# youmi-zym/GO-SLAM

Hardware: AMD Instinct MI355X
Metric: BA keyframes/s (6 x FactorGraph.update: reproject + corr lookup + GRU + 2 GN BA iters) on synthetic 640x480 RGB-D (higher is better)
Workload: dtype f32 (BA/geometry; fp64 solve), f16 (corr volume, GRU convs); 1 GPU; configs[1]-shaped frontend window: 60x80 maps (480x640 RGB-D), P=25 keyframes, E=75 edges, 6 updates/keyframe, iters=2, RGB-D depth prior, upsample on; parallelism=replicas x1 (tracking does not shard)

## Files before the change

go_slam_amd/_lib.py:

```python
import ctypes
import os
import subprocess

_HERE = os.path.dirname(os.path.abspath(__file__))
CSRC = os.path.join(_HERE, "csrc")
LIB_PATH = os.environ.get("GOSLAM_HIP_LIB") or os.path.join(CSRC, "libgoslam_hip.so")

_lib = None

c_int, c_float, c_void_p, c_size_t = ctypes.c_int, ctypes.c_float, ctypes.c_void_p, ctypes.c_size_t

_P = c_void_p
SIGNATURES = {
    "gs_version": (ctypes.c_char_p, []),
    "gs_last_error": (ctypes.c_char_p, []),
    "gs_enc_conv_wpack_elems": (c_size_t, [c_int, c_int, c_int]),
    "gs_enc_conv_stat_chunks": (c_int, [c_int, c_int, c_int]),
    "gs_enc_conv": (c_int, [_P, c_int, c_int, _P, _P, _P, c_int, c_int, c_int, c_int, c_int, c_int, c_int, _P, _P, _P]),
    "gs_norm_act_workspace_bytes_chunks": (c_size_t, [c_int, c_int, c_int]),
    "gs_timing_begin": (c_int, [_P]),
    "gs_timing_end": (c_int, []),
    "gs_timing_read": (c_int, [ctypes.c_char_p, ctypes.POINTER(ctypes.c_double), ctypes.POINTER(c_int)]),
    "gs_timing_names": (c_int, [ctypes.c_char_p, c_int]),
    "gs_corr_index_forward": (c_int, [_P, _P, _P] + [c_int] * 7 + [_P]),
    "gs_corr_index_backward": (c_int, [_P, _P, _P] + [c_int] * 7 + [_P]),
    "gs_corr_lookup_pyramid": (c_int, [_P] * 6 + [c_int] * 9 + [_P]),
    "gs_corr_lookup_enc": (c_int, [_P] * 8 + [c_int] * 7 + [_P]),
    "gs_corr_lookup_enc_slots": (c_int, [_P] * 9 + [c_int] * 7 + [_P]),
    "gs_corr_lookup_pyramid_slots": (c_int, [_P] * 7 + [c_int] * 9 + [_P]),
    "gs_corr_volume_pyramid_slots": (c_int, [_P] * 7 + [c_int] * 5 + [_P, c_size_t, _P]),
    "gs_corr_volume_workspace_bytes": (c_size_t, [c_int] * 4),
    "gs_corr_volume_pyramid": (c_int, [_P] * 6 + [c_int] * 5 + [_P, c_size_t, _P]),
    "gs_corr_level_elems": (c_size_t, [c_int] * 4),
    "gs_altcorr_backward": (c_int, [_P] * 6 + [c_int] * 8 + [_P]),
    "gs_altcorr_forward": (c_int, [_P] * 4 + [c_int] * 9 + [_P]),
    "gs_altcorr_pyramid": (c_int, [_P] * 8 + [c_int] * 5 + [_P]),
    "gs_reproject": (c_int, [_P] * 7 + [c_int] * 3 + [_P]),
    "gs_projmap": (c_int, [_P] * 7 + [c_int] * 3 + [_P]),
    "gs_frame_distance": (c_int, [_P] * 6 + [c_int] * 3 + [c_float, _P]),
    "gs_iproj": (c_int, [_P] * 4 + [c_int] * 3 + [_P]),
    "gs_depth_filter": (c_int, [_P] * 6 + [c_int] * 4 + [_P]),
    "gs_pointcloud_workspace_bytes": (c_size_t, [c_int] * 3),
    "gs_pointcloud_count": (c_int, [_P] * 5 + [c_float, c_float] + [c_int] * 4 + [_P, c_size_t, _P]),
    "gs_pointcloud_mask": (c_int, [_P, _P] + [c_int] * 4 + [_P, c_size_t, _P]),
    "gs_pointcloud_scan": (c_int, [c_int] * 3 + [_P, c_size_t, _P, _P]),
    "gs_pointcloud_emit": (c_int, [_P] * 5 + [c_int] * 4 + [_P, c_size_t, ctypes.c_longlong, _P, _P, _P]),
    "gs_tsdf_batch": (c_int, []),
    "gs_tsdf_integrate": (c_int, [_P] * 3 + [c_int] * 3 + [_P] * 4 + [c_int] * 3 + [c_float] * 10 + [_P]),
    "gs_tsdf_vertex_attr": (c_int, [_P, c_int, _P, _P, c_int, c_int, c_int, c_float, _P, _P, _P]),
    "gs_tsdf_brick_flags_bytes": (c_size_t, [c_int] * 3),
    "gs_tsdf_brick_flags": (c_int, [_P, c_int, c_int, c_int, _P, _P]),
    "gs_tsdf_raycast": (c_int, [_P] * 3 + [c_int] * 3 + [_P, _P] + [c_int] * 3 + [c_float] * 12 + [_P] * 4),
    "gs_frame_prep_color": (c_int, [_P, c_int, c_int, c_int, c_int, c_int, _P]),
    "gs_frame_prep_depth": (c_int, [_P, c_int, c_float, c_int, c_int, c_int, c_int, _P]),
    "gs_cvx_upsample":(c_int, [_P] * 4 + [c_int] * 4 + [_P]),
    "gs_upmask_upsample": (c_int, [_P, c_int, _P, _P, _P, _P, _P, c_int, c_int, c_int, _P]),
    "gs_bias_act": (c_int, [_P, _P, _P, c_int, c_int, c_int, c_int, c_int, _P]),
    "gs_motion_features": (c_int, [_P, _P, _P, c_int, c_int, c_int, _P]),
    "gs_ba_inputs": (c_int, [_P] * 6 + [c_int, c_int, c_int, _P]),
    "gs_lowmem_gather": (c_int, [_P] * 7 + [c_int, c_int, c_int, _P]),
    "gs_lowmem_scatter": (c_int, [_P] * 8 + [c_int, c_int, c_int, _P]),
    "gs_damping_rows": (c_int, [_P] * 5 + [c_int, c_int, c_float, c_float, _P]),
    "gs_conv1x1": (c_int, [_P, c_int, c_int, _P, _P, c_int, _P, c_int, c_int, ctypes.c_longlong, _P]),
    "gs_conv7x7_c4": (c_int, [_P, _P, _P, _P, c_int, c_int, c_int, c_int, c_int, c_int, _P]),
    "gs_conv3x3_wpack_elems": (c_size_t, [c_int, c_int]),
    "gs_conv3x3_pp": (c_int, [_P, c_int, c_int, _P, c_int, _P, c_int, c_int, c_int, c_int, c_int, c_int, _P]),
    "gs_conv3x3_bias_relu": (c_int, [_P, c_int, c_int, _P, _P, _P, c_int, c_int, c_int, c_int, c_int, _P]),
    "gs_conv3x3_gru_zr": (c_int, [_P, c_int, c_int, _P, _P, _P, _P, _P, _P, c_int, c_int, c_int, _P]),
    "gs_conv3x3_gru_zr2": (c_int, [_P, _P, c_int, c_int, _P, _P, _P, _P, _P, _P, c_int, c_int, c_int, _P]),
    "gs_conv3x3_gru_q": (c_int, [_P, _P, c_int, c_int, _P, _P, _P, _P, _P, _P, _P, c_int, c_int, c_int, _P]),
    "gs_conv3x3_head": (c_int, [_P, c_int, _P, c_int, _P, _P, c_int, c_int, c_float, _P, c_int, c_int, c_int, _P]),
    "gs_conv3x3_heads": (c_int, [_P, c_int, c_int, _P, c_int, _P, _P, c_int, _P, _P, c_int, c_int, c_int, c_int, c_int, _P]),
    "gs_conv3x3_heads_finish": (c_int, [_P, _P, _P, c_int, c_int, c_float, c_float, _P, _P, c_int, c_int, c_int, _P]),
    "gs_segment_mean": (c_int, [_P, c_int, _P, c_int, _P, _P, _P, c_int, c_int, c_int, _P]),
    "gs_norm_act_workspace_bytes": (c_size_t, [c_int, c_int, c_int]),
    "gs_norm_act": (c_int, [_P, _P, _P, _P] + [c_int] * 6 + [c_float, _P, c_size_t, c_int, _P]),
    "gs_gru_glo_workspace_bytes": (c_size_t, [c_int]),
    "gs_gru_glo": (c_int, [_P] * 11 + [c_int, c_int, _P, c_size_t, _P]),
    "gs_gru_glo_fused_workspace_bytes": (c_size_t, [c_int, c_int]),
    "gs_gru_glo_fused": (c_int, [_P, c_int] + [_P] * 10 + [c_int, c_int, _P, c_size_t, _P]),
    "gs_gru_gate_zr": (c_int, [_P] * 6 + [c_int] * 3 + [_P]),
    "gs_gru_gate_q": (c_int, [_P] * 7 + [c_int] * 2 + [_P]),
    "gs_edge_prep": (c_int, [_P] * 4 + [c_int, _P, _P] + [c_int] * 6 + [c_float, c_int, c_int, _P]),
    "gs_edge_greedy": (c_int, [_P] * 5 + [c_int] * 5 + [c_float, c_int, c_int, _P]),
    "gs_ba_workspace_bytes": (c_size_t, [c_int] * 5),
    "gs_ba": (c_int, [_P] * 9 + [c_int] * 3 + [c_float, c_float] + [c_int] * 6 + [_P, _P, _P, _P, c_size_t, _P]),
    "gs_ba_ex": (c_int, [_P] * 9 + [c_int] * 3 + [c_float, c_float] + [c_int] * 6 + [_P, _P, _P, _P, c_size_t, c_int, _P]),
    "gs_chol_solve": (c_int, [_P, _P, c_int, c_float, c_float, c_int, _P, _P, _P]),
    "gs_traj_eval_workspace_bytes": (c_size_t, [c_int]),
    "gs_traj_world": (c_int, [_P, _P, c_int, _P, _P, _P]),
    "gs_ape_moments": (c_int, [_P, _P, _P, c_int, _P, _P, c_size_t, _P]),
    "gs_ape_stats": (c_int, [_P, _P, _P, _P, c_int, _P, _P, _P, c_size_t, _P]),
    "gs_grid_meta_default": (c_int, [_P]),
    "gs_neus_level_major_min_points": (c_int, [c_int]),
    "gs_render_sample": (c_int, [_P] * 7 + [c_float, _P, _P, _P] + [c_int] * 3 + [_P]),
    "gs_grid_encode": (c_int, [_P] * 4 + [c_int, _P]),
    "gs_grid_backward": (c_int, [_P, _P, _P, c_int, c_float, _P, _P, c_int, c_float, _P, _P, c_int, _P]),
    "gs_mlp_workspace_bytes": (c_size_t, [c_int, c_int]),
    "gs_mlp_forward": (c_int, [_P] * 3 + [c_int] * 3 + [_P, c_size_t, _P]),
    "gs_neus_forward_workspace_bytes": (c_size_t, [c_int, c_int]),
    "gs_neus_forward": (c_int, [_P] * 9 + [c_float] + [_P] * 18 + [c_float, _P, c_float, c_int, c_int, _P, c_size_t, _P]),
    "gs_neus_forward_pieces": (c_int, [c_int] * 3),
    "gs_neus_forward_segmented": (c_int, [_P] * 9 + [c_float] + [_P] * 18 + [c_float, c_int, _P, _P, c_float]
                                  + [c_int] * 4 + [_P, c_size_t, _P]),
    "gs_render_img_sample": (c_int, [_P, c_int, c_int] + [c_float] * 4 + [_P] * 5 + [c_int] + [_P] * 5
                             + [c_int, c_int, _P]),
    "gs_render_img_metrics_workspace_bytes": (c_size_t, []),
    "gs_render_img_metrics": (c_int, [_P] * 7 + [c_int, c_int] + [_P] * 5 + [c_size_t, _P]),
    "gs_image_quality_tile": (c_int, [ctypes.POINTER(c_int), ctypes.POINTER(c_int)]),
    "gs_image_quality_workspace_bytes": (c_size_t, [c_int, c_int]),
    "gs_image_quality": (c_int, [_P] * 4 + [c_int, c_int, _P, _P, c_size_t, _P]),
    "gs_neus_backward_rays": (c_int, [_P] * 13 + [c_int, c_int, _P]),
    "gs_mapping_loss": (c_int, [_P] * 8 + [c_float] * 4 + [c_int] + [_P] * 4 + [c_int, c_int, _P]),
    "gs_map_grad_sqnorm": (c_int, [_P, c_size_t, c_float, _P, c_size_t, _P, _P]),
    "gs_map_adamw": (c_int, [_P, _P, _P, _P, _P, c_size_t, c_float, _P, c_size_t] + [c_float] * 6 + [c_int, _P, c_float, _P]),
    "gs_map_gram_blocks": (c_int, [c_int]),
    "gs_map_gram": (c_int, [_P, c_int, _P, _P]),
    "gs_map_step_prep": (c_int, [_P, c_int, _P, c_float, c_float, c_int] + [_P] * 13),
    "gs_map_step_post": (c_int, [_P, c_int, c_float, _P, c_int, _P, _P, _P, c_float, _P, _P, c_int, c_float, c_int, _P, _P, _P]),
    "gs_map_adamw_seg": (c_int, [_P, _P, _P, _P, _P, c_size_t, c_float, _P, _P, _P, _P, _P, c_size_t] + [c_float] * 6
                         + [c_int, _P, _P, c_float, _P]),
    "gs_mlp_backward_blocks": (c_int, [c_int]),
    "gs_mlp_backward": (c_int, [_P, _P, _P, _P, c_float, _P, _P, c_int, _P]),
    "gs_neus_backward_points": (c_int, [_P] * 7 + [c_float] + [_P] * 9 + [c_int, c_float, _P, _P, c_int, c_float] + [_P] * 5 + [c_int, c_float, c_int, _P, c_int, c_int, _P, _P]),
    "gs_neus_backward_points_binned": (c_int, [_P] * 7 + [c_float] + [_P] * 9 + [c_int, c_float, _P, _P, c_float] + [_P] * 5
                                       + [c_int, c_float, c_int, _P, c_int, c_int, _P, c_size_t, _P, _P, _P]),
    "gs_neus_bin_workspace_bytes": (c_size_t, [c_int]),
    "gs_neus_backward_raygrad": (c_int, [_P] * 7 + [c_float] + [_P] * 9 + [c_int, c_float] + [_P] * 3
                                 + [c_int, c_int, _P]),
    "gs_pose_grad_reduce": (c_int, [_P, _P, _P, c_int, _P, _P]),
    "gs_ray_draw": (c_int, [_P] * 7 + [c_int] * 4 + [c_float] * 4 + [_P] * 5),
    "gs_sdf_lattice": (c_int, [_P] * 3 + [c_int] * 3 + [_P] * 6 + [_P]),
    "gs_mcubes_workspace_bytes": (c_size_t, [c_int] * 3),
    "gs_mcubes_count": (c_int, [_P, c_int, c_int, c_int, c_float, _P, c_size_t, _P]),
    "gs_mcubes_scan": (c_int, [c_int, c_int, c_int, _P, c_size_t, _P, _P]),
    "gs_mcubes_emit": (c_int, [_P, c_int, c_int, c_int, c_float, _P, c_size_t, ctypes.c_longlong, ctypes.c_longlong,
                               _P, _P, _P]),
    "gs_mesh_depth_workspace_bytes": (c_size_t, []),
    "gs_mesh_depth": (c_int, [_P, c_int, _P, c_int, _P, c_int] + [c_float] * 4 + [c_int, c_int, c_float, c_float, _P, _P,
                                                                                   c_size_t, _P]),
    "gs_mesh_visibility": (c_int, [_P, c_int, _P, _P, c_int] + [c_float] * 4 + [c_int, c_int, c_float, _P, _P, _P]),
    "gs_face_components_workspace_bytes": (c_size_t, [c_int]),
    "gs_face_components": (c_int, [_P, c_int, _P, _P, c_size_t, _P]),
    "gs_face_component_areas": (c_int, [_P, _P, c_int, _P, _P, _P, _P, _P, c_size_t, _P]),
    "gs_hull_extremes_workspace_bytes": (c_size_t, [c_int]),
    "gs_hull_extremes": (c_int, [_P, c_int, _P, _P, c_size_t, _P]),
    "gs_hull_prefilter": (c_int, [_P, c_int, _P, c_int, ctypes.c_double, _P, _P]),
    "gs_mesh_visbuf_workspace_bytes": (c_size_t, []),
    "gs_mesh_visbuf": (c_int, [_P, c_int, _P, c_int, _P, c_int] + [c_float] * 4 + [c_int, c_int, c_float, c_float, _P, _P,
                                                                                    c_size_t, _P]),
    "gs_line_visbuf": (c_int, [_P, c_int, ctypes.c_uint, _P, c_int] + [c_float] * 4 + [c_int, c_int, c_float, c_float, _P,
                                                                                        _P]),
    "gs_vertex_normals": (c_int, [_P, c_int, _P, c_int, ctypes.c_double, _P, _P, _P]),
    "gs_visbuf_resolve": (c_int, [_P, c_int, c_int, c_int, _P, c_int, _P, c_int, _P] + [c_float] * 4
                          + [_P, _P, c_int, _P, c_int, c_float, c_float, ctypes.c_uint, _P, _P]),
    "gs_nn_cell_keys":(c_int, [_P, c_int, _P, _P, _P, _P]),
    "gs_nn_grid_build": (c_int, [_P, c_int, _P, _P, _P, _P, _P, _P, _P]),
    "gs_nn_query_workspace_bytes": (c_size_t, [c_int]),
    "gs_nn_query": (c_int, [_P, _P, _P, _P, c_int, _P, _P, _P, c_int, _P, ctypes.c_double, _P, _P, _P, c_size_t, _P]),
    "gs_icp_moments_workspace_bytes": (c_size_t, [c_int]),
    "gs_icp_moments": (c_int, [_P, c_int, _P, _P, _P, _P, _P, _P, c_size_t, _P]),
}


class ColorView(ctypes.Structure):
    _fields_ = [("src", c_void_p), ("map_x", c_void_p), ("map_y", c_void_p), ("tmp", c_void_p), ("dst", c_void_p),
                ("h", c_int), ("w", c_int), ("c", c_int), ("mh", c_int), ("mw", c_int)]


class DepthView(ctypes.Structure):
    _fields_ = [("src", c_void_p), ("dst", c_void_p), ("h", c_int), ("w", c_int)]


FRAME_PREP_MAX_VIEWS = 32


class GridMeta(ctypes.Structure):
    _fields_ = [("scale", c_float * 16), ("resolution", ctypes.c_uint32 * 16), ("size", ctypes.c_uint32 * 16),
                ("offset", ctypes.c_uint32 * 16), ("hashed", ctypes.c_uint32 * 16), ("total", ctypes.c_uint32)]


def grid_meta():
    m = GridMeta()
    check(lib().gs_grid_meta_default(ctypes.byref(m)), "gs_grid_meta_default")
    return m


def build(verbose=False):
    cmd = ["make", "-C", CSRC, "-j8"]
    res = subprocess.run(cmd, stdout=subprocess.PIPE, stderr=subprocess.STDOUT, text=True)
    if verbose or res.returncode != 0:
        print(res.stdout)
    if res.returncode != 0:
        raise RuntimeError("building libgoslam_hip.so failed:\n" + res.stdout[-4000:])
    return LIB_PATH


def lib():
    global _lib
    if _lib is None:
        if not os.path.exists(LIB_PATH):
            raise RuntimeError(
                f"{LIB_PATH} not found: build it with `python -c 'import __graft_entry__ as g; g.build()'` "
                "(go_slam_amd has no CPU fallback)")
        handle = ctypes.CDLL(LIB_PATH)
        for name, (res, args) in SIGNATURES.items():
            fn = getattr(handle, name)
            fn.restype = res
            fn.argtypes = args
        _lib = handle
    return _lib


def check(rc, what):
    if rc != 0:
# ... 49 lines not shown
```

go_slam_amd/csrc/ba.hip:

```cpp
#include "common.h"

int gs_chol_solve_launch(double* H, double* b, int n, float lm, float ep, float* dx_out, int32_t* fail_flag,
                         int32_t* fail_count, hipStream_t st);

namespace {

constexpr float kMinDepth = 0.25f;
constexpr float kAlpha = 0.05f;
constexpr int kPrepThreads = 1024;
constexpr int kAccSplit = 4;
constexpr int kMaxBuf = 4096;

struct BaWs {
  int32_t* hdr;
  int32_t* kinv;
  int32_t* kx;
  int32_t* edge_m;
  int32_t* row_ptr;
  int32_t* csr_edge;
  int32_t* ent_ptr;
  int32_t* ent_src;
  int32_t* ent_pose;
  int32_t* pair_ptr;
  float* Q;
  float* W;
  float* Ei;
  float* Eij;
  float* part;
  double* H;
  double* b;
  size_t total;
};

BaWs carve(void* base, int E, int P, int M, int nbuf, int hw) {
  BaWs w;
  size_t off = 0;
  auto take = [&](size_t bytes) { size_t o = off; off += gs_align(bytes); return (char*)base + o; };
  w.hdr = (int32_t*)take(16 * 4);
  w.kinv = (int32_t*)take((size_t)nbuf * 4);
  w.kx = (int32_t*)take((size_t)(M + 1) * 4);
  w.edge_m = (int32_t*)take((size_t)(E + 1) * 4);
  w.row_ptr = (int32_t*)take((size_t)(M + 2) * 4);
  w.csr_edge = (int32_t*)take((size_t)(E + 1) * 4);
  w.ent_ptr = (int32_t*)take((size_t)(M + 2) * 4);
  w.ent_src = (int32_t*)take((size_t)(M + E + 1) * 4);
  w.ent_pose = (int32_t*)take((size_t)(M + E + 1) * 4);
  w.pair_ptr = (int32_t*)take((size_t)(M + 2) * 4);
  w.Q = (float*)take((size_t)M * hw * 4);
  w.W = (float*)take((size_t)M * hw * 4);
  w.Ei = (float*)take((size_t)M * 6 * hw * 4);
  w.Eij = (float*)take((size_t)E * 6 * hw * 4);
  w.part = (float*)take((size_t)kAccSplit * M * 8 * hw * 4);
  const size_t n = (size_t)6 * P;
  w.H = (double*)take((n * n + n) * 8);
  w.b = w.H + n * n;
  w.total = off;
  return w;
}

__device__ void block_exclusive_scan(int* data, int n, int* scratch , int* total) {
  const int tid = threadIdx.x;
  const int per = (n + kPrepThreads - 1) / kPrepThreads;
  const int beg = min(tid * per, n), end = min(beg + per, n);
  int s = 0;
  for (int i = beg; i < end; ++i) s += data[i];
  scratch[tid] = s;
  __syncthreads();
  for (int off = 1; off < kPrepThreads; off <<= 1) {
    int v = (tid >= off) ? scratch[tid - off] : 0;
    __syncthreads();
    scratch[tid] += v;
    __syncthreads();
  }
  int run = scratch[tid] - s;
  for (int i = beg; i < end; ++i) {
    int v = data[i];
    data[i] = run;
    run += v;
  }
  if (tid == kPrepThreads - 1) *total = scratch[tid];
  __syncthreads();
}

__global__ __launch_bounds__(kPrepThreads) void ba_prep_kernel(
    const int64_t* __restrict__ ii, const int64_t* __restrict__ jj, int E, int nbuf, int t0, int t1,
    int M_host, BaWs w) {
  __shared__ int flag[kMaxBuf];
  __shared__ int cnt_a[kMaxBuf];
  __shared__ int cnt_b[kMaxBuf];
  __shared__ int scratch[kPrepThreads];
  __shared__ int total;
  const int tid = threadIdx.x;

  for (int k = tid; k < nbuf; k += kPrepThreads) flag[k] = (k >= t0 && k < t1) ? 1 : 0;
  __syncthreads();
  for (int e = tid; e < E; e += kPrepThreads) {
    const int i = (int)ii[e];
    if (i >= 0 && i < nbuf) flag[i] = 1;
  }
  __syncthreads();
  for (int k = tid; k < nbuf; k += kPrepThreads) cnt_a[k] = flag[k];
  __syncthreads();
  block_exclusive_scan(flag, nbuf, scratch, &total);
  const int M_dev = total;
  const int M = min(M_dev, M_host);
  for (int k = tid; k < nbuf; k += kPrepThreads) {
    const bool mem = cnt_a[k] != 0;
    const int r = flag[k];
    const int row = (mem && r < M) ? r : -1;
    w.kinv[k] = row;
    if (row >= 0) w.kx[row] = k;
  }
  if (tid == 0) {
    w.hdr[0] = M_dev;
    w.hdr[1] = (M_dev != M_host) ? 1 : 0;
    w.hdr[2] = 0;
    w.hdr[3] = 0;
  }
  __syncthreads();
  for (int m = tid; m < kMaxBuf; m += kPrepThreads) { cnt_a[m] = 0; cnt_b[m] = 0; }
  __syncthreads();
  for (int k = tid; k < nbuf; k += kPrepThreads) {
    const int row = w.kinv[k];
    if (row >= 0 && k >= t0 && k < t1) cnt_b[row] = 1;
  }
  __syncthreads();
  for (int e = tid; e < E; e += kPrepThreads) {
    const int i = (int)ii[e], j = (int)jj[e];
    const int row = (i >= 0 && i < nbuf) ? w.kinv[i] : -1;
    w.edge_m[e] = row;
    if (row >= 0) {
      atomicAdd(&cnt_a[row], 1);
      if (j >= t0 && j < t1) atomicAdd(&cnt_b[row], 1);
    }
  }
  __syncthreads();
  for (int m = tid; m < M_host; m += kPrepThreads) flag[m] = cnt_b[m] * cnt_b[m];
  __syncthreads();
  block_exclusive_scan(cnt_a, M_host, scratch, &total);
  if (tid == 0) w.row_ptr[M_host] = total;
  block_exclusive_scan(cnt_b, M_host, scratch, &total);
  if (tid == 0) w.ent_ptr[M_host] = total;
  block_exclusive_scan(flag, M_host, scratch, &total);
  if (tid == 0) { w.pair_ptr[M_host] = total; w.hdr[4] = total; }
  __syncthreads();
  for (int m = tid; m < M_host; m += kPrepThreads) {
    w.row_ptr[m] = cnt_a[m];
    w.ent_ptr[m] = cnt_b[m];
    w.pair_ptr[m] = flag[m];
  }
  __syncthreads();
  for (int m = tid; m < M; m += kPrepThreads) {
    int rp = cnt_a[m], ep = cnt_b[m];
    const int k = w.kx[m];
    if (k >= t0 && k < t1) { w.ent_src[ep] = m; w.ent_pose[ep] = k - t0; ++ep; }
    for (int e = 0; e < E; ++e) {
      if (w.edge_m[e] == m) {
        w.csr_edge[rp++] = e;
        const int j = (int)jj[e];
        if (j >= t0 && j < t1) { w.ent_src[ep] = M_host + e; w.ent_pose[ep] = j - t0; ++ep; }
      }
    }
  }
}

__global__ __launch_bounds__(256) void ba_accum_kernel(
    const float* __restrict__ poses, const float* __restrict__ disps, const float* __restrict__ intr,
    const float* __restrict__ disps_sens, const float* __restrict__ targets, const float* __restrict__ weights,
    const float* __restrict__ eta, const int64_t* __restrict__ jj, int t0, int t1, int hw, int wd,
    int motion_only, int reset_fail, BaWs w) {
  __shared__ float red[4][92];
  if (reset_fail && blockIdx.x == 0 && blockIdx.y == 0 && blockIdx.z == 0 && threadIdx.x == 0) { w.hdr[2] = 0; w.hdr[3] = 0; }
  typedef const __attribute__((address_space(4))) int* cip;
  typedef const __attribute__((address_space(4))) int64_t* clp;
  typedef const __attribute__((address_space(4))) float* cfp;
  const int m = blockIdx.y;
  if (m >= ((cip)w.hdr)[0]) return;
  const int split = blockIdx.z, nsp = gridDim.z;
  const int nsplit = min(nsp, max(((cip)w.row_ptr)[m + 1] - ((cip)w.row_ptr)[m], 1));
  if (split >= nsplit) return;
  const int tid = threadIdx.x;
  const int p = blockIdx.x * 256 + tid;
  const bool active = p < hw;
  const int pc = active ? p : hw - 1;
  const int k = ((cip)w.kx)[m];
  const int P = t1 - t0;
  const int n6 = 6 * P;
  const float fx = ((cfp)intr)[0], fy = ((cfp)intr)[1], cx = ((cfp)intr)[2], cy = ((cfp)intr)[3];
  const float u = (float)(pc % wd), v = (float)(pc / wd);
  const float disp = disps[(size_t)k * hw + pc];
  float Xi[4] = {(u - cx) / fx, (v - cy) / fy, 1.0f, disp};
  float ti[3], qi[4];
  {
    cfp pp = (cfp)(poses + (size_t)k * 7);
    ti[0] = pp[0]; ti[1] = pp[1]; ti[2] = pp[2];
    qi[0] = pp[3]; qi[1] = pp[4]; qi[2] = pp[5]; qi[3] = pp[6];
  }
  const int pi = k - t0;
  const bool i_in = (pi >= 0) && (pi < P);

  float Csum = 0.f, wsum = 0.f;
  float Ei[6] = {0.f, 0.f, 0.f, 0.f, 0.f, 0.f};

  const int e_beg = ((cip)w.row_ptr)[m], e_end = ((cip)w.row_ptr)[m + 1];
  for (int idx = e_beg + split; idx < e_end; idx += nsp) {
    const int e = ((cip)w.csr_edge)[idx];
    const int jx = (int)((clp)jj)[e];
    const size_t tb = ((size_t)e * 2) * hw + pc;
    const float w_u = weights[tb], w_v = weights[tb + hw], t_u = targets[tb], t_v = targets[tb + hw];
    float tij[3], qij[4];
    if (jx == k) {
      tij[0] = -0.1f; tij[1] = 0.f; tij[2] = 0.f;
      qij[0] = 0.f; qij[1] = 0.f; qij[2] = 0.f; qij[3] = 1.f;
    } else {
      cfp pj = (cfp)(poses + (size_t)jx * 7);
      float tj[3] = {pj[0], pj[1], pj[2]};
      float qj[4] = {pj[3], pj[4], pj[5], pj[6]};
      gs_rel_se3(ti, qi, tj, qj, tij, qij);
    }
    float Xj[4];
    gs_act_se3(tij, qij, Xi, Xj);
    const float x = Xj[0], y = Xj[1], h = Xj[3];
    const bool close = Xj[2] < kMinDepth;
    const float d = close ? 0.0f : 1.0f / Xj[2];
    const float d2 = d * d;
    float wu = (close || !active) ? 0.0f : 0.001f * w_u;
    float wv = (close || !active) ? 0.0f : 0.001f * w_v;
    const float ru = t_u - (fx * d * x + cx);
    const float rv = t_v - (fy * d * y + cy);

    float hij[78];
#pragma unroll
    for (int l = 0; l < 78; ++l) hij[l] = 0.f;
    float vi[6], vj[6], Eii_e[6], Eij_e[6];
    float Jx[12];
    float* Ji = &Jx[0];
    float* Jj = &Jx[6];

    Jj[0] = fx * (h * d);
    Jj[1] = fx * 0.0f;
    Jj[2] = fx * (-x * h * d2);
    Jj[3] = fx * (-x * y * d2);
    Jj[4] = fx * (1.0f + x * x * d2);
    Jj[5] = fx * (-y * d);
    float Jz = fx * (tij[0] * d - tij[2] * (x * d2));
    float Ce = wu * Jz * Jz;
    float be = wu * ru * Jz;
    if (jx == k) wu = 0.0f;
    gs_adj_se3(tij, qij, Jj, Ji);
#pragma unroll
    for (int n = 0; n < 6; ++n) Ji[n] = -Ji[n];
    {
      int l = 0;
#pragma unroll
      for (int n = 0; n < 12; ++n)
#pragma unroll
        for (int mm = 0; mm <= n; ++mm) { hij[l] = fmaf(wu * Jx[n], Jx[mm], hij[l]); ++l; }
    }
#pragma unroll
    for (int n = 0; n < 6; ++n) {
      vi[n] = wu * ru * Ji[n];
      vj[n] = wu * ru * Jj[n];
      Eii_e[n] = wu * Jz * Ji[n];
      Eij_e[n] = wu * Jz * Jj[n];
    }
    Jj[0] = fy * 0.0f;
    Jj[1] = fy * (h * d);
    Jj[2] = fy * (-y * h * d2);
    Jj[3] = fy * (-1.0f - y * y * d2);
    Jj[4] = fy * (x * y * d2);
    Jj[5] = fy * (x * d);
    Jz = fy * (tij[1] * d - tij[2] * (y * d2));
    Ce = Ce + wv * Jz * Jz;
    be = be + wv * rv * Jz;
    if (jx == k) wv = 0.0f;
    gs_adj_se3(tij, qij, Jj, Ji);
#pragma unroll
    for (int n = 0; n < 6; ++n) Ji[n] = -Ji[n];
    {
      int l = 0;
#pragma unroll
      for (int n = 0; n < 12; ++n)
#pragma unroll
        for (int mm = 0; mm <= n; ++mm) { hij[l] = fmaf(wv * Jx[n], Jx[mm], hij[l]); ++l; }
    }
#pragma unroll
    for (int n = 0; n < 6; ++n) {
      vi[n] = vi[n] + wv * rv * Ji[n];
      vj[n] = vj[n] + wv * rv * Jj[n];
      Eii_e[n] = Eii_e[n] + wv * Jz * Ji[n];
      Eij_e[n] = Eij_e[n] + wv * Jz * Jj[n];
    }

    if (!motion_only) {
      Csum += Ce;
      wsum += be;
#pragma unroll
      for (int n = 0; n < 6; ++n) Ei[n] += Eii_e[n];
      if (active) {
        float* eo = w.Eij + ((size_t)e * 6) * hw + p;
#pragma unroll
        for (int n = 0; n < 6; ++n) eo[(size_t)n * hw] = Eij_e[n];
      }
    }

    const int pj_ = jx - t0;
    const bool j_in = (pj_ >= 0) && (pj_ < P);
    if (i_in || j_in) {
      const int wave = tid >> 6, lane = tid & 63;
      float rs[90];
#pragma unroll
      for (int l = 0; l < 78; ++l) rs[l] = hij[l];
#pragma unroll
      for (int n = 0; n < 6; ++n) { rs[78 + n] = vi[n]; rs[84 + n] = vj[n]; }
      gs_wave_reduce_scatter<90>(rs, lane);
      const int ix = gs_bitrev6(lane);
      red[wave][ix] = rs[0];
      if (64 + ix < 90) red[wave][64 + ix] = rs[1];
      __syncthreads();
      if (tid < 90) {
        const double s = (double)((red[0][tid] + red[1][tid]) + (red[2][tid] + red[3][tid]));
        if (tid < 78) {
          int n = 0;
          while ((n + 1) * (n + 2) / 2 <= tid) ++n;
          const int mm = tid - n * (n + 1) / 2;
// ... 13 lines not shown
      }
      __syncthreads();
    }
  }

  if (!motion_only && active) {
    if (nsplit > 1) {
      float* po = w.part + (((size_t)split * gridDim.y + m) * 8) * hw + p;
      po[0] = Csum;
      po[(size_t)hw] = wsum;
#pragma unroll
      for (int n = 0; n < 6; ++n) po[(size_t)(2 + n) * hw] = Ei[n];
      return;
    }
    const size_t o = (size_t)m * hw + p;
    const float sens = disps_sens[(size_t)k * hw + p];
    const float mk = (sens > 0.0f) ? 1.0f : 0.0f;
    const float C = Csum + mk * kAlpha + (1.0f - mk) * eta[o];
    const float ww = wsum - mk * kAlpha * (disp - sens);
    w.Q[o] = 1.0f / C;
    w.W[o] = ww;
    if (i_in) {
      float* eo = w.Ei + ((size_t)m * 6) * hw + p;
#pragma unroll
      for (int n = 0; n < 6; ++n) eo[(size_t)n * hw] = Ei[n];
    }
  }
}

__global__ __launch_bounds__(256) void ba_accum_finish_kernel(const float* __restrict__ disps,
                                                              const float* __restrict__ disps_sens,
                                                              const float* __restrict__ eta, int t0, int t1, int hw, int nsp,
                                                              BaWs w) {
  const int m = blockIdx.y;
  if (m >= w.hdr[0]) return;
  const int nsplit = min(nsp, max(w.row_ptr[m + 1] - w.row_ptr[m], 1));
  if (nsplit <= 1) return;
  const int p = blockIdx.x * 256 + threadIdx.x;
  if (p >= hw) return;
  float acc[8];
#pragma unroll
  for (int n = 0; n < 8; ++n) acc[n] = 0.0f;
  for (int s2 = 0; s2 < nsplit; ++s2) {
    const float* pi_ = w.part + (((size_t)s2 * gridDim.y + m) * 8) * hw + p;
#pragma unroll
    for (int n = 0; n < 8; ++n) acc[n] += pi_[(size_t)n * hw];
  }
  const int k = w.kx[m];
  const size_t o = (size_t)m * hw + p;
  const float disp = disps[(size_t)k * hw + p];
  const float sens = disps_sens[(size_t)k * hw + p];
  const float mk = (sens > 0.0f) ? 1.0f : 0.0f;
  const float C = acc[0] + mk * kAlpha + (1.0f - mk) * eta[o];
  const float ww = acc[1] - mk * kAlpha * (disp - sens);
  w.Q[o] = 1.0f / C;
  w.W[o] = ww;
  const int pi = k - t0;
  if (pi >= 0 && pi < t1 - t0) {
    float* eo = w.Ei + ((size_t)m * 6) * hw + p;
#pragma unroll
    for (int n = 0; n < 6; ++n) eo[(size_t)n * hw] = acc[2 + n];
  }
}

__global__ __launch_bounds__(256) void ba_schur_kernel(int M, int hw, int P, BaWs w) {
  __shared__ float red[4][44];
  const int tid = threadIdx.x;
  const int wave = tid >> 6, lane = tid & 63;
  typedef const __attribute__((address_space(4))) int* cip;
  cip pair_ptr = (cip)w.pair_ptr, ent_ptr = (cip)w.ent_ptr, ent_pose = (cip)w.ent_pose, ent_src = (cip)w.ent_src;
  const int n_pairs = pair_ptr[M];
  const int n6 = 6 * P;
  for (int pidx = blockIdx.x; pidx < n_pairs; pidx += gridDim.x) {
    int lo = 0, hi = M;
    while (hi - lo > 1) {
      const int mid = (lo + hi) >> 1;
      if (pair_ptr[mid] <= pidx) lo = mid; else hi = mid;
    }
    const int m = lo;
    const int eb = ent_ptr[m];
    const int nm = ent_ptr[m + 1] - eb;
    const int r = pidx - pair_ptr[m];
    const int a = r / nm, b = r - a * nm;
    const int pa = ent_pose[eb + a], pb = ent_pose[eb + b];
    if (pa < pb) continue;
    const int sa = ent_src[eb + a], sb = ent_src[eb + b];
    const float* Ea = (sa < M) ? w.Ei + (size_t)sa * 6 * hw : w.Eij + (size_t)(sa - M) * 6 * hw;
    const float* Eb = (sb < M) ? w.Ei + (size_t)sb * 6 * hw : w.Eij + (size_t)(sb - M) * 6 * hw;
    const float* Qm = w.Q + (size_t)m * hw;
    const float* Wm = w.W + (size_t)m * hw;
    const bool diag = (a == b);
    float S[36];
#pragma unroll
    for (int i = 0; i < 36; ++i) S[i] = 0.f;
    float vv[6] = {0.f, 0.f, 0.f, 0.f, 0.f, 0.f};
    constexpr int UP = 4;
    for (int p0 = tid; p0 < hw; p0 += UP * 256) {
      float q[UP], ea[UP][6], eb_[UP][6], ww[UP];
#pragma unroll
      for (int u = 0; u < UP; ++u) {
        const int p = p0 + 256 * u;
        const bool ok = p < hw;
        const int pc = ok ? p : tid;
        q[u] = Qm[pc];
#pragma unroll
        for (int n = 0; n < 6; ++n) {
          ea[u][n] = Ea[(size_t)n * hw + pc];
          eb_[u][n] = Eb[(size_t)n * hw + pc];
        }
        ww[u] = diag ? Wm[pc] : 0.0f;
      }
#pragma unroll
      for (int u = 0; u < UP; ++u) {
        if (p0 + 256 * u < hw) {
#pragma unroll
          for (int n = 0; n < 6; ++n) ea[u][n] = ea[u][n] * q[u];
#pragma unroll
          for (int n = 0; n < 6; ++n)
#pragma unroll
            for (int c = 0; c < 6; ++c) S[n * 6 + c] = fmaf(ea[u][n], eb_[u][c], S[n * 6 + c]);
          if (diag) {
#pragma unroll
            for (int n = 0; n < 6; ++n) vv[n] = fmaf(ea[u][n], ww[u], vv[n]);
          }
        }
      }
    }
    {
      float rs[42];
#pragma unroll
      for (int i = 0; i < 36; ++i) rs[i] = S[i];
#pragma unroll
      for (int n = 0; n < 6; ++n) rs[36 + n] = vv[n];
      gs_wave_reduce_scatter<42>(rs, lane);
      const int ix = gs_bitrev6(lane);
      if (ix < 42) red[wave][ix] = rs[0];
    }
    __syncthreads();
    if (tid < 36) {
      const int rr = tid / 6, cc = tid - rr * 6;
      const double s = (double)((red[0][tid] + red[1][tid]) + (red[2][tid] + red[3][tid]));
      if (pa > pb || rr >= cc)
        gs_atomic_add_f64(&w.H[(size_t)(6 * pa + rr) * n6 + (6 * pb + cc)], -s);
    } else if (diag && tid < 42) {
      const double s = (double)((red[0][tid] + red[1][tid]) + (red[2][tid] + red[3][tid]));
      gs_atomic_add_f64(&w.b[6 * pa + (tid - 36)], -s);
    }
    __syncthreads();
  }
}

__global__ __launch_bounds__(256) void ba_update_kernel(
    float* __restrict__ poses, float* __restrict__ disps, const float* __restrict__ dx,
    float* __restrict__ dz, int M, int t0, int t1, int hw, BaWs w) {
  const int tid = threadIdx.x;
  const int P = t1 - t0;
  if ((int)blockIdx.y == M) {
    if (blockIdx.x != 0) return;
    for (int kk = t0 + tid; kk < t1; kk += 256) {
      float* pp = poses + (size_t)kk * 7;
      float t[3] = {pp[0], pp[1], pp[2]};
      float q[4] = {pp[3], pp[4], pp[5], pp[6]};
      float xi[6], tn[3], qn[4];
#pragma unroll
      for (int n = 0; n < 6; ++n) xi[n] = dx[(size_t)(kk - t0) * 6 + n];
      gs_retr_se3(xi, t, q, tn, qn);
      pp[0] = tn[0]; pp[1] = tn[1]; pp[2] = tn[2];
      pp[3] = qn[0]; pp[4] = qn[1]; pp[5] = qn[2]; pp[6] = qn[3];
    }
    return;
  }
  const int m = blockIdx.y;
  const int p = blockIdx.x * 256 + tid;
  if (p >= hw) return;
  if (m >= w.hdr[0]) {
    dz[(size_t)m * hw + p] = 0.0f;
    return;
  }
  const int eb = w.ent_ptr[m], ee = w.ent_ptr[m + 1];
  float dw = 0.f;
  for (int idx = eb; idx < ee; ++idx) {
    const int pn = w.ent_pose[idx];
    if (pn <= 0 || pn >= P) continue;
    const int s = w.ent_src[idx];
    const float* En = (s < M) ? w.Ei + (size_t)s * 6 * hw : w.Eij + (size_t)(s - M) * 6 * hw;
    float acc = 0.f;
#pragma unroll
    for (int n = 0; n < 6; ++n) acc += En[(size_t)n * hw + p] * dx[(size_t)pn * 6 + n];
    dw += acc;
  }
  const size_t o = (size_t)m * hw + p;
  const float z = w.Q[o] * (w.W[o] - dw);
  dz[o] = z;
  const size_t dk = (size_t)w.kx[m] * hw + p;
  disps[dk] = disps[dk] + z;
}

__global__ void ba_status_kernel(int32_t* status_out, BaWs w) {
  if (threadIdx.x < 4) status_out[threadIdx.x] = (threadIdx.x == 2) ? w.hdr[3] : (threadIdx.x == 3 ? w.hdr[4] : w.hdr[threadIdx.x]);
}

}

extern "C" size_t gs_ba_workspace_bytes(int n_edges, int n_poses, int n_depth, int nbuf, int hw) {
  if (n_edges < 0 || n_poses < 0 || n_depth < 0 || nbuf < 0 || hw < 0) return 0;
  return carve(nullptr, n_edges, n_poses, n_depth, nbuf, hw).total + 256;
}

extern "C" int gs_ba_ex(float* poses, float* disps, const float* intrinsics, const float* disps_sens,
                        const float* targets, const float* weights, const float* eta, const int64_t* ii,
                        const int64_t* jj, int t0, int t1, int iterations, float lm, float ep, int motion_only,
                        int n_edges, int n_depth, int nbuf, int h, int w, float* dx, float* dz,
                        int32_t* status_out, void* workspace, size_t workspace_bytes, int flags, gs_stream_t stream) {
  GS_REQUIRE(poses && disps && intrinsics && disps_sens && targets && weights && ii && jj && dx && workspace,
             "ba: null pointer");
  GS_REQUIRE(motion_only || (eta && dz), "ba: eta/dz required unless motion_only");
  GS_REQUIRE(h > 0 && w > 0 && n_edges >= 0 && iterations >= 0, "ba: bad shape");
  GS_REQUIRE(t0 >= 0 && t1 > t0 && t1 <= nbuf, "ba: window [%d,%d) outside buffer of %d frames", t0, t1, nbuf);
  GS_REQUIRE(nbuf <= kMaxBuf, "ba: buffer of %d frames exceeds the supported %d", nbuf, kMaxBuf);
  GS_REQUIRE(n_depth > 0 && n_depth <= nbuf && n_depth <= 65534, "ba: n_depth=%d out of range", n_depth);
  const int hw = h * w, P = t1 - t0, M = n_depth;
  const size_t need = gs_ba_workspace_bytes(n_edges, P, M, nbuf, hw);
  if (workspace_bytes < need) {
    gs_set_error("ba: workspace too small (%zu < %zu bytes)", workspace_bytes, need);
    return GS_ERR_WORKSPACE;
  }
  void* base = (void*)gs_align((size_t)workspace);
  BaWs ws = carve(base, n_edges, P, M, nbuf, hw);
  hipStream_t st = (hipStream_t)stream;
  const int n6 = 6 * P;

  const bool reuse = (flags & 1) != 0;
  if (!reuse) {
    ba_prep_kernel<<<1, kPrepThreads, 0, st>>>(ii, jj, n_edges, nbuf, t0, t1, M, ws);
    GS_CHECK_LAUNCH("ba_prep");
  }
  const int chunks = gs_cdiv(hw, 256);
  for (int it = 0; it < iterations; ++it) {
    if (hipMemsetAsync(ws.H, 0, ((size_t)n6 * n6 + n6) * sizeof(double), st) != hipSuccess) {
      gs_set_error("ba: memset failed");
      return GS_ERR_LAUNCH;
    }
    const int nsp = (!motion_only && n_edges >= 6 * M) ? kAccSplit : 1;
    ba_accum_kernel<<<dim3(chunks, M, nsp), 256, 0, st>>>(poses, disps, intrinsics, disps_sens, targets, weights,
                                                          eta, jj, t0, t1, hw, w, motion_only,
                                                          (reuse && it == 0) ? 1 : 0, ws);
    GS_CHECK_LAUNCH("ba_accum");
    if (!motion_only) {
      if (nsp > 1) {
        ba_accum_finish_kernel<<<dim3(chunks, M), 256, 0, st>>>(disps, disps_sens, eta, t0, t1, hw, nsp, ws);
        GS_CHECK_LAUNCH("ba_accum_finish");
      }
      ba_schur_kernel<<<2048, 256, 0, st>>>(M, hw, P, ws);
      GS_CHECK_LAUNCH("ba_schur");
    }
    int rc = gs_chol_solve_launch(ws.H, ws.b, n6, lm, ep, dx, &ws.hdr[2], &ws.hdr[3], st);
    if (rc != GS_OK) return rc;
    if (motion_only)
      ba_update_kernel<<<dim3(1, 1), 256, 0, st>>>(poses, disps, dx, dz, 0, t0, t1, hw, ws);
    else
      ba_update_kernel<<<dim3(chunks, M + 1), 256, 0, st>>>(poses, disps, dx, dz, M, t0, t1, hw, ws);
    GS_CHECK_LAUNCH("ba_update");
  }
  if (status_out) {
    ba_status_kernel<<<1, 64, 0, st>>>(status_out, ws);
    GS_CHECK_LAUNCH("ba_status");
  }
  return GS_OK;
}

extern "C" int gs_ba(float* poses, float* disps, const float* intrinsics, const float* disps_sens,
                     const float* targets, const float* weights, const float* eta, const int64_t* ii,
                     const int64_t* jj, int t0, int t1, int iterations, float lm, float ep, int motion_only,
                     int n_edges, int n_depth, int nbuf, int h, int w, float* dx, float* dz,
                     int32_t* status_out, void* workspace, size_t workspace_bytes, gs_stream_t stream) {
  return gs_ba_ex(poses, disps, intrinsics, disps_sens, targets, weights, eta, ii, jj, t0, t1, iterations, lm, ep,
                  motion_only, n_edges, n_depth, nbuf, h, w, dx, dz, status_out, workspace, workspace_bytes, 0, stream);
}
```

go_slam_amd/csrc/chol.hip:

```cpp
#include "common.h"

namespace {

constexpr int NB = 32;
constexpr int PR = 64;
constexpr int TT = 64;
constexpr int SB = 64;

__device__ __forceinline__ double readlane_f64(double v, int lane) {
  const unsigned long long u = __builtin_bit_cast(unsigned long long, v);
  const unsigned int lo = __builtin_amdgcn_readlane((int)(u & 0xffffffffu), lane);
  const unsigned int hi = __builtin_amdgcn_readlane((int)(u >> 32), lane);
  return __builtin_bit_cast(double, ((unsigned long long)hi << 32) | lo);
}

__device__ __forceinline__ void sqrt_rsqrt(double x, double& s, double& rs) {
  const double r = __builtin_amdgcn_rsq(x);
  double g = x * r, h = 0.5 * r;
  double e = fma(-g, h, 0.5);
  g = fma(g, e, g); h = fma(h, e, h);
  e = fma(-g, h, 0.5);
  g = fma(g, e, g); h = fma(h, e, h);
  s = g; rs = h + h;
}
// ... 461 lines not shown
  for (int p0 = 0; p0 < n; p0 += PW) {
    const int pend = min(p0 + PW, n);
    for (int k0 = p0; k0 < pend; k0 += CB) {
      const int s0 = k0 + CB;
      const int rows = n + 1 - s0;
      const int kw = k0 - p0;
      if (kw > 0) {
        const int rr = tid / 3, cg = tid - 3 * rr;
        if (rr < rows + CB) {
          const int r = k0 + rr;
          const double* Xr = Lp + tri(r, p0);
          const int c0 = 2 * cg, c1 = c0 + 1;
          const bool ok0 = k0 + c0 <= r && k0 + c0 < n, ok1 = k0 + c1 <= r && k0 + c1 < n;
          const double* L0 = Lp + tri(min(k0 + c0, n - 1), p0);
          const double* L1 = Lp + tri(min(k0 + c1, n - 1), p0);
          double a0 = 0.0, a1 = 0.0;
#pragma unroll 6
          for (int k = 0; k < kw; ++k) {
            const double x = Xr[k];
            a0 = fma(x, L0[k], a0);
            a1 = fma(x, L1[k], a1);
          }
          if (ok0) Lp[tri(r, k0 + c0)] -= a0;
          if (ok1) Lp[tri(r, k0 + c1)] -= a1;
        }
        __syncthreads();
      }
      CHOL_ACC(2);
      const bool need = tid < ((max(rows, CB) + 63) & ~63);
      double l[CB][CB], inv[CB];
      if (need) {
#pragma unroll
        for (int i = 0; i < CB; ++i)
#pragma unroll
          for (int j = 0; j <= i; ++j) l[i][j] = Lp[tri(k0 + i, k0 + j)];
#pragma unroll
        for (int j = 0; j < CB; ++j) {
          double piv = l[j][j];
#pragma unroll
          for (int t = 0; t < j; ++t) piv = fma(-l[j][t], l[j][t], piv);
          if (!(piv > 0.0) && piv == piv) bad = true;
          sqrt_rsqrt(piv, l[j][j], inv[j]);
#pragma unroll
          for (int i = j + 1; i < CB; ++i) {
            double sacc = l[i][j];
#pragma unroll
            for (int t = 0; t < j; ++t) sacc = fma(-l[i][t], l[j][t], sacc);
            l[i][j] = sacc * inv[j];
          }
        }
      }
      CHOL_ACC(0);
      if (tid < rows) {
        double* Ar = Lp + tri(s0 + tid, k0);
        double x[CB];
#pragma unroll
        for (int j = 0; j < CB; ++j) {
          double s = Ar[j];
#pragma unroll
          for (int u = 0; u < j; ++u) s = fma(-x[u], l[j][u], s);
          x[j] = s * inv[j];
        }
#pragma unroll
        for (int j = 0; j < CB; ++j) Ar[j] = x[j];
      }
      CHOL_ACC(1);
      __syncthreads();
      if (tid < CB) {
#pragma unroll
        for (int i = 0; i < CB; ++i)
          if (i == tid) {
#pragma unroll
            for (int j = 0; j <= i; ++j) Lp[tri(k0 + i, k0 + j)] = l[i][j];
            invd[k0 + i] = inv[i];
          }
      }
      CHOL_ACC(3);
    }
    const int s1 = pend;
    const int rows1 = n + 1 - s1;
    const int pw = pend - p0;
    if (rows1 > 1) {
      typedef double double4v __attribute__((ext_vector_type(4)));
      const int T = (rows1 + 15) >> 4, ntile = (T * (T + 1)) >> 1;
      const int wv = __builtin_amdgcn_readfirstlane(tid >> 6), ln = tid & 63;
      for (int t = wv; t < ntile; t += SMALL_NT / 64) {
        int ti = (int)((sqrtf(8.0f * (float)t + 1.0f) - 1.0f) * 0.5f);
        while (((ti + 1) * (ti + 2)) >> 1 <= t) ++ti;
        while ((ti * (ti + 1)) >> 1 > t) --ti;
        const int tj = t - ((ti * (ti + 1)) >> 1);
        const int r0 = s1 + 16 * ti, c0 = s1 + 16 * tj;
        const double* pa = Lp + tri(min(r0 + (ln & 15), n), p0);
        const double* pb = Lp + tri(min(c0 + (ln & 15), n), p0);
        double4v acc = {0.0, 0.0, 0.0, 0.0};
#pragma unroll
        for (int kb = 0; kb < (PW + 3) / 4; ++kb) {
          const int k = 4 * kb + (ln >> 4);
          const double a = k < pw ? pa[k] : 0.0, b = k < pw ? pb[k] : 0.0;
          acc = __builtin_amdgcn_mfma_f64_16x16x4f64(a, b, acc, 0, 0, 0);
        }
        const int c = c0 + (ln & 15);
#pragma unroll
        for (int q = 0; q < 4; ++q) {
          const int rr = r0 + (ln >> 4) + 4 * q;
          if (rr <= n && c < n && c <= rr) Lp[tri(rr, c)] -= acc[q];
        }
      }
    }
    __syncthreads();
    CHOL_ACC(4);
  }
  CHOL_ACC_DUMP;
}

__device__ __forceinline__ void lds_backward(double* Lp, const double* invd, const int n, float* __restrict__ dx) {
  const int npk = (n * (n + 1)) >> 1;
  double* y = Lp + npk;
  if (threadIdx.x < 64) {
    const int lane = threadIdx.x;
    for (int k0 = n - CB; k0 >= 0; k0 -= CB) {
      double l[CB][CB], x[CB];
#pragma unroll
      for (int i = 0; i < CB; ++i)
#pragma unroll
        for (int j = 0; j <= i; ++j) l[i][j] = Lp[tri(k0 + i, k0 + j)];
#pragma unroll
      for (int i = CB - 1; i >= 0; --i) {
        double sacc = y[k0 + i];
#pragma unroll
        for (int t = i + 1; t < CB; ++t) sacc = fma(-l[t][i], x[t], sacc);
        x[i] = sacc * invd[k0 + i];
      }
      for (int c = k0 - 1 - lane; c >= 0; c -= 64) {
        double s = y[c];
#pragma unroll
        for (int i = 0; i < CB; ++i) s = fma(-Lp[tri(k0 + i, c)], x[i], s);
        y[c] = s;
      }
      if (lane < CB) {
        double xl = x[0];
#pragma unroll
        for (int i = 1; i < CB; ++i) xl = (i == lane) ? x[i] : xl;
        dx[k0 + lane] = (float)xl;
        y[k0 + lane] = xl;
      }
      __builtin_amdgcn_fence(__ATOMIC_RELEASE, "wavefront");
      __builtin_amdgcn_wave_barrier();
      __builtin_amdgcn_fence(__ATOMIC_ACQUIRE, "wavefront");
    }
  }
  __syncthreads();
}

__device__ __forceinline__ void lds_load_packed(double* Lp, const double* __restrict__ H, const double* __restrict__ bg,
                                                const int n, const int c0, const double lm, const double ep) {
  const int tid = threadIdx.x;
  const int m = n - c0;
  const int npk = (m * (m + 1)) >> 1;
  for (int base = 0; base < npk; base += SMALL_NT * 4) {
    double v[4];
    int dg[4];
#pragma unroll
    for (int u = 0; u < 4; ++u) {
      const int idx = base + u * SMALL_NT + tid;
      int r = (int)((sqrtf(8.0f * (float)idx + 1.0f) - 1.0f) * 0.5f);
      while (((r + 1) * (r + 2)) >> 1 <= idx) ++r;
      while ((r * (r + 1)) >> 1 > idx) --r;
      const int c = idx - ((r * (r + 1)) >> 1);
      dg[u] = (c == r) ? 1 : 0;
      v[u] = idx < npk ? H[(size_t)(c0 + r) * n + (c0 + c)] : 0.0;
    }
#pragma unroll
    for (int u = 0; u < 4; ++u) {
      const int idx = base + u * SMALL_NT + tid;
      if (idx < npk) Lp[idx] = dg[u] ? v[u] + (ep + lm * v[u]) : v[u];
    }
  }
  for (int i = tid; i <= m; i += SMALL_NT) Lp[npk + i] = (i < m) ? bg[c0 + i] : 0.0;
}

__global__ __launch_bounds__(SMALL_NT) void chol_small_kernel(const double* __restrict__ H, const double* __restrict__ bg,
                                                         int n, double lm, double ep, float* __restrict__ dx,
                                                         int32_t* fail_flag, int32_t* fail_count) {
  extern __shared__ double sm[];
  double* Lp = sm;
  double* invd = sm + (((n + 1) * (n + 2)) >> 1);
  const int tid = threadIdx.x;
  CHOL_STAMP(0);
  lds_load_packed(Lp, H, bg, n, 0, lm, ep);
  __syncthreads();
  CHOL_STAMP(1);

  __shared__ int s_bad;
  bool bad = false;
  lds_factor(Lp, invd, n, bad);
  CHOL_STAMP(2);

  if (tid == 0) s_bad = bad ? 1 : 0;
  __syncthreads();
  if (s_bad) {
    for (int i = tid; i < n; i += SMALL_NT) dx[i] = 0.0f;
    if (tid == 0) { *fail_flag = 1; *fail_count += 1; }
    return;
  }
  if (tid == 0) *fail_flag = 0;
  lds_backward(Lp, invd, n, dx);
  CHOL_STAMP(3);
}

#ifndef CHOL_TB
#define CHOL_TB 2
#endif
constexpr int MID_N = 300;
constexpr int MID_SW60_N = 300;

template <int KS>
__device__ __forceinline__ __attribute__((ext_vector_type(4))) double mid_tile_product(const double* pa, const double* pb,
                                                                                      int ln, int SW) {
  typedef double double4v __attribute__((ext_vector_type(4)));
  double4v acc = {0.0, 0.0, 0.0, 0.0};
  constexpr int G = 5;
#pragma unroll
  for (int g0 = 0; g0 < KS; g0 += G) {
    double a[G], b[G];
#pragma unroll
    for (int u = 0; u < G; ++u) {
      const int k = 4 * (g0 + u) + (ln >> 4);
      a[u] = (g0 + u < KS && k < SW) ? pa[k] : 0.0;
      b[u] = (g0 + u < KS && k < SW) ? pb[k] : 0.0;
    }
#pragma unroll
    for (int u = 0; u < G; ++u)
      if (g0 + u < KS) acc = __builtin_amdgcn_mfma_f64_16x16x4f64(a[u], b[u], acc, 0, 0, 0);
  }
  return acc;
}

__global__ __launch_bounds__(SMALL_NT) void chol_mid_kernel(double* __restrict__ H, double* __restrict__ bg, int n,
                                                       double lm, double ep, int SW, float* __restrict__ dx,
                                                       int32_t* fail_flag, int32_t* fail_count) {
  extern __shared__ double sm[];
  typedef double double4v __attribute__((ext_vector_type(4)));
  const int tid = threadIdx.x;
  const int wv = __builtin_amdgcn_readfirstlane(tid >> 6), ln = tid & 63;
  double* invd = sm;
  double* yv = sm + n;
  double* T = sm + 2 * n;
  const int SWP = SW + 1;
  __shared__ int s_bad;
  bool bad = false;
  for (int i = tid; i < n; i += SMALL_NT) {
    const double d = H[(size_t)i * n + i];
    H[(size_t)i * n + i] = d + (ep + lm * d);
  }
  __syncthreads();
  int c0 = 0;
  CHOL_STAMP(20);
  for (; n - c0 > SMALL_N; c0 += SW) {
    const int R = n + 1 - c0;
    const int stg_ = (c0 / SW) < 4 ? 21 + 4 * (c0 / SW) : 56;
    (void)stg_;
    for (int base = 0; base < R * SW; base += 4 * SMALL_NT) {
      double v[4];
      int at[4];
#pragma unroll
      for (int u = 0; u < 4; ++u) {
        const int idx = base + u * SMALL_NT + tid;
        const int r = idx / SW, k = idx - r * SW;
        v[u] = 0.0;
        at[u] = idx < R * SW ? r * SWP + k : -1;
        if (idx < R * SW) {
          if (r == R - 1) v[u] = bg[c0 + k];
          else if (k <= r) v[u] = H[(size_t)(c0 + r) * n + (c0 + k)];
        }
      }
#pragma unroll
      for (int u = 0; u < 4; ++u)
        if (at[u] >= 0) T[at[u]] = v[u];
    }
    __syncthreads();
    CHOL_STAMP(stg_ + 0);
    for (int p0 = 0; p0 < SW; p0 += PW) {
      const int pend = p0 + PW;
      for (int k0 = p0; k0 < pend; k0 += CB) {
        const int s0 = k0 + CB;
        const int rows = R - s0;
        const int kw = k0 - p0;
        if (kw > 0) {
          const int cg = tid % 3;
          for (int rr = tid < 3 * (SMALL_NT / 3) ? tid / 3 : R; rr < rows + CB; rr += SMALL_NT / 3) {
            const int r = k0 + rr;
            const double* Xr = T + r * SWP + p0;
            const int c0 = 2 * cg, c1 = c0 + 1;
            const bool ok0 = k0 + c0 <= r, ok1 = k0 + c1 <= r;
            const double* L0 = T + (k0 + c0) * SWP + p0;
            const double* L1 = T + (k0 + c1) * SWP + p0;
            double a0 = 0.0, a1 = 0.0;
#pragma unroll 6
            for (int k = 0; k < kw; ++k) {
              const double x = Xr[k];
              a0 = fma(x, L0[k], a0);
              a1 = fma(x, L1[k], a1);
            }
            if (ok0) T[r * SWP + k0 + c0] -= a0;
            if (ok1) T[r * SWP + k0 + c1] -= a1;
          }
          __syncthreads();
        }
        const bool need = tid < ((max(rows, CB) + 63) & ~63);
        double l[CB][CB], inv[CB];
        if (need) {
#pragma unroll
          for (int i = 0; i < CB; ++i)
#pragma unroll
            for (int j = 0; j <= i; ++j) l[i][j] = T[(k0 + i) * SWP + (k0 + j)];
#pragma unroll
          for (int j = 0; j < CB; ++j) {
            double piv = l[j][j];
#pragma unroll
            for (int t = 0; t < j; ++t) piv = fma(-l[j][t], l[j][t], piv);
            if (!(piv > 0.0) && piv == piv) bad = true;
            sqrt_rsqrt(piv, l[j][j], inv[j]);
#pragma unroll
            for (int i = j + 1; i < CB; ++i) {
              double sacc = l[i][j];
#pragma unroll
              for (int t = 0; t < j; ++t) sacc = fma(-l[i][t], l[j][t], sacc);
              l[i][j] = sacc * inv[j];
            }
          }
        }
        if (tid < rows) {
          double* Ar = T + (s0 + tid) * SWP + k0;
          double x[CB];
#pragma unroll
          for (int j = 0; j < CB; ++j) {
            double s = Ar[j];
#pragma unroll
            for (int u = 0; u < j; ++u) s = fma(-x[u], l[j][u], s);
            x[j] = s * inv[j];
          }
#pragma unroll
// ... 63 lines not shown
            if (ok[u][q]) cur[u][q] = (rl == R - 1) ? bg[c0 + cl] : H[(size_t)(c0 + rl) * n + (c0 + cl)];
          }
        }
#pragma unroll
        for (int u = 0; u < TB; ++u) {
          if (tb + u >= ntile) break;
          const double* pa = T + min(r0s[u] + (ln & 15), R - 1) * SWP;
          const double* pb = T + min(q0s[u] + (ln & 15), R - 1) * SWP;
          const double4v acc = SW == 60 ? mid_tile_product<15>(pa, pb, ln, SW) : mid_tile_product<8>(pa, pb, ln, SW);
          const int cl = q0s[u] + (ln & 15);
#pragma unroll
          for (int q = 0; q < 4; ++q) {
            const int rl = r0s[u] + (ln >> 4) + 4 * q;
            if (ok[u][q]) {
              const double v = cur[u][q] - acc[q];
              if (rl == R - 1) bg[c0 + cl] = v;
              else H[(size_t)(c0 + rl) * n + (c0 + cl)] = v;
            }
          }
        }
      }
    }
    CHOL_STAMP(stg_ + 2);
    for (int idx = tid; idx < (R - 1) * SW; idx += SMALL_NT) {
      const int r = idx / SW, k = idx - r * SW;
      if (k <= r) H[(size_t)(c0 + r) * n + (c0 + k)] = T[r * SWP + k];
    }
    for (int k = tid; k < SW; k += SMALL_NT) yv[c0 + k] = T[(R - 1) * SWP + k];
    __threadfence_block();
    __syncthreads();
    CHOL_STAMP(stg_ + 3);
  }
  const int m = n - c0;
  double* Lp = T;
  lds_load_packed(Lp, H, bg, n, c0, 0.0, 0.0);
  __syncthreads();
  CHOL_STAMP(40);
  lds_factor(Lp, invd + c0, m, bad);
  CHOL_STAMP(41);
  if (tid == 0) s_bad = 0;
  __syncthreads();
  if (bad) s_bad = 1;
  __syncthreads();
  if (s_bad) {
    for (int i = tid; i < n; i += SMALL_NT) dx[i] = 0.0f;
    if (tid == 0) { *fail_flag = 1; *fail_count += 1; }
    return;
  }
  if (tid == 0) *fail_flag = 0;
  lds_backward(Lp, invd + c0, m, dx + c0);
  CHOL_STAMP(42);
  {
    const double* xt = Lp + ((m * (m + 1)) >> 1);
    for (int i = tid; i < m; i += SMALL_NT) yv[c0 + i] = xt[i];
  }
  __syncthreads();
  {
    double* part = T;
    const int ng = 8;
    for (int idx = tid; idx < ng * c0; idx += SMALL_NT) {
      const int g = idx / c0, c = idx - g * c0;
      double s = 0.0;
      for (int r = c0 + g; r < n; r += ng) s = fma(H[(size_t)r * n + c], yv[r], s);
      part[g * c0 + c] = s;
    }
    __syncthreads();
    for (int c = tid; c < c0; c += SMALL_NT) {
      double s = yv[c];
#pragma unroll
      for (int g = 0; g < 8; ++g) s -= part[g * c0 + c];
      yv[c] = s;
    }
    __syncthreads();
  }
  CHOL_STAMP(43);
  for (int a = c0 - SW; a >= 0; a -= SW) {
    for (int idx = tid; idx < SW * SW; idx += SMALL_NT) {
      const int r = idx / SW, k = idx - r * SW;
      T[r * SWP + k] = (k <= r) ? H[(size_t)(a + r) * n + (a + k)] : 0.0;
    }
    __syncthreads();
    for (int k0 = SW - CB; k0 >= 0; k0 -= CB) {
      double x[CB];
      if (tid < ((max(k0, CB) + 63) & ~63)) {
        double l[CB][CB];
#pragma unroll
        for (int i = 0; i < CB; ++i)
#pragma unroll
          for (int j = 0; j <= i; ++j) l[i][j] = T[(k0 + i) * SWP + (k0 + j)];
#pragma unroll
        for (int i = CB - 1; i >= 0; --i) {
          double sacc = yv[a + k0 + i];
#pragma unroll
          for (int t = i + 1; t < CB; ++t) sacc = fma(-l[t][i], x[t], sacc);
          x[i] = sacc * invd[a + k0 + i];
        }
      }
      __syncthreads();
      if (tid < CB) {
#pragma unroll
        for (int i = 0; i < CB; ++i)
          if (i == tid) { dx[a + k0 + i] = (float)x[i]; yv[a + k0 + i] = x[i]; }
      }
      for (int c = tid; c < k0; c += SMALL_NT) {
        double s = yv[a + c];
#pragma unroll
        for (int i = 0; i < CB; ++i) s = fma(-T[(k0 + i) * SWP + c], x[i], s);
        yv[a + c] = s;
      }
      __syncthreads();
    }
    if (a > 0) {
      double* part = T;
      const int ng = min(16, SMALL_NT / a);
      for (int idx = tid; idx < ng * a; idx += SMALL_NT) {
        const int g = idx / a, c = idx - g * a;
        double s = 0.0;
        for (int r = g; r < SW; r += ng) s = fma(H[(size_t)(a + r) * n + c], yv[a + r], s);
        part[g * a + c] = s;
      }
      __syncthreads();
      for (int c = tid; c < a; c += SMALL_NT) {
        double s = yv[c];
        for (int g = 0; g < ng; ++g) s -= part[g * a + c];
        yv[c] = s;
      }
      __syncthreads();
    }
  }
  CHOL_STAMP(44);
}

enum { CHOL_PATH_DISPATCH = 0, CHOL_PATH_SMALL = 1, CHOL_PATH_MID = 2, CHOL_PATH_BLOCKED = 3 };

size_t chol_mid_lds(int n) {
  const int SW = n <= MID_SW60_N ? 60 : 30;
  const size_t tall = (size_t)(n + 1) * (SW + 1);
  const size_t tail = (size_t)(SMALL_N + 1) * (SMALL_N + 2) / 2 + SMALL_N;
  return ((size_t)2 * n + (tall > tail ? tall : tail)) * sizeof(double);
}

bool chol_small_fits(int n) { return n >= 1 && n <= SMALL_N && n % CB == 0; }
bool chol_mid_fits(int n) {
  return n >= 1 && n <= MID_N && n % CB == 0 && chol_mid_lds(n) <= 160 * 1024 - 256;
}

int chol_dispatch(int n) {
  if (chol_small_fits(n)) return CHOL_PATH_SMALL;
  if (chol_mid_fits(n)) return CHOL_PATH_MID;
  return CHOL_PATH_BLOCKED;
}

int chol_solve_path(double* H, double* b, int n, float lm, float ep, int path, float* dx_out, int32_t* fail_flag,
                    int32_t* fail_count, hipStream_t st) {
  if (path == CHOL_PATH_SMALL) {
    const size_t lds = ((size_t)(n + 1) * (n + 2) / 2 + (size_t)n) * sizeof(double);
    static GsLdsLimit limit;
    const size_t cap = ((size_t)(SMALL_N + 1) * (SMALL_N + 2) / 2 + SMALL_N) * sizeof(double);
    if (int rc = limit.raise((const void*)chol_small_kernel, cap, "chol")) return rc;
    chol_small_kernel<<<1, SMALL_NT, lds, st>>>(H, b, n, (double)lm, (double)ep, dx_out, fail_flag, fail_count);
    GS_CHECK_LAUNCH("chol_small");
    return GS_OK;
  }
  if (path == CHOL_PATH_MID) {
    const int SW = n <= MID_SW60_N ? 60 : 30;
    const size_t lds = chol_mid_lds(n);
    static GsLdsLimit limit;
    if (int rc = limit.raise((const void*)chol_mid_kernel, lds, "chol_mid")) return rc;
    chol_mid_kernel<<<1, SMALL_NT, lds, st>>>(H, b, n, (double)lm, (double)ep, SW, dx_out, fail_flag, fail_count);
    GS_CHECK_LAUNCH("chol_mid");
    return GS_OK;
  }
  const int nb0 = n < NB ? n : NB;
  chol_panel_kernel<<<gs_cdiv(n - nb0 + 1, PR), 64, 0, st>>>(H, b, n, 0, fail_flag, 1, (double)lm, (double)ep);
  GS_CHECK_LAUNCH("chol_panel");
  constexpr size_t step_lds = ((size_t)NB * DS + (size_t)(2 * NB + 2 * PR) * (NB + 1) + NB) * sizeof(double);
  static_assert(step_lds >= (size_t)2 * TT * (NB + 1) * sizeof(double), "chol_step: the trailing role's operands fit");
  for (int kp = 0; kp + NB < n; kp += NB) {
    const int c1 = kp + NB, nb1 = (n - c1 < NB) ? (n - c1) : NB, rem1 = n - c1 - nb1;
    const int n_panel = gs_cdiv(rem1 + 1, PR);
    const int T = rem1 > 0 ? gs_cdiv(rem1 + 1, TT) : 0;
    chol_step_kernel<<<n_panel + T * (T + 1) / 2, 256, step_lds, st>>>(H, b, n, kp, n_panel, fail_flag);
    GS_CHECK_LAUNCH("chol_step");
  }
  int k0 = ((n - 1) / SB) * SB;
  for (; k0 >= SB; k0 -= 2 * SB) {
    const int k_lo = k0 - SB;
    chol_back_pair_kernel<<<gs_cdiv(k_lo, 192) + 1, 256, 0, st>>>(H, b, n, k_lo, dx_out, fail_flag, fail_count);
    GS_CHECK_LAUNCH("chol_back_pair");
  }
  if (k0 == 0) {
    chol_back_block_kernel<<<1, 256, 0, st>>>(H, b, n, 0, dx_out, fail_flag, fail_count);
    GS_CHECK_LAUNCH("chol_back_block");
  }
  return GS_OK;
}

}

int gs_chol_solve_launch(double* H, double* b, int n, float lm, float ep, float* dx_out, int32_t* fail_flag,
                         int32_t* fail_count, hipStream_t st) {
  return chol_solve_path(H, b, n, lm, ep, chol_dispatch(n), dx_out, fail_flag, fail_count, st);
}

extern "C" int gs_chol_solve(double* H, double* b, int n, float lm, float ep, int path, float* dx, int32_t* status,
                             gs_stream_t stream) {
  GS_REQUIRE(n >= 1, "chol_solve: n = %d < 1", n);
  GS_REQUIRE(path >= CHOL_PATH_DISPATCH && path <= CHOL_PATH_BLOCKED, "chol_solve: unknown path %d (0 .. 3)", path);
  if (path == CHOL_PATH_SMALL && !chol_small_fits(n)) {
    gs_set_error("chol_solve: the small path needs n <= %d and n %% %d == 0 (n = %d)", SMALL_N, CB, n);
    return GS_ERR_UNSUPPORTED;
  }
  if (path == CHOL_PATH_MID && !chol_mid_fits(n)) {
    gs_set_error("chol_solve: the mid path needs n <= %d, n %% %d == 0 and %zu B of LDS to fit (n = %d)", MID_N, CB,
                 chol_mid_lds(n), n);
    return GS_ERR_UNSUPPORTED;
  }
  GS_REQUIRE(H && b && dx && status, "chol_solve: null pointer");
  if (path == CHOL_PATH_DISPATCH) path = chol_dispatch(n);
  return chol_solve_path(H, b, n, lm, ep, path, dx, status, status + 1, (hipStream_t)stream);
}
```

go_slam_amd/csrc/common.h:

```cpp
#pragma once
#include <hip/hip_runtime.h>
#include <hip/hip_fp16.h>
#include <stdint.h>
#include <stdio.h>
#include <stdarg.h>

#include "../../include/goslam_hip.h"

#define GS_WAVE 64

void gs_set_error(const char* fmt, ...);

#define GS_REQUIRE(cond, ...)                      \
  do {                                             \
    if (!(cond)) {                                 \
      gs_set_error(__VA_ARGS__);                   \
      return GS_ERR_INVALID_ARG;                   \
    }                                              \
  } while (0)

extern thread_local int gs_timing_on;
void gs_timing_mark(const char* name);

#define GS_TIMING_PRE()                      \
  do {                                       \
    if (gs_timing_on) gs_timing_mark("");    \
  } while (0)

#define GS_CHECK_LAUNCH(name)                                                   \
  do {                                                                          \
     \
    hipError_t e_ = hipGetLastError();                                          \
    if (gs_timing_on) gs_timing_mark(name);                                     \
    if (e_ != hipSuccess) {                                                     \
      gs_set_error("%s: launch failed: %s", name, hipGetErrorString(e_));       \
      return GS_ERR_LAUNCH;                                                     \
    }                                                                           \
  } while (0)

#include <atomic>
struct GsLdsLimit {
  std::atomic<unsigned int> raised[64];
  GsLdsLimit() { for (auto& r : raised) r.store(0u, std::memory_order_relaxed); }
  int raise(const void* fn, size_t bytes, const char* what) {
    int dev = 0;
    if (hipGetDevice(&dev) != hipSuccess) dev = 0;
    std::atomic<unsigned int>& slot = raised[dev & 63];
    if (dev < 64 && slot.load(std::memory_order_acquire) >= bytes) return GS_OK;
    if (hipFuncSetAttribute(fn, hipFuncAttributeMaxDynamicSharedMemorySize, (int)bytes) != hipSuccess) {
      gs_set_error("%s: cannot raise the dynamic LDS limit to %zu bytes", what, bytes);
      return GS_ERR_LAUNCH;
    }
    unsigned int cur = slot.load(std::memory_order_relaxed);
    while (cur < bytes && !slot.compare_exchange_weak(cur, (unsigned int)bytes, std::memory_order_release)) {}
    return GS_OK;
  }
};

static inline int gs_cdiv(int a, int b) { return (a + b - 1) / b; }
static inline size_t gs_align(size_t x, size_t a = 256) { return (x + a - 1) / a * a; }


__device__ __forceinline__ void gs_act_so3(const float* q, const float* X, float* Y) {
  float uv0 = 2.0f * (q[1] * X[2] - q[2] * X[1]);
  float uv1 = 2.0f * (q[2] * X[0] - q[0] * X[2]);
  float uv2 = 2.0f * (q[0] * X[1] - q[1] * X[0]);
  Y[0] = X[0] + q[3] * uv0 + (q[1] * uv2 - q[2] * uv1);
  Y[1] = X[1] + q[3] * uv1 + (q[2] * uv0 - q[0] * uv2);
  Y[2] = X[2] + q[3] * uv2 + (q[0] * uv1 - q[1] * uv0);
}

__device__ __forceinline__ void gs_act_se3(const float* t, const float* q, const float* X, float* Y) {
  float R[3];
  gs_act_so3(q, X, R);
  Y[0] = R[0] + X[3] * t[0];
  Y[1] = R[1] + X[3] * t[1];
  Y[2] = R[2] + X[3] * t[2];
  Y[3] = X[3];
}

__device__ __forceinline__ void gs_adj_se3(const float* t, const float* q, const float* X, float* Y) {
  float qinv[4] = {-q[0], -q[1], -q[2], q[3]};
  gs_act_so3(qinv, &X[0], &Y[0]);
  gs_act_so3(qinv, &X[3], &Y[3]);
  float u[3], v[3];
  u[0] = t[2] * X[1] - t[1] * X[2];
  u[1] = t[0] * X[2] - t[2] * X[0];
  u[2] = t[1] * X[0] - t[0] * X[1];
  gs_act_so3(qinv, u, v);
  Y[3] = Y[3] + v[0];
  Y[4] = Y[4] + v[1];
  Y[5] = Y[5] + v[2];
}

__device__ __forceinline__ void gs_rel_se3(const float* ti, const float* qi, const float* tj,
                                           const float* qj, float* tij, float* qij) {
  qij[0] = -qj[3] * qi[0] + qj[0] * qi[3] - qj[1] * qi[2] + qj[2] * qi[1];
  qij[1] = -qj[3] * qi[1] + qj[1] * qi[3] - qj[2] * qi[0] + qj[0] * qi[2];
  qij[2] = -qj[3] * qi[2] + qj[2] * qi[3] - qj[0] * qi[1] + qj[1] * qi[0];
  qij[3] = qj[3] * qi[3] + qj[0] * qi[0] + qj[1] * qi[1] + qj[2] * qi[2];
  float r[3];
  gs_act_so3(qij, ti, r);
  tij[0] = tj[0] - r[0];
  tij[1] = tj[1] - r[1];
  tij[2] = tj[2] - r[2];
}

__device__ __forceinline__ void gs_quat_mul(const float* a, const float* b, float* o) {
  o[0] = a[3] * b[0] + a[0] * b[3] + a[1] * b[2] - a[2] * b[1];
  o[1] = a[3] * b[1] + a[1] * b[3] + a[2] * b[0] - a[0] * b[2];
  o[2] = a[3] * b[2] + a[2] * b[3] + a[0] * b[1] - a[1] * b[0];
  o[3] = a[3] * b[3] - a[0] * b[0] - a[1] * b[1] - a[2] * b[2];
}

__device__ __forceinline__ void gs_exp_so3(const float* phi, float* q) {
  float theta_sq = phi[0] * phi[0] + phi[1] * phi[1] + phi[2] * phi[2];
  float theta_p4 = theta_sq * theta_sq;
  float theta = sqrtf(theta_sq);
  float imag, real;
  if (theta_sq < 1e-8f) {
    imag = 0.5f - (1.0f / 48.0f) * theta_sq + (1.0f / 3840.0f) * theta_p4;
    real = 1.0f - (1.0f / 8.0f) * theta_sq + (1.0f / 384.0f) * theta_p4;
  } else {
    imag = sinf(0.5f * theta) / theta;
    real = cosf(0.5f * theta);
  }
  q[0] = imag * phi[0];
  q[1] = imag * phi[1];
  q[2] = imag * phi[2];
  q[3] = real;
}

__device__ __forceinline__ void gs_cross_inplace(const float* a, float* b) {
  float x0 = a[1] * b[2] - a[2] * b[1];
  float x1 = a[2] * b[0] - a[0] * b[2];
  float x2 = a[0] * b[1] - a[1] * b[0];
  b[0] = x0; b[1] = x1; b[2] = x2;
}

__device__ __forceinline__ void gs_exp_se3(const float* xi, float* t, float* q) {
  gs_exp_so3(xi + 3, q);
  float tau[3] = {xi[0], xi[1], xi[2]};
  float phi[3] = {xi[3], xi[4], xi[5]};
  float theta_sq = phi[0] * phi[0] + phi[1] * phi[1] + phi[2] * phi[2];
  float theta = sqrtf(theta_sq);
  t[0] = tau[0]; t[1] = tau[1]; t[2] = tau[2];
  if (theta > 1e-4f) {
    float a = (1.0f - cosf(theta)) / theta_sq;
    gs_cross_inplace(phi, tau);
    t[0] = t[0] + a * tau[0];
    t[1] = t[1] + a * tau[1];
    t[2] = t[2] + a * tau[2];
    float b = (theta - sinf(theta)) / (theta * theta_sq);
    gs_cross_inplace(phi, tau);
    t[0] = t[0] + b * tau[0];
    t[1] = t[1] + b * tau[1];
    t[2] = t[2] + b * tau[2];
  }
}

__device__ __forceinline__ void gs_retr_se3(const float* xi, const float* t, const float* q,
                                            float* t1, float* q1) {
  float dt[3], dq[4];
  gs_exp_se3(xi, dt, dq);
  gs_quat_mul(dq, q, q1);
  float r[3];
  gs_act_so3(dq, t, r);
  t1[0] = r[0] + dt[0];
  t1[1] = r[1] + dt[1];
  t1[2] = r[2] + dt[2];
}

template <int CTRL>
__device__ __forceinline__ float gs_dpp(float v) {
  return __builtin_bit_cast(float, __builtin_amdgcn_update_dpp(0, __builtin_bit_cast(int, v), CTRL, 0xf, 0xf, true));
}

__device__ __forceinline__ float gs_wave_sum(float v) {
  v = v + gs_dpp<0xB1>(v);
  v = v + gs_dpp<0x4E>(v);
  v = v + gs_dpp<0x141>(v);
  v = v + gs_dpp<0x140>(v);
  float r0 = __builtin_bit_cast(float, __builtin_amdgcn_readlane(__builtin_bit_cast(int, v), 0));
  float r1 = __builtin_bit_cast(float, __builtin_amdgcn_readlane(__builtin_bit_cast(int, v), 16));
  float r2 = __builtin_bit_cast(float, __builtin_amdgcn_readlane(__builtin_bit_cast(int, v), 32));
  float r3 = __builtin_bit_cast(float, __builtin_amdgcn_readlane(__builtin_bit_cast(int, v), 48));
  return (r0 + r1) + (r2 + r3);
}

__device__ __forceinline__ float gs_sigmoid(float x) { return __builtin_amdgcn_rcpf(1.0f + __expf(-x)); }
__device__ __forceinline__ float gs_tanh(float x) {
// ... 54 lines not shown
```

go_slam_amd/csrc/geom.hip:

```cpp
#include "geom_common.h"

namespace {

constexpr float kMinDepthKernel = 0.25f;
constexpr float kMinDepthPy = 0.2f;

__global__ __launch_bounds__(256) void reproject_kernel(
    const float* __restrict__ poses, const float* __restrict__ disps, const float* __restrict__ intr,
    const int64_t* __restrict__ ii, const int64_t* __restrict__ jj, float* __restrict__ coords,
    float* __restrict__ valid, int hw, int wd) {
  const int p = blockIdx.x * 256 + threadIdx.x;
  const int e = blockIdx.y;
  if (p >= hw) return;
  const int ix = (int)ii[e], jx = (int)jj[e];
  float tij[3], qij[4];
  if (ix == jx) {
    tij[0] = -0.1f; tij[1] = 0.f; tij[2] = 0.f;
    qij[0] = 0.f; qij[1] = 0.f; qij[2] = 0.f; qij[3] = 1.f;
  } else {
    float ti[3], qi[4], tj[3], qj[4];
    gs_load_pose(poses, ix, ti, qi);
    gs_load_pose(poses, jx, tj, qj);
    float qinv[4] = {-qi[0], -qi[1], -qi[2], qi[3]};
    float r[3], tinv[3];
    gs_act_so3(qinv, ti, r);
    tinv[0] = -r[0]; tinv[1] = -r[1]; tinv[2] = -r[2];
    gs_act_so3(qj, tinv, r);
    tij[0] = tj[0] + r[0]; tij[1] = tj[1] + r[1]; tij[2] = tj[2] + r[2];
    gs_quat_mul(qj, qinv, qij);
  }
  const float fxi = intr[ix * 4 + 0], fyi = intr[ix * 4 + 1], cxi = intr[ix * 4 + 2], cyi = intr[ix * 4 + 3];
  const float fxj = intr[jx * 4 + 0], fyj = intr[jx * 4 + 1], cxj = intr[jx * 4 + 2], cyj = intr[jx * 4 + 3];
  const float u = (float)(p % wd), v = (float)(p / wd);
  float X0[4] = {(u - cxi) / fxi, (v - cyi) / fyi, 1.0f, disps[(size_t)ix * hw + p]};
  float X1[4];
  gs_act_se3(tij, qij, X0, X1);
  const float Z = (X1[2] < 0.5f * kMinDepthPy) ? 1.0f : X1[2];
  const size_t o = (size_t)e * hw + p;
  reinterpret_cast<float2*>(coords)[o] = make_float2(fxj * (X1[0] / Z) + cxj, fyj * (X1[1] / Z) + cyj);
  valid[o] = ((X1[2] > kMinDepthPy) && (X0[2] > kMinDepthPy)) ? 1.0f : 0.0f;
}

__global__ __launch_bounds__(256) void projmap_kernel(
    const float* __restrict__ poses, const float* __restrict__ disps, const float* __restrict__ intr,
    const int64_t* __restrict__ ii, const int64_t* __restrict__ jj, float* __restrict__ coords,
    float* __restrict__ valid, int hw, int wd) {
  const int p = blockIdx.x * 256 + threadIdx.x;
  const int e = blockIdx.y;
  if (p >= hw) return;
  const int ix = (int)ii[e], jx = (int)jj[e];
  float ti[3], qi[4], tj[3], qj[4], tij[3], qij[4];
  gs_load_pose(poses, ix, ti, qi);
  gs_load_pose(poses, jx, tj, qj);
  gs_rel_se3(ti, qi, tj, qj, tij, qij);
  const float fx = intr[0], fy = intr[1], cx = intr[2], cy = intr[3];
  const float u = (float)(p % wd), v = (float)(p / wd);
  float Xi[4] = {(u - cx) / fx, (v - cy) / fy, 1.0f, disps[(size_t)ix * hw + p]};
  float Xj[4];
  gs_act_se3(tij, qij, Xi, Xj);
  float cu = u, cv = v;
  if (Xj[2] > 0.01f) {
    cu = fx * (Xj[0] / Xj[2]) + cx;
    cv = fy * (Xj[1] / Xj[2]) + cy;
  }
  const size_t o = (size_t)e * hw + p;
  coords[o * 3 + 0] = cu;
  coords[o * 3 + 1] = cv;
  coords[o * 3 + 2] = 0.0f;
  valid[o] = (Xj[2] > kMinDepthKernel) ? 1.0f : 0.0f;
}

__global__ __launch_bounds__(256) void frame_distance_kernel(
    const float* __restrict__ poses, const float* __restrict__ disps, const float* __restrict__ intr,
    const int64_t* __restrict__ ii, const int64_t* __restrict__ jj, float* __restrict__ dist,
    int hw, int wd, float beta) {
  const int e = blockIdx.x;
  const int ix = (int)ii[e], jx = (int)jj[e];
  float ti[3], qi[4], tj[3], qj[4], tij[3], qij[4];
  gs_load_pose(poses, ix, ti, qi);
  gs_load_pose(poses, jx, tj, qj);
  gs_rel_se3(ti, qi, tj, qj, tij, qij);
  const float fx = intr[0], fy = intr[1], cx = intr[2], cy = intr[3];
  float accum = 0.f, valid = 0.f;
  const float* dsp = disps + (size_t)ix * hw;
  for (int p = threadIdx.x; p < hw; p += 256) {
    const float u = (float)(p % wd), v = (float)(p / wd);
    float Xi[4] = {(u - cx) / fx, (v - cy) / fy, 1.0f, dsp[p]};
    float Xj[4];
    gs_act_se3(tij, qij, Xi, Xj);
    float du = fx * (Xj[0] / Xj[2]) + cx - u;
    float dv = fy * (Xj[1] / Xj[2]) + cy - v;
    float d = sqrtf(du * du + dv * dv);
    if (Xj[2] > kMinDepthKernel) { accum += beta * d; valid += beta; }
    float Yx = Xi[0] + Xi[3] * tij[0];
    float Yy = Xi[1] + Xi[3] * tij[1];
    float Yz = Xi[2] + Xi[3] * tij[2];
    du = fx * (Yx / Yz) + cx - u;
    dv = fy * (Yy / Yz) + cy - v;
    d = sqrtf(du * du + dv * dv);
    if (Yz > kMinDepthKernel) { accum += (1.0f - beta) * d; valid += (1.0f - beta); }
  }
  __shared__ float red[2][4];
  accum = gs_wave_sum(accum);
  valid = gs_wave_sum(valid);
  const int wave = threadIdx.x >> 6;
  if ((threadIdx.x & 63) == 0) { red[0][wave] = accum; red[1][wave] = valid; }
  __syncthreads();
  if (threadIdx.x == 0) {
    const float a = (red[0][0] + red[0][1]) + (red[0][2] + red[0][3]);
    const float vl = (red[1][0] + red[1][1]) + (red[1][2] + red[1][3]);
    const float total = (float)hw * (beta + (1.0f - beta));
    dist[e] = (vl / (total + 1e-8f) < 0.75f) ? 1000.0f : a / vl;
  }
}

__global__ __launch_bounds__(256) void iproj_kernel(
    const float* __restrict__ poses, const float* __restrict__ disps, const float* __restrict__ intr,
    float* __restrict__ points, int hw, int wd) {
  const int p = blockIdx.x * 256 + threadIdx.x;
  const int n = blockIdx.y;
  if (p >= hw) return;
  float t[3], q[4];
  gs_load_pose(poses, n, t, q);
  const float u = (float)(p % wd), v = (float)(p / wd);
  gs_iproj_point(t, q, intr[0], intr[1], intr[2], intr[3], u, v, disps[(size_t)n * hw + p],
                 points + ((size_t)n * hw + p) * 3);
}

__global__ __launch_bounds__(256) void depth_filter_kernel(
    const float* __restrict__ poses, const float* __restrict__ disps, const float* __restrict__ intr,
    const int64_t* __restrict__ inds, const float* __restrict__ thresh, float* __restrict__ counter,
    int num, int hw, int ht, int wd) {
  const int p = blockIdx.x * 256 + threadIdx.x;
  const int b = blockIdx.y;
  if (p >= hw) return;
  counter[(size_t)b * hw + p] = gs_depth_filter_count(poses, disps, (int)inds[b], p, intr[0], intr[1], intr[2],
                                                      intr[3], thresh[b], num, hw, ht, wd);
}

}

#define GS_GEOM_COMMON(name)                                                              \
  GS_REQUIRE(n >= 0 && h > 0 && w > 0, name ": bad shape");                               \
  if (n == 0) return GS_OK;                                                               \
  hipStream_t st = (hipStream_t)stream;                                                   \
  const int hw = h * w;

extern "C" int gs_reproject(const float* poses, const float* disps, const float* intrinsics,
                            const int64_t* ii, const int64_t* jj, float* coords, float* valid, int n, int h,
                            int w, gs_stream_t stream) {
  GS_REQUIRE(poses && disps && intrinsics && ii && jj && coords && valid, "reproject: null pointer");
  GS_GEOM_COMMON("reproject");
  GS_REQUIRE(n <= 65535, "reproject: n=%d exceeds grid.y limit", n);
  reproject_kernel<<<dim3(gs_cdiv(hw, 256), n), 256, 0, st>>>(poses, disps, intrinsics, ii, jj, coords, valid, hw, w);
  GS_CHECK_LAUNCH("reproject");
  return GS_OK;
}

extern "C" int gs_projmap(const float* poses, const float* disps, const float* intrinsics, const int64_t* ii,
                          const int64_t* jj, float* coords, float* valid, int n, int h, int w,
                          gs_stream_t stream) {
  GS_REQUIRE(poses && disps && intrinsics && ii && jj && coords && valid, "projmap: null pointer");
  GS_GEOM_COMMON("projmap");
  GS_REQUIRE(n <= 65535, "projmap: n=%d exceeds grid.y limit", n);
  projmap_kernel<<<dim3(gs_cdiv(hw, 256), n), 256, 0, st>>>(poses, disps, intrinsics, ii, jj, coords, valid, hw, w);
  GS_CHECK_LAUNCH("projmap");
  return GS_OK;
}

extern "C" int gs_frame_distance(const float* poses, const float* disps, const float* intrinsics,
                                 const int64_t* ii, const int64_t* jj, float* dist, int n, int h, int w,
                                 float beta, gs_stream_t stream) {
  GS_REQUIRE(poses && disps && intrinsics && ii && jj && dist, "frame_distance: null pointer");
  GS_GEOM_COMMON("frame_distance");
  frame_distance_kernel<<<n, 256, 0, st>>>(poses, disps, intrinsics, ii, jj, dist, hw, w, beta);
  GS_CHECK_LAUNCH("frame_distance");
  return GS_OK;
}

extern "C" int gs_iproj(const float* poses, const float* disps, const float* intrinsics, float* points, int n,
                        int h, int w, gs_stream_t stream) {
  GS_REQUIRE(poses && disps && intrinsics && points, "iproj: null pointer");
  GS_GEOM_COMMON("iproj");
  GS_REQUIRE(n <= 65535, "iproj: n=%d exceeds grid.y limit", n);
  iproj_kernel<<<dim3(gs_cdiv(hw, 256), n), 256, 0, st>>>(poses, disps, intrinsics, points, hw, w);
  GS_CHECK_LAUNCH("iproj");
  return GS_OK;
}

extern "C" int gs_depth_filter(const float* poses, const float* disps, const float* intrinsics,
                               const int64_t* ix, const float* thresh, float* counter, int n, int num, int h,
                               int w, gs_stream_t stream) {
  GS_REQUIRE(poses && disps && intrinsics && ix && thresh && counter, "depth_filter: null pointer");
  GS_GEOM_COMMON("depth_filter");
  GS_REQUIRE(n <= 65535 && num > 0, "depth_filter: bad n/num");
  depth_filter_kernel<<<dim3(gs_cdiv(hw, 256), n), 256, 0, st>>>(poses, disps, intrinsics, ix, thresh, counter, num, hw, h, w);
  GS_CHECK_LAUNCH("depth_filter");
  return GS_OK;
}
```

go_slam_amd/csrc/gru_gates.hip:

```cpp
#include "common.h"

namespace {

typedef _Float16 half8 __attribute__((ext_vector_type(8)));

__device__ __forceinline__ float sigm(float x) { return gs_sigmoid(x); }

__global__ __launch_bounds__(256) void gru_gate_zr_kernel(const _Float16* __restrict__ zr_pre,
                                                          const float* __restrict__ bias,
                                                          const float* __restrict__ glo,
                                                          const _Float16* __restrict__ inp_pre,
                                                          _Float16* __restrict__ hx,
                                                          _Float16* __restrict__ z_out, int hw, int ldx,
                                                          size_t total ) {
  const size_t t = (size_t)blockIdx.x * 256 + threadIdx.x;
  if (t >= total) return;
  const int c8 = (int)(t & 15);
  const size_t pix = t >> 4;
  const int n = (int)(pix / hw);
  const half8 zp = *reinterpret_cast<const half8*>(zr_pre + pix * 256 + c8 * 8);
  const half8 rp = *reinterpret_cast<const half8*>(zr_pre + pix * 256 + 128 + c8 * 8);
  half8* hp = reinterpret_cast<half8*>(hx + pix * ldx + c8 * 8);
  const half8 net = *hp;
  half8 zi = {0, 0, 0, 0, 0, 0, 0, 0}, ri = zi;
// ... 245 lines not shown
        acc[k] += __shfl_xor(acc[k], 8);
        acc[k] += __shfl_xor(acc[k], 16);
        acc[k] += __shfl_xor(acc[k], 32);
      }
      if (lane < 8) {
        float* dst = partial + blk * 128 + pr * 64 + lane * 8;
        *reinterpret_cast<float4*>(dst) = make_float4(acc[0], acc[1], acc[2], acc[3]);
        *reinterpret_cast<float4*>(dst + 4) = make_float4(acc[4], acc[5], acc[6], acc[7]);
      }
      __builtin_amdgcn_fence(__ATOMIC_RELEASE, "wavefront");
      __builtin_amdgcn_wave_barrier();
    }
  }
}

__global__ __launch_bounds__(384) void glo_heads_kernel(const float* __restrict__ partial, int nchunk, float inv_hw,
                                                        const _Float16* __restrict__ wz, const _Float16* __restrict__ wr,
                                                        const _Float16* __restrict__ wq, const float* __restrict__ bz,
                                                        const float* __restrict__ br, const float* __restrict__ bq,
                                                        float* __restrict__ gzr, float* __restrict__ gq) {
  const int n = blockIdx.x, t = threadIdx.x;
  __shared__ float g[128];
  __shared__ float part3[3][128];
  {
    const int third = t >> 7, ch = t & 127;
    float s = 0.0f;
    for (int c0 = third; c0 < nchunk; c0 += 30) {
      float v[10];
#pragma unroll
      for (int u = 0; u < 10; ++u) {
        const int c = c0 + 3 * u;
        v[u] = c < nchunk ? partial[((size_t)n * nchunk + c) * 128 + ch] : 0.0f;
      }
#pragma unroll
      for (int u = 0; u < 10; ++u)
        if (c0 + 3 * u < nchunk) s += v[u];
    }
    part3[third][ch] = s;
  }
  __syncthreads();
  if (t < 128) g[t] = (float)(_Float16)(((part3[0][t] + part3[1][t]) + part3[2][t]) * inv_hw);
  __syncthreads();
  const int head = t >> 7, o = t & 127;
  const _Float16* w = (head == 0 ? wz : head == 1 ? wr : wq) + (size_t)o * 128;
  float s = (head == 0 ? bz : head == 1 ? br : bq)[o];
#pragma unroll 4
  for (int k8 = 0; k8 < 16; ++k8) {
    const half8 v = *reinterpret_cast<const half8*>(w + k8 * 8);
#pragma unroll
    for (int k = 0; k < 8; ++k) s = fmaf((float)v[k], g[k8 * 8 + k], s);
  }
  s = (float)(_Float16)s;
  if (head < 2) gzr[(size_t)n * 256 + head * 128 + o] = s;
  else gq[(size_t)n * 128 + o] = s;
}
}

extern "C" int gs_bias_act(const void* x, const float* bias, void* y, int rows, int channels, int x_stride,
                           int y_stride, int act, gs_stream_t stream) {
  GS_REQUIRE(x && y, "bias_act: null pointer");
  GS_REQUIRE(rows >= 0 && channels > 0 && channels % 8 == 0, "bias_act: channels must be a multiple of 8");
  GS_REQUIRE(x_stride >= channels && x_stride % 8 == 0, "bias_act: x_stride must be >= channels and a multiple of 8");
  GS_REQUIRE(y_stride >= channels && y_stride % 8 == 0, "bias_act: y_stride must be >= channels and a multiple of 8");
  GS_REQUIRE(act >= 0 && act <= 2, "bias_act: act in {0 none, 1 relu, 2 sigmoid}");
  if (rows == 0) return GS_OK;
  const size_t total = (size_t)rows * (channels / 8);
  const unsigned grid = (unsigned)((total + 255) / 256);
  hipStream_t st = (hipStream_t)stream;
  const _Float16* xi = (const _Float16*)x;
  _Float16* yo = (_Float16*)y;
  const int c8n = channels / 8;
#define GS_BA(A, B) bias_act_kernel<A, B><<<grid, 256, 0, st>>>(xi, bias, yo, c8n, x_stride, y_stride, total)
  if (bias) { if (act == 0) GS_BA(0, true); else if (act == 1) GS_BA(1, true); else GS_BA(2, true); }
  else      { if (act == 0) GS_BA(0, false); else if (act == 1) GS_BA(1, false); else GS_BA(2, false); }
#undef GS_BA
  GS_CHECK_LAUNCH("bias_act");
  return GS_OK;
}

extern "C" int gs_segment_mean(const void* x, int x_stride, const float* in_bias, int in_relu, const int* seg_offsets,
                               const int* seg_edges, void* out, int n_seg, int hw, int channels, gs_stream_t stream) {
  GS_REQUIRE(x && seg_offsets && seg_edges && out, "segment_mean: null pointer");
  GS_REQUIRE(n_seg >= 0 && hw > 0 && channels > 0 && channels % 8 == 0, "segment_mean: channels must be a multiple of 8");
  GS_REQUIRE(x_stride >= channels && x_stride % 8 == 0, "segment_mean: x_stride must be >= channels, multiple of 8");
  if (n_seg == 0) return GS_OK;
  const size_t total = (size_t)n_seg * hw * (channels / 8);
  segment_mean_kernel<<<(unsigned)((total + 255) / 256), 256, 0, (hipStream_t)stream>>>(
      (const _Float16*)x, x_stride, in_bias, in_relu, seg_offsets, seg_edges, (_Float16*)out, hw, channels / 8, total);
  GS_CHECK_LAUNCH("segment_mean");
  return GS_OK;
}

constexpr int GLO_CHUNKS = 32;
extern "C" size_t gs_gru_glo_workspace_bytes(int n) { return (size_t)(n > 0 ? n : 0) * GLO_CHUNKS * 128 * sizeof(float); }

extern "C" int gs_gru_glo(const void* w_pre, const float* w_bias, const void* net, const void* wz, const void* wr,
                          const void* wq, const float* bz, const float* br, const float* bq, float* gzr, float* gq,
                          int n, int hw, void* workspace, size_t workspace_bytes, gs_stream_t stream) {
  GS_REQUIRE(w_pre && w_bias && net && wz && wr && wq && bz && br && bq && gzr && gq, "gru_glo: null pointer");
  GS_REQUIRE(n >= 0 && hw > 0, "gru_glo: bad shape");
  if (n == 0) return GS_OK;
  GS_REQUIRE(workspace && workspace_bytes >= gs_gru_glo_workspace_bytes(n), "gru_glo: workspace too small");
  hipStream_t st = (hipStream_t)stream;
  const int nchunk = GLO_CHUNKS;
  glo_pool_kernel<<<dim3(nchunk, n), 256, 0, st>>>((const _Float16*)w_pre, w_bias, (const _Float16*)net,
                                                   (float*)workspace, hw, nchunk);
  GS_CHECK_LAUNCH("gru_glo pool");
  glo_heads_kernel<<<n, 384, 0, st>>>((const float*)workspace, nchunk, 1.0f / (float)hw, (const _Float16*)wz,
                                      (const _Float16*)wr, (const _Float16*)wq, bz, br, bq, gzr, gq);
  GS_CHECK_LAUNCH("gru_glo heads");
  return GS_OK;
}

extern "C" size_t gs_gru_glo_fused_workspace_bytes(int n, int hw) {
  if (n <= 0 || hw <= 0) return 0;
  return (size_t)n * ((hw + 31) / 32) * 128 * sizeof(float);
}

extern "C" int gs_gru_glo_fused(const void* net, int net_stride, const void* w_pack, const float* w_bias, const void* wz,
                                const void* wr, const void* wq, const float* bz, const float* br, const float* bq,
                                float* gzr, float* gq, int n, int hw, void* workspace, size_t workspace_bytes,
                                gs_stream_t stream) {
  GS_REQUIRE(net && w_pack && w_bias && wz && wr && wq && bz && br && bq && gzr && gq, "gru_glo_fused: null pointer");
  GS_REQUIRE(n >= 0 && hw > 0 && net_stride >= 128 && net_stride % 8 == 0, "gru_glo_fused: bad shape");
  GS_REQUIRE((((size_t)net | (size_t)w_pack) & 15) == 0, "gru_glo_fused: net / w_pack must be 16-byte aligned");
  if (n == 0) return GS_OK;
  GS_REQUIRE(workspace && workspace_bytes >= gs_gru_glo_fused_workspace_bytes(n, hw), "gru_glo_fused: workspace too small");
  hipStream_t st = (hipStream_t)stream;
  const int bpi = (hw + 31) / 32;
  const size_t nblk = (size_t)n * bpi;
  const size_t lds = (size_t)(4 * 8 * 512 + 4 * 32 * 72) * sizeof(_Float16) + 128 * sizeof(float);
  static GsLdsLimit limit;
  if (int rc = limit.raise((const void*)glo_conv_pool_kernel, lds, "gru_glo_fused")) return rc;
  size_t grid = 256 * 3;
  if (grid > (nblk + 3) / 4) grid = (nblk + 3) / 4;
  glo_conv_pool_kernel<<<(unsigned)grid, 256, lds, st>>>((const _Float16*)net, net_stride, (const _Float16*)w_pack, w_bias,
                                                         (float*)workspace, hw, bpi, nblk);
  GS_CHECK_LAUNCH("gru_glo_fused pool");
  glo_heads_kernel<<<n, 384, 0, st>>>((const float*)workspace, bpi, 1.0f / (float)hw, (const _Float16*)wz,
                                      (const _Float16*)wr, (const _Float16*)wq, bz, br, bq, gzr, gq);
  GS_CHECK_LAUNCH("gru_glo_fused heads");
  return GS_OK;
}

namespace {
__global__ __launch_bounds__(256) void motion_features_kernel(const float2* __restrict__ coords1,
                                                              const float2* __restrict__ target,
                                                              _Float16* __restrict__ out, int hw, int w, size_t total) {
  const size_t t = (size_t)blockIdx.x * 256 + threadIdx.x;
  if (t >= total) return;
  const int p = (int)(t % hw);
  const float gx = (float)(p % w), gy = (float)(p / w);
  const float2 c = coords1[t], tg = target[t];
  typedef _Float16 half4m __attribute__((ext_vector_type(4)));
  half4m o;
  o[0] = (_Float16)fminf(fmaxf(c.x - gx, -64.0f), 64.0f);
  o[1] = (_Float16)fminf(fmaxf(c.y - gy, -64.0f), 64.0f);
  o[2] = (_Float16)fminf(fmaxf(tg.x - c.x, -64.0f), 64.0f);
  o[3] = (_Float16)fminf(fmaxf(tg.y - c.y, -64.0f), 64.0f);
  reinterpret_cast<half4m*>(out)[t] = o;
}

__global__ __launch_bounds__(256) void damping_rows_kernel(const float* __restrict__ eta, const int* __restrict__ inv,
                                                           const int64_t* __restrict__ index,
                                                           float* __restrict__ damping_buf, float* __restrict__ out,
                                                           int hw, float scale, float eps, size_t total) {
  const size_t t = (size_t)blockIdx.x * 256 + threadIdx.x;
  if (t >= total) return;
  const int k = (int)(t / hw), p = (int)(t - (size_t)k * hw);
  const int m = inv[k];
  float* slot = damping_buf + (size_t)index[k] * hw + p;
  float v;
  if (m >= 0) { v = eta[(size_t)m * hw + p]; *slot = v; }
  else v = *slot;
  out[t] = scale * v + eps;
}

__global__ __launch_bounds__(256) void ba_inputs_kernel(const float2* __restrict__ coords1, const float2* __restrict__ delta,
                                                        const float2* __restrict__ weight, float2* __restrict__ target,
                                                        float* __restrict__ ba_target, float* __restrict__ ba_weight,
                                                        int hw, size_t total) {
  const size_t t = (size_t)blockIdx.x * 256 + threadIdx.x;
  if (t >= total) return;
  const size_t e = t / hw;
  const int p = (int)(t - e * hw);
  const float2 c = coords1[t], d = delta[t], wt = weight[t];
  const float2 tg = make_float2(c.x + d.x, c.y + d.y);
  target[t] = tg;
  float* bt = ba_target + e * 2 * hw + p;
  bt[0] = tg.x; bt[hw] = tg.y;
  float* bw = ba_weight + e * 2 * hw + p;
  bw[0] = wt.x; bw[hw] = wt.y;
}
}

extern "C" int gs_motion_features(const float* coords1, const float* target, void* out, int n, int h, int w,
                                  gs_stream_t stream) {
  GS_REQUIRE(coords1 && target && out, "motion_features: null pointer");
  GS_REQUIRE(n >= 0 && h > 0 && w > 0, "motion_features: bad shape");
  if (n == 0) return GS_OK;
  const size_t total = (size_t)n * h * w;
  motion_features_kernel<<<(unsigned)((total + 255) / 256), 256, 0, (hipStream_t)stream>>>(
      (const float2*)coords1, (const float2*)target, (_Float16*)out, h * w, w, total);
  GS_CHECK_LAUNCH("motion_features");
  return GS_OK;
}

extern "C" int gs_ba_inputs(const float* coords1, const float* delta, const float* weight, float* target,
                            float* ba_target, float* ba_weight, int n, int h, int w, gs_stream_t stream) {
  GS_REQUIRE(coords1 && delta && weight && target && ba_target && ba_weight, "ba_inputs: null pointer");
  GS_REQUIRE(n >= 0 && h > 0 && w > 0, "ba_inputs: bad shape");
  if (n == 0) return GS_OK;
  const size_t total = (size_t)n * h * w;
  ba_inputs_kernel<<<(unsigned)((total + 255) / 256), 256, 0, (hipStream_t)stream>>>(
      (const float2*)coords1, (const float2*)delta, (const float2*)weight, (float2*)target, ba_target, ba_weight,
      h * w, total);
  GS_CHECK_LAUNCH("ba_inputs");
  return GS_OK;
}

extern "C" int gs_damping_rows(const float* eta, const int* inv, const int64_t* index, float* damping_buf, float* out,
                               int n_rows, int hw, float scale, float eps, gs_stream_t stream) {
  GS_REQUIRE(inv && index && damping_buf && out, "damping_rows: null pointer");
  GS_REQUIRE(n_rows >= 0 && hw > 0, "damping_rows: bad shape");
  if (n_rows == 0) return GS_OK;
  const size_t total = (size_t)n_rows * hw;
  damping_rows_kernel<<<(unsigned)((total + 255) / 256), 256, 0, (hipStream_t)stream>>>(eta, inv, index, damping_buf, out,
                                                                                       hw, scale, eps, total);
  GS_CHECK_LAUNCH("damping_rows");
  return GS_OK;
}
```

go_slam_amd/depth_video.py:

```python
import torch
import torch.multiprocessing as _mp

from . import droid_backends
from .droid_net import cvx_upsample


class DepthVideo:
    def __init__(self, cfg_or_ht, args_or_wd, buffer=512, device="cuda:0", stereo=False, full_res=False):
        if isinstance(cfg_or_ht, int):
            self.cfg, self.args = None, None
            mh, mw = int(cfg_or_ht), int(args_or_wd)
            shared = False
        else:
            cfg, args = cfg_or_ht, args_or_wd
            self.cfg, self.args = cfg, args
            mh, mw = cfg["cam"]["H_out"] // 8, cfg["cam"]["W_out"] // 8
            buffer, device = cfg["tracking"]["buffer"], args.device
            stereo = (cfg["mode"] == "stereo")
            full_res, shared = True, True
        self.device = torch.device(device)
        self.scale_factor = 8
        self.map_ht, self.map_wd = mh, mw
        self.ht, self.wd = (cfg["cam"]["H_out"], cfg["cam"]["W_out"]) if self.cfg is not None else (8 * mh, 8 * mw)
        self.stereo = stereo
# ... 56 lines not shown
    def _count(self):
        return int(self._counter.value)

    def _set_count(self, n):
        self._counter.value = int(n)

    def __setitem__(self, index, item):
        n = self._count()
        if isinstance(index, int) and index >= n:
            self._set_count(index + 1)
        elif torch.is_tensor(index) and int(index.max()) > n:
            self._set_count(int(index.max()) + 1)
        self.timestamp[index] = item[0]
        if hasattr(self, "images"):
            self.images[index] = item[1]
        pose, disp, depth = item[2], item[3], item[4]
        if pose is not None:
            self.poses[index] = pose
        if disp is not None:
            self.disps[index] = disp
        if depth is not None:
            if hasattr(self, "depths_gt"):
                self.depths_gt[index] = depth
            sub = depth[..., 3::8, 3::8].to(self.device)
            self.disps_sens[index] = torch.where(sub > 0, 1.0 / sub, sub)
            self.disps[index] = self.disps_sens[index].clone()
        for slot, name in ((5, "intrinsics"), (6, "fmaps"), (7, "nets"), (8, "inps")):
            if len(item) > slot and (slot > 5 or item[slot] is not None):
                getattr(self, name)[index] = item[slot]
        if len(item) > 6:
            self._run_write_hooks(index)
        if len(item) > 9 and item[9] is not None and hasattr(self, "poses_gt"):
            self.poses_gt[index] = item[9].to(self.poses_gt.device)

    def add_write_hook(self, fn):
        import weakref
        hooks = self.__dict__.setdefault("_write_hooks", [])
        hooks.append(weakref.WeakMethod(fn) if hasattr(fn, "__self__") else (lambda f=fn: f))

    def __getstate__(self):
        state = dict(self.__dict__)
        state.pop("_write_hooks", None)
        return state

    def _run_write_hooks(self, index):
        hooks = self.__dict__.get("_write_hooks")
        if hooks:
            live = []
            for h in hooks:
                fn = h()
                if fn is not None:
                    fn(index)
                    live.append(h)
            self._write_hooks = live

    def __getitem__(self, index):
        if isinstance(index, int) and index > 0:
            index = self._count() + index
        return (self.poses[index], self.disps[index], self.intrinsics[index], self.fmaps[index], self.nets[index],
                self.inps[index])

    def append(self, *item):
        self[self._count()] = item

    def get_bound(self):
        with self.mapping.get_lock():
            return self.bound[0]

    def get_mapping_item(self, index, device="cuda:0", decay=0.1):
        from .lietorch_shim import SE3
        with self.mapping.get_lock():
            image = self.images[index].permute(1, 2, 0).contiguous().to(device)
            mask = self.mask_filtered[index].clone().to(device)
            depth = 1.0 / (self.disps_filtered[index].to(device) + 1e-7)
            w2c = SE3(self.poses_filtered[index].clone()).to(device)
            c2w = (SE3(self.pose_compensate[0].clone()).to(device) * w2c.inv()).matrix()
            gt_c2w = self.poses_gt[index].clone().to(device)
            self.update_priority[index] *= decay
            self._finish_locked_section()
        return image, depth, c2w, gt_c2w, mask

    def get_mapping_items(self, indices, device="cuda:0", decay=0.1):
        from .lietorch_shim import SE3
        order = list(indices)
        uniq = list(dict.fromkeys(order))
        if not uniq:
            return {}
        t = torch.as_tensor(uniq, dtype=torch.long, device=self.images.device)
        count = {}
        for i in order:
            count[i] = count.get(i, 0) + 1
        with self.mapping.get_lock():
            images = self.images[t].permute(0, 2, 3, 1).contiguous().to(device)
            masks = self.mask_filtered[t].clone().to(device)
            depths = 1.0 / (self.disps_filtered[t].to(device) + 1e-7)
            w2c = SE3(self.poses_filtered[t].clone()).to(device)
            c2w = (SE3(self.pose_compensate[0:1].clone()).to(device) * w2c.inv()).matrix()
            gt = self.poses_gt[t].clone().to(device)
            for k in range(max(count.values())):
                sel = [i for i in uniq if count[i] > k]
                self.update_priority[torch.as_tensor(sel, dtype=torch.long, device=self.update_priority.device)] *= decay
            self._finish_locked_section()
        return {i: (images[j], depths[j], c2w[j], gt[j], masks[j]) for j, i in enumerate(uniq)}

    def normalize(self):
        with self.get_lock():
            n = self._count()
            s = self.disps[:n].mean()
            self.disps[:n] /= s
            self.poses[:n, :3] *= s
            self.dirty[:n] = True
            self._finish_locked_section()

    def _finish_locked_section(self):
        if self._shared and self.device.type == "cuda":
            torch.cuda.current_stream(self.device).synchronize()

    @staticmethod
    def format_indices(ii, jj, device="cuda"):
        if not isinstance(ii, torch.Tensor):
            ii = torch.as_tensor(ii)
        if not isinstance(jj, torch.Tensor):
            jj = torch.as_tensor(jj)
        return (ii.to(device=device, dtype=torch.long).reshape(-1).contiguous(),
                jj.to(device=device, dtype=torch.long).reshape(-1).contiguous())

    def upsample(self, ix, mask):
        if hasattr(mask, "upsample_into"):
            ix = ix.to(device=self.device, dtype=torch.long).contiguous()
            if self.disps.is_cuda and self.disps.is_contiguous() and self.disps_up.is_contiguous():
                mask.upsample_into(self.disps, ix, self.disps_up)
                return
            mask = mask.materialize()
        m = mask.reshape(-1, 576, self.map_ht, self.map_wd)
        if m.dtype == torch.float16 and m.is_cuda:
            cl = m.is_contiguous(memory_format=torch.channels_last)
            if not cl:
                m = m.contiguous()
            ix = ix.to(device=self.device, dtype=torch.long).contiguous()
            from . import _lib
            with torch.cuda.device(self.device):
                rc = _lib.lib().gs_cvx_upsample(_lib.ptr(self.disps), _lib.ptr(m), _lib.ptr(ix),
                                                _lib.ptr(self.disps_up), ix.numel(), self.map_ht, self.map_wd, int(cl),
                                                _lib.stream_ptr(self.device))
            _lib.check(rc, "DepthVideo.upsample")
            return
        up = cvx_upsample(self.disps[ix].unsqueeze(-1), mask)
        self.disps_up[ix] = up.squeeze(-1).float()

    def reproject(self, ii, jj):
        ii, jj = DepthVideo.format_indices(ii, jj, self.device)
        return droid_backends.reproject(self.poses, self.disps, self.intrinsics, ii, jj)

    def distance(self, ii=None, jj=None, beta=0.3, bidirectional=True):
        return_matrix = False
        N = self._count()
        if ii is None:
            return_matrix = True
            ii, jj = torch.meshgrid(torch.arange(N), torch.arange(N), indexing="ij")
        ii, jj = DepthVideo.format_indices(ii, jj, self.device)
        intr = self.intrinsics[0].contiguous()
        if bidirectional:
            poses = self.poses[:N].clone()
            d1 = droid_backends.frame_distance(poses, self.disps, intr, ii, jj, beta)
            d2 = droid_backends.frame_distance(poses, self.disps, intr, jj, ii, beta)
            d = 0.5 * (d1 + d2)
        else:
            d = droid_backends.frame_distance(self.poses, self.disps, intr, ii, jj, beta)
        return d.reshape(N, N) if return_matrix else d

    ba_accepts_tables = True

    def ba(self, target, weight, eta, ii, jj, t0=1, t1=None, iters=2, lm=1e-4, ep=0.1,
           motion_only=False, ba_type=None, tables=None):
        lock = self.get_lock() if ba_type is None else self.get_ba_lock(ba_type)
        with lock:
            if t1 is None:
                t1 = max(int(ii.max()), int(jj.max())) + 1
            out = droid_backends.ba(self.poses, self.disps, self.intrinsics[0].contiguous(), self.disps_sens,
                                    target, weight, eta, ii, jj, t0, t1, iters, lm, ep, motion_only, tables=tables)
            self.disps.clamp_(min=0.001)
            self._finish_locked_section()
        return out
```

go_slam_amd/droid_backends.py:

```python
import os

import torch

from . import _lib

_DT = {torch.float16: 0, torch.float32: 1, torch.float64: 2}

_ws_cache = {}
_ba_status = {}
BA_CHECK = os.environ.get("GOSLAM_BA_CHECK", "0") == "1"


def _chk(name, t, dtype=None):
    if not isinstance(t, torch.Tensor):
        raise RuntimeError(f"{name} must be a tensor")
    if not t.is_cuda:
        raise RuntimeError(f"{name} must be a GPU tensor (go_slam_amd has no CPU path)")
    if not t.is_contiguous():
        raise RuntimeError(f"{name} must be contiguous")
    if dtype is not None and t.dtype != dtype:
        raise RuntimeError(f"{name} must have dtype {dtype}, got {t.dtype}")
    return t


# ... 49 lines not shown
        rc = L.gs_ba_ex(_lib.ptr(poses), _lib.ptr(disps), _lib.ptr(intrinsics), _lib.ptr(disps_sens),
                        _lib.ptr(targets), _lib.ptr(weights), _lib.ptr(eta), _lib.ptr(ii), _lib.ptr(jj),
                        int(t0), int(t1), int(iterations), float(lm), float(ep), int(bool(motion_only)),
                        E, M, nbuf, ht, wd, _lib.ptr(dx), _lib.ptr(dz), _lib.ptr(status),
                        _lib.ptr(ws), ws.numel(), flags, _lib.stream_ptr(dev))
    _lib.check(rc, "droid_backends.ba")
    if new_key is not None:
        tables["key"] = new_key
        tables["ii"], tables["jj"] = ii, jj
    if BA_CHECK:
        st = ba_status(dev)
        if st["depth_rows_mismatch"]:
            raise RuntimeError(f"droid_backends.ba: eta has {M} rows but the graph has {st['depth_keyframes']} depth "
                               "keyframes (unique(arange(t0, t1) U ii))")
    return [dx, dz]


def ba_status(device=None):
    dev = torch.device("cuda", torch.cuda.current_device()) if device is None else torch.device(device)
    status = _ba_status.get(dev.index if dev.index is not None else torch.cuda.current_device())
    if status is None:
        return None
    s = status.tolist()
    return {"depth_keyframes": s[0], "depth_rows_mismatch": bool(s[1]), "cholesky_failures": s[2]}


def frame_distance(poses, disps, intrinsics, ii, jj, beta):
    _chk("poses", poses, torch.float32)
    _chk("disps", disps, torch.float32)
    _chk("intrinsics", intrinsics, torch.float32)
    _chk("ii", ii, torch.int64)
    _chk("jj", jj, torch.int64)
    n = ii.shape[0]
    _, ht, wd = disps.shape
    dist = torch.empty(n, dtype=torch.float32, device=poses.device)
    with torch.cuda.device(poses.device):
        rc = _lib.lib().gs_frame_distance(_lib.ptr(poses), _lib.ptr(disps), _lib.ptr(intrinsics), _lib.ptr(ii),
                                          _lib.ptr(jj), _lib.ptr(dist), n, ht, wd, float(beta),
                                          _lib.stream_ptr(poses.device))
    _lib.check(rc, "droid_backends.frame_distance")
    return dist


def projmap(poses, disps, intrinsics, ii, jj):
    _chk("poses", poses, torch.float32)
    _chk("disps", disps, torch.float32)
    _chk("intrinsics", intrinsics, torch.float32)
    _chk("ii", ii, torch.int64)
    _chk("jj", jj, torch.int64)
    n = ii.shape[0]
    _, ht, wd = disps.shape
    coords = torch.empty(n, ht, wd, 3, dtype=torch.float32, device=poses.device)
    valid = torch.empty(n, ht, wd, 1, dtype=torch.float32, device=poses.device)
    with torch.cuda.device(poses.device):
        rc = _lib.lib().gs_projmap(_lib.ptr(poses), _lib.ptr(disps), _lib.ptr(intrinsics), _lib.ptr(ii),
                                   _lib.ptr(jj), _lib.ptr(coords), _lib.ptr(valid), n, ht, wd,
                                   _lib.stream_ptr(poses.device))
    _lib.check(rc, "droid_backends.projmap")
    return [coords, valid]


def depth_filter(poses, disps, intrinsics, ix, thresh):
    _chk("poses", poses, torch.float32)
    _chk("disps", disps, torch.float32)
    _chk("intrinsics", intrinsics, torch.float32)
    _chk("ix", ix, torch.int64)
    _chk("thresh", thresh, torch.float32)
    num, ht, wd = disps.shape
    n = ix.shape[0]
    counter = torch.empty(n, ht, wd, dtype=torch.float32, device=disps.device)
    with torch.cuda.device(disps.device):
        rc = _lib.lib().gs_depth_filter(_lib.ptr(poses), _lib.ptr(disps), _lib.ptr(intrinsics), _lib.ptr(ix),
                                        _lib.ptr(thresh), _lib.ptr(counter), n, num, ht, wd,
                                        _lib.stream_ptr(disps.device))
    _lib.check(rc, "droid_backends.depth_filter")
    return counter


def iproj(poses, disps, intrinsics):
    _chk("poses", poses, torch.float32)
    _chk("disps", disps, torch.float32)
    _chk("intrinsics", intrinsics, torch.float32)
    n, ht, wd = disps.shape
    points = torch.empty(n, ht, wd, 3, dtype=torch.float32, device=disps.device)
    with torch.cuda.device(disps.device):
        rc = _lib.lib().gs_iproj(_lib.ptr(poses), _lib.ptr(disps), _lib.ptr(intrinsics), _lib.ptr(points),
                                 n, ht, wd, _lib.stream_ptr(disps.device))
    _lib.check(rc, "droid_backends.iproj")
    return points


def corr_index_forward(volume, coords, radius):
    _chk("volume", volume)
    _chk("coords", coords, torch.float32)
    if volume.dtype not in _DT:
        raise RuntimeError(f"corr_index_forward: unsupported dtype {volume.dtype}")
    n, h1, w1, h2, w2 = volume.shape
    rd = 2 * radius + 1
    corr = torch.empty(n, rd, rd, h1, w1, dtype=volume.dtype, device=volume.device)
    with torch.cuda.device(volume.device):
        rc = _lib.lib().gs_corr_index_forward(_lib.ptr(volume), _lib.ptr(coords), _lib.ptr(corr), n, h1, w1, h2,
                                              w2, int(radius), _DT[volume.dtype],
                                              _lib.stream_ptr(volume.device))
    _lib.check(rc, "droid_backends.corr_index_forward")
    return [corr]


def corr_index_backward(volume, coords, corr_grad, radius):
    _chk("volume", volume)
    _chk("coords", coords, torch.float32)
    _chk("corr_grad", corr_grad, volume.dtype)
    n, h1, w1, h2, w2 = volume.shape
    grad = torch.zeros_like(volume)
    with torch.cuda.device(volume.device):
        rc = _lib.lib().gs_corr_index_backward(_lib.ptr(coords), _lib.ptr(corr_grad), _lib.ptr(grad), n, h1, w1,
                                               h2, w2, int(radius), _DT[volume.dtype],
                                               _lib.stream_ptr(volume.device))
    _lib.check(rc, "droid_backends.corr_index_backward")
    return [grad]


CORR_ROWMAJOR, CORR_TILE8 = 0, 1


def corr_lookup_pyramid(pyramid, coords, radius=3, channels_last=False, layout=CORR_ROWMAJOR, map_size=None):
    assert len(pyramid) == 4
    for i, v in enumerate(pyramid):
        _chk(f"pyramid[{i}]", v, pyramid[0].dtype)
    _chk("coords", coords, torch.float32)
    if layout == CORR_TILE8:
        n, h1, w1 = pyramid[0].shape[:3]
        h2, w2 = map_size
        for l in range(4):
            want = (n, h1, w1, _lib.lib().gs_corr_level_elems(h2, w2, l, layout)) if l < 2 else (n, h1, w1, h2 >> l, w2 >> l)
            if tuple(pyramid[l].shape) != want:
                raise RuntimeError(f"tile8 pyramid level {l} has shape {tuple(pyramid[l].shape)}, expected {want}")
    else:
        n, h1, w1, h2, w2 = pyramid[0].shape
        for l in range(4):
            if tuple(pyramid[l].shape) != (n, h1, w1, h2 >> l, w2 >> l):
                raise RuntimeError(f"pyramid level {l} has shape {tuple(pyramid[l].shape)}")
    rd = 2 * radius + 1
    corr = torch.empty((n, 4 * rd * rd, h1, w1), dtype=pyramid[0].dtype, device=coords.device,
                       memory_format=torch.channels_last if channels_last else torch.contiguous_format)
    with torch.cuda.device(coords.device):
        rc = _lib.lib().gs_corr_lookup_pyramid(_lib.ptr(pyramid[0]), _lib.ptr(pyramid[1]), _lib.ptr(pyramid[2]),
                                               _lib.ptr(pyramid[3]), _lib.ptr(coords), _lib.ptr(corr), n, h1, w1,
                                               h2, w2, int(radius), _DT[pyramid[0].dtype], int(bool(channels_last)),
                                               int(layout), _lib.stream_ptr(coords.device))
    _lib.check(rc, "corr_lookup_pyramid")
    return corr


def reproject(poses, disps, intrinsics, ii, jj):
    _chk("poses", poses, torch.float32)
    _chk("disps", disps, torch.float32)
    _chk("intrinsics", intrinsics, torch.float32)
    _chk("ii", ii, torch.int64)
    _chk("jj", jj, torch.int64)
    n = ii.shape[0]
    _, ht, wd = disps.shape
    coords = torch.empty(1, n, ht, wd, 2, dtype=torch.float32, device=poses.device)
    valid = torch.empty(1, n, ht, wd, 1, dtype=torch.float32, device=poses.device)
    with torch.cuda.device(poses.device):
        rc = _lib.lib().gs_reproject(_lib.ptr(poses), _lib.ptr(disps), _lib.ptr(intrinsics), _lib.ptr(ii),
                                     _lib.ptr(jj), _lib.ptr(coords), _lib.ptr(valid), n, ht, wd,
                                     _lib.stream_ptr(poses.device))
    _lib.check(rc, "reproject")
    return coords, valid


def altcorr_forward(fmap1, fmap2, coords, radius):
    _chk("fmap1", fmap1)
    _chk("fmap2", fmap2, fmap1.dtype)
    _chk("coords", coords, torch.float32)
    if fmap1.dtype not in (torch.float16, torch.float32):
        raise RuntimeError(f"altcorr_forward: unsupported dtype {fmap1.dtype}")
    B, H1, W1, C = fmap1.shape
    _, H2, W2, _ = fmap2.shape
    S = coords.shape[1]
    rd = 2 * radius + 1
    corr = torch.empty(B, S, rd * rd, H1, W1, dtype=fmap1.dtype, device=fmap1.device)
    with torch.cuda.device(fmap1.device):
        rc = _lib.lib().gs_altcorr_forward(_lib.ptr(fmap1), _lib.ptr(fmap2), _lib.ptr(coords), _lib.ptr(corr), B, S,
                                           H1, W1, H2, W2, C, int(radius), _DT[fmap1.dtype],
                                           _lib.stream_ptr(fmap1.device))
    _lib.check(rc, "droid_backends.altcorr_forward")
    return [corr]


def altcorr_backward(fmap1, fmap2, coords, corr_grad, radius):
    for name, t in (("fmap1", fmap1), ("fmap2", fmap2), ("coords", coords), ("corr_grad", corr_grad)):
        _chk(name, t, torch.float32)
    B, H1, W1, C = fmap1.shape
    _, H2, W2, _ = fmap2.shape
    S = coords.shape[1]
    g1 = torch.empty_like(fmap1)
    g2 = torch.zeros_like(fmap2)
    gc = torch.zeros_like(coords)
    with torch.cuda.device(fmap1.device):
        rc = _lib.lib().gs_altcorr_backward(_lib.ptr(fmap1), _lib.ptr(fmap2), _lib.ptr(coords), _lib.ptr(corr_grad),
                                            _lib.ptr(g1), _lib.ptr(g2), B, S, H1, W1, H2, W2, C, int(radius),
                                            _lib.stream_ptr(fmap1.device))
    _lib.check(rc, "droid_backends.altcorr_backward")
    return [g1, g2, gc]


CORR_VOLUME_MAX_W = 96


def corr_volume_supported(fmap1):
    n, dim, h, w = fmap1.shape
    return fmap1.dtype == torch.float16 and dim == 128 and h >= 8 and w % 4 == 0 and 8 <= w <= CORR_VOLUME_MAX_W


def corr_tile8_supported(fmap):
    return corr_volume_supported(fmap) and fmap.shape[-1] % 16 == 0


def corr_untile8(vol, hl, wl):
    n, h, w, plane = vol.shape
    nty, ntx = (hl + 7) // 8, (wl + 7) // 8
    t = vol.view(n, h, w, nty, ntx, 8, 8).permute(0, 1, 2, 3, 5, 4, 6).reshape(n, h, w, nty * 8, ntx * 8)
    return t[..., :hl, :wl].contiguous()


def corr_volume_pyramid(fmap1, fmap2, layout=CORR_ROWMAJOR):
    _chk("fmap1", fmap1, torch.float16)
    _chk("fmap2", fmap2, torch.float16)
    if fmap1.shape != fmap2.shape or not corr_volume_supported(fmap1):
        raise RuntimeError(f"corr_volume_pyramid: unsupported shape {tuple(fmap1.shape)} / {tuple(fmap2.shape)}")
    n, dim, h, w = fmap1.shape
    dev = fmap1.device
    L = _lib.lib()
    if layout == CORR_TILE8:
        if not corr_tile8_supported(fmap1):
            raise RuntimeError(f"corr_volume_pyramid: tile8 layout needs w % 16 == 0, got {tuple(fmap1.shape)}")
        vols = [torch.empty(n, h, w, L.gs_corr_level_elems(h, w, l, layout), dtype=torch.float16, device=dev)
                for l in range(2)]
        vols += [torch.empty(n, h, w, h >> l, w >> l, dtype=torch.float16, device=dev) for l in (2, 3)]
    else:
        vols = [torch.empty(n, h, w, h >> l, w >> l, dtype=torch.float16, device=dev) for l in range(4)]
    need = L.gs_corr_volume_workspace_bytes(n, dim, h, w)
    ws = _workspace(dev, need + 256)
    with torch.cuda.device(dev):
        rc = L.gs_corr_volume_pyramid(_lib.ptr(fmap1), _lib.ptr(fmap2), *[_lib.ptr(v) for v in vols], n, dim, h, w,
                                      int(layout), _lib.ptr(ws), ws.numel(), _lib.stream_ptr(dev))
    _lib.check(rc, "corr_volume_pyramid")
    return vols
```

go_slam_amd/factor_graph.py:

```python
import numpy as np
import torch

from .corr import AltCorrBlock, CorrBlock, CorrPool

def coords_grid(ht, wd, device):
    y, x = torch.meshgrid(torch.arange(ht, device=device).float(), torch.arange(wd, device=device).float(),
                          indexing="ij")
    return torch.stack([x, y], dim=-1)


def _segments_np(index):
    uniq, ix = np.unique(index, return_inverse=True)
    ix = ix.reshape(-1).astype(np.int64)
    order = np.argsort(ix, kind="stable").astype(np.int32)
    offsets = np.zeros(uniq.size + 1, dtype=np.int32)
    offsets[1:] = np.cumsum(np.bincount(ix, minlength=uniq.size))
    return {"uniq": uniq.astype(np.int64), "ix": ix, "offsets": offsets, "order": order, "n": int(uniq.size)}


def _as_tensors(d):
    return {k: (torch.from_numpy(np.ascontiguousarray(v)) if isinstance(v, np.ndarray) else v) for k, v in d.items()}


def upload_tables(host, device):
    out = dict(host)
    if torch.device(device).type == "cpu":
        return out
    groups = {}
    for k, v in host.items():
        if torch.is_tensor(v):
            groups.setdefault(v.dtype, []).append(k)
    for dt, keys in groups.items():
        per16 = max(1, 16 // torch.empty(0, dtype=dt).element_size())
        pieces, spans, off = [], [], 0
        for k in keys:
            n = host[k].numel()
            pad = (-n) % per16
            pieces.append(host[k].reshape(-1))
            if pad:
                pieces.append(torch.zeros(pad, dtype=dt))
            spans.append((k, off, n))
            off += n + pad
        flat = torch.cat(pieces).to(device) if off else torch.zeros(0, dtype=dt, device=device)
        for k, o, n in spans:
            out[k] = flat[o:o + n].view(host[k].shape)
    return out


class FactorGraph:
    def __init__(self, video, update_op, device="cuda:0", corr_impl="volume", max_factors=-1, upsample=False,
                 channels_last=True):
        assert corr_impl in ("volume", "alt")
        self.channels_last = channels_last
        self.pool_volumes = True
        self.video = video
        self.update_op = update_op
        self.device = torch.device(device)
        self.max_factors = max_factors
        self.corr_impl = corr_impl
        self.upsample = upsample
        self.ht, self.wd = (int(x) for x in video.disps.shape[-2:])
        self.coords0 = coords_grid(self.ht, self.wd, self.device)
        z = lambda *s: torch.zeros(*s, device=self.device)
        self.ii = torch.zeros(0, dtype=torch.long, device=self.device)
        self.jj = torch.zeros(0, dtype=torch.long, device=self.device)
        self.age = torch.zeros(0, dtype=torch.long, device=self.device)
        self.corr, self.net, self.inp = None, None, None
        self.damping = 1e-6 * torch.ones_like(video.disps)
        self.target = z(1, 0, self.ht, self.wd, 2)
        self.weight = z(1, 0, self.ht, self.wd, 2)
        self.ii_inac = torch.zeros(0, dtype=torch.long, device=self.device)
        self.jj_inac = torch.zeros(0, dtype=torch.long, device=self.device)
        self.ii_bad = torch.zeros(0, dtype=torch.long, device=self.device)
        self.jj_bad = torch.zeros(0, dtype=torch.long, device=self.device)
        self.target_inac = z(1, 0, self.ht, self.wd, 2)
        self.weight_inac = z(1, 0, self.ht, self.wd, 2)

    def _edge_index(self, t0, t1, use_inactive):
        tens = (self.ii, self.jj, self.ii_inac, self.jj_inac)
        key = tuple(x._version for x in tens) + (t0, t1, bool(use_inactive))
        c = getattr(self, "_eidx", None)
        if c is not None and c["key"] == key and all(a is b for a, b in zip(c["tens"], tens)):
            return c
        dev = self.device
        E, Ei = self.ii.numel(), self.ii_inac.numel()
        host = torch.cat([self.ii, self.jj, self.ii_inac, self.jj_inac]).cpu().numpy()
        ii_c, jj_c = host[:E], host[E:2 * E]
        a0 = max(1, int(ii_c.min()) + 1) if t0 is None else t0
        a0 = max(1, a0)
        a1 = (max(int(ii_c.max()), int(jj_c.max())) + 1) if t1 is None else t1
        seg_h = _segments_np(ii_c)
        c = {"key": key, "tens": tens, "t0": a0, "t1": a1, "seg": None, "sel": None, "ii_min": int(ii_c.min())}
        up = {"seg." + k: v for k, v in seg_h.items() if isinstance(v, np.ndarray)}
        ii_all = ii_c
        if use_inactive:
            iin, jin = host[2 * E:2 * E + Ei], host[2 * E + Ei:]
            m = (iin >= a0 - 3) & (jin >= a0 - 3)
            up["sel"] = np.nonzero(m)[0].astype(np.int64)
            ii_all = np.concatenate([iin[m], ii_c])
            up["ii"] = ii_all
            up["jj"] = np.concatenate([jin[m], jj_c])
        else:
            c["ii"], c["jj"] = self.ii.contiguous(), self.jj.contiguous()
        dindex = np.unique(np.concatenate([np.arange(a0, a1, dtype=np.int64), ii_all]))
        up["damping_index"] = dindex
        uniq = seg_h["uniq"]
        if uniq.size:
            pos = np.minimum(np.searchsorted(uniq, dindex), uniq.size - 1)
            inv = np.where(uniq[pos] == dindex, pos, -1)
        else:
            inv = np.full(dindex.shape, -1)
        up["damping_inv"] = inv.astype(np.int32)
        up = upload_tables(_as_tensors(up), dev)
        c["seg"] = {k: (up["seg." + k] if isinstance(v, np.ndarray) else v) for k, v in seg_h.items()}
        for k in ("sel", "ii", "jj", "damping_index", "damping_inv"):
            if k in up:
                c[k] = up[k]
        uniq = torch.from_numpy(uniq)
        c["uniq_host"] = uniq
        self._eidx = c
        return c

    def _glue_fusable(self, coords1):
        return coords1.is_cuda and self.channels_last and self.target.dtype == torch.float32 \
            and self.target.is_contiguous() and coords1.is_contiguous()

    def _ba_buffers(self, idx, use_inactive):
        if "ba_target" not in idx:
            ht, wd = self.ht, self.wd
            E = self.ii.numel()
            if use_inactive and idx["sel"].numel():
                ti = self.target_inac[0, idx["sel"]].permute(0, 3, 1, 2)
                wi = self.weight_inac[0, idx["sel"]].permute(0, 3, 1, 2)
            else:
                ti = wi = torch.zeros(0, 2, ht, wd, device=self.device)
            n_in = ti.shape[0]
            bt = torch.empty(n_in + E, 2, ht, wd, device=self.device)
            bw = torch.empty(n_in + E, 2, ht, wd, device=self.device)
            bt[:n_in], bw[:n_in] = ti, wi
            idx["ba_target"], idx["ba_weight"], idx["n_inactive"] = bt, bw, n_in
        return idx["ba_target"], idx["ba_weight"], idx["n_inactive"]

    @torch.no_grad()
    def add_factors(self, ii, jj, remove=False):
        ii = torch.as_tensor(ii, dtype=torch.long, device=self.device).reshape(-1)
        jj = torch.as_tensor(jj, dtype=torch.long, device=self.device).reshape(-1)
        ii, jj = self._filter_repeated_edges(ii, jj)
        if ii.numel() == 0:
            return
        if self.max_factors > 0 and self.ii.numel() + ii.numel() > self.max_factors and self.corr is not None \
                and remove:
            perm = torch.argsort(self.age, descending=False)
            self.rm_factors(perm >= self.max_factors - ii.numel(), store=True)
        net = self._fmt(self.video.nets[ii]).unsqueeze(0)
        if self.corr_impl == "volume":
            c = (ii == jj).long()
            fmap1 = self.video.fmaps[ii, 0].unsqueeze(0)
            fmap2 = self.video.fmaps[jj, c].unsqueeze(0)
            if self.corr is None and self.pool_volumes and CorrPool.supported(fmap1, self.channels_last):
                self.corr = CorrPool(self.ht, self.wd, self.device, capacity=max(self.max_factors, 48) + 32)
            if isinstance(self.corr, CorrPool):
                self.corr.append(fmap1, fmap2)
            else:
                corr = CorrBlock(fmap1, fmap2, channels_last=self.channels_last)
                self.corr = corr if self.corr is None else self.corr.cat(corr)
            inp = self._fmt(self.video.inps[ii]).unsqueeze(0)
            self.inp = inp if self.inp is None else self._cat_edges(self.inp, inp)
        with torch.autocast("cuda", enabled=False):
            target, _ = self.video.reproject(ii, jj)
            weight = torch.zeros_like(target)
        self.ii = torch.cat([self.ii, ii])
        self.jj = torch.cat([self.jj, jj])
        self.age = torch.cat([self.age, torch.zeros_like(ii)])
        self.net = net if self.net is None else self._cat_edges(self.net, net)
        self.target = torch.cat([self.target, target], 1)
        self.weight = torch.cat([self.weight, weight], 1)

    def _fmt(self, x4):
        return x4.contiguous(memory_format=torch.channels_last) if self.channels_last else x4.contiguous()

    def _cat_edges(self, a5, b5):
        return self._fmt(torch.cat([a5[0], b5[0]], 0)).unsqueeze(0)

    @torch.no_grad()
    def rm_factors(self, mask, store=False):
        mask = mask.to(device=self.device, dtype=torch.bool).reshape(-1)
        if mask.is_cuda:
            order = torch.argsort(mask.to(torch.uint8), stable=True)
            n_keep = mask.numel() - int(mask.sum())
            keep, gone = order[:n_keep], order[n_keep:]
        else:
            keep, gone = torch.nonzero(~mask).reshape(-1), torch.nonzero(mask).reshape(-1)
        if gone.numel() == 0:
            return
        if store:
            self.ii_inac = torch.cat([self.ii_inac, self.ii.index_select(0, gone)])
            self.jj_inac = torch.cat([self.jj_inac, self.jj.index_select(0, gone)])
            self.target_inac = torch.cat([self.target_inac, self.target.index_select(1, gone)], 1)
            self.weight_inac = torch.cat([self.weight_inac, self.weight.index_select(1, gone)], 1)
        self.ii, self.jj, self.age = (x.index_select(0, keep) for x in (self.ii, self.jj, self.age))
        if self.corr_impl == "volume" and self.corr is not None:
            self.corr = self.corr[keep]
        if self.inp is not None:
            self.inp = self._select_edges(self.inp, keep)
        if self.net is not None:
            self.net = self._select_edges(self.net, keep)
        self.target = self.target.index_select(1, keep)
        self.weight = self.weight.index_select(1, keep)

    @staticmethod
    def _edges_on_host(*pairs):
        out = []
        for a, b in pairs:
            out += list(zip(a.cpu().tolist(), b.cpu().tolist()))
        return out

    def _filter_repeated_edges(self, ii, jj):
        if ii.numel() == 0 or self.ii.numel() + self.ii_inac.numel() == 0:
            return ii, jj
        if ii.is_cuda:
            have = torch.cat([self.ii, self.ii_inac]) * (1 << 20) + torch.cat([self.jj, self.jj_inac])
            keep = torch.nonzero(~torch.isin(ii * (1 << 20) + jj, have)).reshape(-1)
            if keep.numel() == ii.numel():
                return ii, jj
            return ii.index_select(0, keep), jj.index_select(0, keep)
        have = set(self._edges_on_host((self.ii, self.jj), (self.ii_inac, self.jj_inac)))
        keep = torch.tensor([e not in have for e in zip(ii.cpu().tolist(), jj.cpu().tolist())],
                            dtype=torch.bool, device=ii.device)
        return ii[keep], jj[keep]

    @torch.no_grad()
    def filter_edges(self):
        conf = self.weight.mean(dim=(0, 2, 3, 4))
        mask = ((self.ii - self.jj).abs() > 2) & (conf < 1e-3)
        self.ii_bad = torch.cat([self.ii_bad, self.ii[mask]])
        self.jj_bad = torch.cat([self.jj_bad, self.jj[mask]])
        self.rm_factors(mask, store=False)

    @torch.no_grad()
    def clear_edges(self):
        if self.ii.numel():
            if self.corr_impl == "volume" and self.corr is not None:
                self.corr = self.corr[torch.zeros(0, dtype=torch.long, device=self.ii.device)]
            self.ii, self.jj, self.age = (x.new_empty((0,)) for x in (self.ii, self.jj, self.age))
            self.target, self.weight = (x.new_empty((x.shape[0], 0) + tuple(x.shape[2:])) for x in (self.target, self.weight))
        self.net = None
        self.inp = None

    _KEYFRAME_BUFFERS = ("timestamp", "images", "dirty", "red", "poses", "poses_gt", "disps", "disps_sens",
                         "disps_up", "depths_gt", "intrinsics", "poses_filtered", "disps_filtered",
                         "mask_filtered", "update_priority", "nets", "inps", "fmaps")

    @torch.no_grad()
    def rm_keyframe(self, ix):
        v = self.video
        for name in self._KEYFRAME_BUFFERS:
            buf = getattr(v, name, None)
            if torch.is_tensor(buf):
                buf[ix] = buf[ix + 1]
        m = (self.ii_inac == ix) | (self.jj_inac == ix)
        self.ii_inac = self.ii_inac - (self.ii_inac >= ix).long()
        self.jj_inac = self.jj_inac - (self.jj_inac >= ix).long()
        if bool(m.any()):
            keep = ~m
            self.ii_inac, self.jj_inac = self.ii_inac[keep], self.jj_inac[keep]
            self.target_inac, self.weight_inac = self.target_inac[:, keep], self.weight_inac[:, keep]
        m = (self.ii == ix) | (self.jj == ix)
        self.ii = self.ii - (self.ii >= ix).long()
        self.jj = self.jj - (self.jj >= ix).long()
        self.rm_factors(m, store=False)

    def add_neighborhood_factors(self, t0, t1, r=3):
        ii, jj = torch.meshgrid(torch.arange(t0, t1), torch.arange(t0, t1), indexing="ij")
        ii, jj = ii.reshape(-1), jj.reshape(-1)
        c = 1 if getattr(self.video, "stereo", False) else 0
        keep = ((ii - jj).abs() > c) & ((ii - jj).abs() <= r)
        self.add_factors(ii[keep].to(self.device), jj[keep].to(self.device))

    @staticmethod
    def propose_proximity_edges(d, existing, t0, t1, t, rad, nms, thresh, max_factors, stereo):
        import numpy as np
        ilen, jlen = t - t0, t - t1

        def suppress(di, dj):
            d[max(0, di - nms):min(ilen, di + nms + 1), max(0, dj - nms):min(jlen, dj + nms + 1)] = np.inf

        for i, j in existing:
            if t0 <= i < t and t1 <= j < t:
                d[i - t0, j - t1] = np.inf
                suppress(i - t0, j - t1)
        es = []
        for i in range(t0, t):
            if stereo:
                es.append((i, i))
                d[i - t0, i - t1] = np.inf
            for j in range(max(i - rad, 0), i):
                es += [(i, j), (j, i)]
                d[i - t0, j - t1] = np.inf
                suppress(i - t0, j - t1)
        flat = d.reshape(-1)
        order = np.argsort(flat, kind="stable")
        order = order[flat[order] <= thresh]
        for k in order.tolist():
            di, dj = k // jlen, k % jlen
            if d[di, dj] > thresh:
                continue
            if len(es) > max_factors:
                break
            i, j = t0 + di, t1 + dj
            es += [(i, j), (j, i)]
            suppress(di, dj)
        return es

    @staticmethod
    def propose_edges_on_device(raw, existing, i0, j0, t, rad, nms, cut, thresh, max_factors, stereo, jmin, loop):
        from . import _lib
        dev = raw.device
        n_local = sum((1 if stereo else 0) + 2 * max(i - max(i - rad, jmin), 0) for i in range(i0, t))
        cap = n_local + max(int(max_factors), 0) + 16
        raw = raw.detach().float().contiguous()
        d_work = torch.empty_like(raw)
        es = torch.zeros(cap, 2, dtype=torch.long, device=dev)
        count = torch.zeros(1, dtype=torch.int32, device=dev)
        ex_i, ex_j = (None, None) if existing is None else (existing[0].long().contiguous(), existing[1].long().contiguous())
        n_ex = 0 if existing is None else int(ex_i.numel())
        L, st = _lib.lib(), _lib.stream_ptr(dev)
        with torch.cuda.device(dev):
            _lib.check(L.gs_edge_prep(_lib.ptr(raw), _lib.ptr(d_work), _lib.ptr(ex_i), _lib.ptr(ex_j), n_ex, _lib.ptr(es),
                                      _lib.ptr(count), cap, i0, j0, t, rad, nms, float(cut), int(bool(stereo)), jmin, st),
                       "edge_prep")
            vals, order = torch.sort(d_work, stable=True)
            _lib.check(L.gs_edge_greedy(_lib.ptr(raw), _lib.ptr(vals), _lib.ptr(order), _lib.ptr(es), _lib.ptr(count), cap,
                                        i0, j0, t, nms, float(thresh), int(max_factors), int(bool(loop)), st),
                       "edge_greedy")
        return es[:int(count)]

    @torch.no_grad()
    def add_proximity_factors(self, t0=0, t1=0, rad=2, nms=2, beta=0.25, thresh=16.0, remove=False, max_t=None):
        cnt = self.video.counter
        t = max_t if max_t is not None else int(getattr(cnt, "value", cnt))
        if t <= t0 or t <= t1:
            return
        vdev = torch.device(self.device)
        ii, jj = torch.meshgrid(torch.arange(t0, t, device=vdev), torch.arange(t1, t, device=vdev), indexing="ij")
        ii, jj = ii.reshape(-1), jj.reshape(-1)
        d_dev = self.video.distance(ii, jj, beta=beta)
        if d_dev.is_cuda and (t - t0) * (t - t1) <= 512 * 512:
            existing = (torch.cat([self.ii, self.ii_bad, self.ii_inac]), torch.cat([self.jj, self.jj_bad, self.jj_inac]))
            e = FactorGraph.propose_edges_on_device(d_dev, existing, t0, t1, t, rad, nms, 100.0, thresh, self.max_factors,
                                                    bool(getattr(self.video, "stereo", False)), 0, False)
            if e.shape[0]:
                self.add_factors(e[:, 0].contiguous(), e[:, 1].contiguous(), remove)
            return
        d = d_dev.detach().float().cpu()
        ii, jj = ii.cpu(), jj.cpu()
        d[ii - rad < jj] = float("inf")
        d[d > 100] = float("inf")
        d = d.reshape(t - t0, t - t1).numpy().copy()
        existing = self._edges_on_host((self.ii, self.jj), (self.ii_bad, self.jj_bad), (self.ii_inac, self.jj_inac))
        es = FactorGraph.propose_proximity_edges(d, existing, t0, t1, t, rad, nms, thresh, self.max_factors,
                                                 bool(getattr(self.video, "stereo", False)))
        if not es:
            return
        e = torch.tensor(es, dtype=torch.long, device=self.device)
        self.add_factors(e[:, 0], e[:, 1], remove)

    @torch.no_grad()
    def update(self, t0=None, t1=None, iters=2, use_inactive=False, EPS=1e-7, motion_only=False):
        idx = self._edge_index(t0, t1, use_inactive)
        t0, t1, seg = idx["t0"], idx["t1"], idx["seg"]
        coords1, mask = self.video.reproject(self.ii, self.jj)
        fused = self._glue_fusable(coords1)
        ht, wd = self.ht, self.wd
        E = self.ii.numel()
        if fused:
            from . import _lib
            L, st = _lib.lib(), _lib.stream_ptr(self.device)
            m4 = torch.empty(E, ht, wd, 4, dtype=torch.float16, device=self.device)
            _lib.check(L.gs_motion_features(_lib.ptr(coords1), _lib.ptr(self.target), _lib.ptr(m4), E, ht, wd, st),
                       "motion_features")
            motion = m4.permute(0, 3, 1, 2).unsqueeze(0)
        else:
            motion = torch.cat([coords1 - self.coords0, self.target - coords1], dim=-1)
            motion = motion.permute(0, 1, 4, 2, 3).clamp(-64.0, 64.0)

        corr = self.corr.lazy(coords1) if hasattr(self.corr, "lazy") else self.corr(coords1)
        with torch.autocast("cuda", dtype=torch.float16):
            self.net, delta, weight, damping, upmask = self.update_op(
                self.net, self.inp, corr, motion, self.ii, self.jj, seg=seg)

        fuse_damping = fused and damping.dtype == torch.float32 and damping.is_contiguous() and \
            self.damping.is_contiguous() and damping.shape[1] == idx["uniq_host"].numel()
        if not fuse_damping:
            self.damping[seg["uniq"]] = damping.float()
        eta_rows = damping
        if fused and delta.dtype == torch.float32 and weight.dtype == torch.float32:
            bt, bw, n_in = self._ba_buffers(idx, use_inactive)
            target_new = torch.empty_like(coords1)
            _lib.check(L.gs_ba_inputs(_lib.ptr(coords1), _lib.ptr(delta.contiguous()), _lib.ptr(weight.contiguous()),
                                      _lib.ptr(target_new), bt[n_in:].data_ptr(), bw[n_in:].data_ptr(), E, ht, wd, st),
                       "ba_inputs")
            self.target, self.weight = target_new, weight
            target, weight = bt, bw
        else:
            self.target = coords1 + delta.float()
            self.weight = weight.float()
            if use_inactive:
                sel = idx["sel"]
                target = torch.cat([self.target_inac[:, sel], self.target], 1)
                weight = torch.cat([self.weight_inac[:, sel], self.weight], 1)
            else:
                target, weight = self.target, self.weight
            target = target.view(-1, ht, wd, 2).permute(0, 3, 1, 2).contiguous()
            weight = weight.view(-1, ht, wd, 2).permute(0, 3, 1, 2).contiguous()

        if fuse_damping:
            damping = torch.empty(idx["damping_index"].numel(), ht, wd, device=self.device)
            _lib.check(L.gs_damping_rows(_lib.ptr(eta_rows), _lib.ptr(idx["damping_inv"]), _lib.ptr(idx["damping_index"]),
                                         _lib.ptr(self.damping), _lib.ptr(damping), damping.shape[0], ht * wd, 0.2,
                                         float(EPS), st), "damping_rows")
        else:
            damping = 0.2 * self.damping[idx["damping_index"]].contiguous() + EPS

        tables = idx.setdefault("ba_tables", {}) if getattr(self.video, "ba_accepts_tables", False) else None
        if tables is None:
            self.video.ba(target, weight, damping, idx["ii"], idx["jj"], t0=t0, t1=t1, iters=iters,
                          lm=1e-4, ep=0.1, motion_only=motion_only)
        else:
            self.video.ba(target, weight, damping, idx["ii"], idx["jj"], t0=t0, t1=t1, iters=iters,
                          lm=1e-4, ep=0.1, motion_only=motion_only, tables=tables)
        if self.upsample:
            self.video.upsample(seg["uniq"], upmask[0])
        self.age += 1

    def _select_edges(self, x5, sel):
        x4 = x5[0]
        if self.channels_last and x4.is_contiguous(memory_format=torch.channels_last):
            return x4.permute(0, 2, 3, 1).index_select(0, sel).permute(0, 3, 1, 2).unsqueeze(0)
        return x4.index_select(0, sel).unsqueeze(0)

    def _lowmem_index(self, t0, t1, rig):
        tens = (self.ii, self.jj)
        key = tuple(x._version for x in tens) + (t0, t1, rig, getattr(getattr(self.video, "inps", None), "_version", 0))
        c = getattr(self, "_lidx", None)
        if c is not None and c["key"] == key and all(a is b for a, b in zip(c["tens"], tens)):
            return c
        dev = self.device
        host = torch.stack([self.ii, self.jj]).cpu().numpy()
        ii_c, jj_c = host[0], host[1]
        a0 = max(1, int(ii_c.min()) + 1) if t0 is None else t0
        a0 = max(1, a0)
        a1 = (max(int(ii_c.max()), int(jj_c.max())) + 1) if t1 is None else t1
        chunks, up, segs = [], {}, []
        s = 13
        for i in range(int(ii_c.min()), int(ii_c.max()) + 1, s):
            sel = np.nonzero((ii_c >= i) & (ii_c < i + s))[0].astype(np.int64)
            if sel.size < 1:
                continue
            iis, jjs = ii_c[sel], jj_c[sel]
            n = len(segs)
            up.update({f"{n}.sel": sel, f"{n}.ii": iis, f"{n}.jj": jjs, f"{n}.corr_ii": rig * iis,
                       f"{n}.corr_jj": rig * jjs + (iis == jjs).astype(np.int64), f"{n}.uniq": np.unique(iis)})
            segs.append(_segments_np(iis))
            up.update({f"{n}.seg.{k}": v for k, v in segs[-1].items() if isinstance(v, np.ndarray)})
        up["damping_index"] = np.unique(np.concatenate([np.arange(a0, a1, dtype=np.int64), ii_c]))
        up = _as_tensors(up)
        up = upload_tables(up, dev)
        for n, seg_h in enumerate(segs):
            ck = {k: up[f"{n}.{k}"] for k in ("sel", "ii", "jj", "corr_ii", "corr_jj", "uniq")}
            seg = {k: (up[f"{n}.seg.{k}"] if isinstance(v, np.ndarray) else v) for k, v in seg_h.items()}
            ck["seg_kw"] = {"seg": seg} if getattr(self.update_op, "_forward_fast", None) is not None else {}
            def _inp(ix=ck["ii"], box=ck):
                v = box.get("inp_cached")
                if v is None:
                    v = box["inp_cached"] = self._fmt(self.video.inps[ix]).unsqueeze(0)
                return v
            ck["inp"] = _inp
            chunks.append(ck)
        c = {"key": key, "tens": tens, "t0": a0, "t1": a1, "chunks": chunks, "ii": self.ii.contiguous(),
             "jj": self.jj.contiguous(), "damping_index": up["damping_index"]}
        self._lidx = c
        return c

    @torch.no_grad()
    def update_lowmem(self, t0=None, t1=None, iters=2, use_inactive=False, EPS=1e-7, steps=8, max_t=None,
                      ba_type="dense", motion_only=False):
        cur_t = self.video.counter
        cur_t = int(getattr(cur_t, "value", cur_t))
        t = max_t if max_t is not None else cur_t
        fm = self.video.fmaps[:cur_t + 2]
        num, rig, ch, ht, wd = fm.shape
        corr_op = AltCorrBlock(fm.reshape(1, num * rig, ch, ht, wd))
        lookup = getattr(corr_op, "lookup", corr_op)
        idx = self._lowmem_index(t0, t1, rig)
        t0, t1 = idx["t0"], idx["t1"]
        ii_all, jj_all = idx["ii"], idx["jj"]
        cl = torch.channels_last
        for _ in range(steps):
            coords1, mask = self.video.reproject(ii_all, jj_all)
            fast = (coords1.is_cuda and self.channels_last and coords1.dtype == torch.float32 and coords1.is_contiguous()
                    and self.target.dtype == torch.float32 and self.target.is_contiguous()
                    and self.weight.dtype == torch.float32 and self.weight.is_contiguous()
                    and self.net.dtype == torch.float16 and self.net[0].is_contiguous(memory_format=cl)
                    and self.net.shape[2] == 128
                    and tuple(self.target.shape) == tuple(coords1.shape) == tuple(self.weight.shape))
            if fast:
                from . import _lib
                L, st = _lib.lib(), _lib.stream_ptr(self.device)
                ht, wd = self.ht, self.wd
            else:
                motion = torch.cat([coords1 - self.coords0, self.target - coords1], dim=-1)
                motion = motion.permute(0, 1, 4, 2, 3).clamp(-64.0, 64.0)
            for ck in idx["chunks"]:
                sel, iis, jjs = ck["sel"], ck["ii"], ck["jj"]
                if fast:
                    n = sel.numel()
                    c1 = torch.empty(1, n, ht, wd, 2, dtype=torch.float32, device=self.device)
                    m4 = torch.empty(n, ht, wd, 4, dtype=torch.float16, device=self.device)
                    net_c = torch.empty(n, ht, wd, 128, dtype=torch.float16, device=self.device)
                    _lib.check(L.gs_lowmem_gather(_lib.ptr(coords1), _lib.ptr(self.target), _lib.ptr(self.net),
                                                  _lib.ptr(sel), _lib.ptr(c1), _lib.ptr(m4), _lib.ptr(net_c), n, ht, wd, st),
                               "lowmem_gather")
                    net_in = net_c.permute(0, 3, 1, 2).unsqueeze(0)
                    motion_c = m4.permute(0, 3, 1, 2).unsqueeze(0)
                else:
                    c1 = coords1.index_select(1, sel)
                    net_in, motion_c = self._select_edges(self.net, sel), motion.index_select(1, sel)
                corr1 = lookup(c1, ck["corr_ii"], ck["corr_jj"])
                with torch.autocast("cuda", dtype=torch.float16):
                    net, delta, weight, damping, upmask = self.update_op(
                        net_in, ck["inp"](), corr1, motion_c, iis, jjs, **ck["seg_kw"])
                    if self.upsample:
                        self.video.upsample(ck["uniq"], upmask[0])
                if fast and net.dtype == torch.float16 and net[0].is_contiguous(memory_format=cl) \
                        and tuple(net.shape) == (1, sel.numel(), 128, ht, wd) \
                        and delta.dtype == torch.float32 and weight.dtype == torch.float32 \
                        and tuple(delta.shape) == tuple(weight.shape) == (1, sel.numel(), ht, wd, 2):
                    delta_c, weight_c = delta.contiguous(), weight.contiguous()
                    _lib.check(L.gs_lowmem_scatter(_lib.ptr(c1), _lib.ptr(delta_c), _lib.ptr(weight_c),
                                                   _lib.ptr(net), _lib.ptr(sel), _lib.ptr(self.target), _lib.ptr(self.weight),
                                                   _lib.ptr(self.net), sel.numel(), ht, wd, st), "lowmem_scatter")
                else:
                    self.net[:, sel] = net.to(self.net.dtype)
                    self.target[:, sel] = c1 + delta.float()
                    self.weight[:, sel] = weight.float()
                self.damping[ck["uniq"]] = damping.float()
            damping = 0.2 * self.damping[idx["damping_index"]].contiguous() + EPS
            target = self.target.view(-1, self.ht, self.wd, 2).permute(0, 3, 1, 2).contiguous()
            weight = self.weight.view(-1, self.ht, self.wd, 2).permute(0, 3, 1, 2).contiguous()
            lm, ep = (1e-4, 1e-1) if ba_type == "loop" else (1e-5, 1e-2)
            kw = {"tables": idx.setdefault("ba_tables", {})} if getattr(self.video, "ba_accepts_tables", False) else {}
            self.video.ba(target, weight, damping, ii_all, jj_all, t0=t0, t1=t1,
                          iters=iters, lm=lm, ep=ep, motion_only=motion_only, ba_type=ba_type, **kw)
            self.video.dirty[:t] = True
```

go_slam_amd/synth.py:

```python
import math

import torch

SHAPES = {
    "S480": (60, 80, 640.0),
    "Rep": (40, 80, 640.0),
    "Scan": (30, 40, 320.0),
    "tiny": (12, 16, 128.0),
}


def _quat_mul(a, b):
    ax, ay, az, aw = a.unbind(-1)
    bx, by, bz, bw = b.unbind(-1)
    return torch.stack([
        aw * bx + ax * bw + ay * bz - az * by,
        aw * by + ay * bw + az * bx - ax * bz,
        aw * bz + az * bw + ax * by - ay * bx,
        aw * bw - ax * bx - ay * by - az * bz,
    ], dim=-1)


def make_intrinsics(shape="S480"):
    ht, wd, w_out = SHAPES[shape]
    s = (w_out / 640.0) / 8.0
    return torch.tensor([577.590698 * s, 578.729797 * s, 318.905426 * s, 242.683609 * s],
                        dtype=torch.float32)


def make_video(num_kf, shape="S480", seed=43, rgbd=True, buffer=None):
    g = torch.Generator().manual_seed(seed)
    ht, wd, _ = SHAPES[shape]
    B = buffer or num_kf
    poses = torch.zeros(B, 7)
    poses[:, 6] = 1.0
    t = torch.zeros(3)
    q = torch.tensor([0.0, 0.0, 0.0, 1.0])
    for k in range(num_kf):
        if k > 0:
            t = t + torch.randn(3, generator=g) * 0.05
            ang = torch.randn(3, generator=g) * math.radians(2.0)
            th = ang.norm().clamp(min=1e-8)
            dq = torch.cat([torch.sin(th / 2) * ang / th, torch.cos(th / 2)[None]])
            q = _quat_mul(dq, q)
            q = q / q.norm()
        poses[k, :3] = t
        poses[k, 3:] = q
    depth = 1.0 + 3.0 * torch.rand(B, 1, ht, wd, generator=g)
    depth = torch.nn.functional.avg_pool2d(torch.nn.functional.pad(depth, (1, 1, 1, 1), mode="replicate"), 3, 1)
    disps = (1.0 / depth[:, 0]).contiguous()
    if rgbd:
        disps_sens = disps + 0.01 * torch.randn(B, ht, wd, generator=g)
        disps_sens = disps_sens.clamp(min=0.05)
        disps_sens = torch.where(torch.rand(B, ht, wd, generator=g) < 0.05,
                                 torch.zeros_like(disps_sens), disps_sens)
    else:
        disps_sens = torch.zeros(B, ht, wd)
    intr = make_intrinsics(shape)[None].repeat(B, 1)
    return dict(poses=poses, disps=disps, disps_sens=disps_sens.contiguous(), intrinsics=intr.contiguous())


def make_graph(num_kf, num_edges, seed=43, radius=2):
    g = torch.Generator().manual_seed(seed + 1)
    pairs = []
    for i in range(num_kf):
        for j in range(num_kf):
            if i != j and abs(i - j) <= radius:
                pairs.append((i, j))
    have = set(pairs)
    pairs = pairs[:num_edges]
    have = set(pairs)
    guard = 0
    while len(pairs) < num_edges and guard < 100000:
        guard += 1
        i = int(torch.randint(0, num_kf, (1,), generator=g))
        j = int(torch.randint(0, num_kf, (1,), generator=g))
        if i != j and (i, j) not in have:
            have.add((i, j))
            pairs.append((i, j))
    ii = torch.tensor([p[0] for p in pairs], dtype=torch.int64)
    jj = torch.tensor([p[1] for p in pairs], dtype=torch.int64)
    return ii, jj


def make_ba_problem(num_kf=8, num_edges=20, shape="tiny", seed=43, rgbd=True, noise_px=0.5, coords=None):
    g = torch.Generator().manual_seed(seed + 2)
    vid = make_video(num_kf, shape, seed, rgbd)
    ii, jj = make_graph(num_kf, num_edges, seed)
    ht, wd, _ = SHAPES[shape]
    E = len(ii)
    if coords is None:
        v, u = torch.meshgrid(torch.arange(ht, dtype=torch.float32), torch.arange(wd, dtype=torch.float32),
                              indexing="ij")
        coords = torch.stack([u, v], dim=-1)[None].repeat(E, 1, 1, 1)
    target = coords + noise_px * torch.randn(E, ht, wd, 2, generator=g)
    target = target.permute(0, 3, 1, 2).contiguous()
    weight = torch.rand(E, 2, ht, wd, generator=g)
    t0, t1 = 1, num_kf
    kx = torch.unique(torch.cat([torch.arange(t0, t1), ii]))
    eta = 1e-2 * torch.rand(len(kx), ht, wd, generator=g) + 1e-4
    vid.update(dict(ii=ii, jj=jj, target=target, weight=weight, eta=eta, t0=t0, t1=t1))
    return vid


def make_features(num, shape="S480", seed=43, dim=128, dtype=torch.float16):
    g = torch.Generator().manual_seed(seed + 3)
    ht, wd, _ = SHAPES[shape]
    return torch.randn(num, dim, ht, wd, generator=g).to(dtype)


def make_altcorr_chunk(seed=211):
    ht, wd, _ = SHAPES["Scan"]
    g = torch.Generator().manual_seed(seed)
    fm = (torch.randn(1, 5, 128, ht, wd, generator=g) * 1.5).half()
    ii = torch.tensor([0, 1, 2, 4, 3, 1, 0, 2, 4])
    jj = torch.tensor([1, 0, 4, 2, 3, 3, 4, 0, 1])
    ys, xs = torch.meshgrid(torch.arange(ht, dtype=torch.float32), torch.arange(wd, dtype=torch.float32), indexing="ij")
    coords = []
    for e in range(9):
        a = 1.0 + 0.15 * (torch.rand(4, generator=g) - 0.5)
        t = 4.0 * torch.randn(2, generator=g)
        x = a[0] * xs + 0.05 * (a[1] - 1) * ys + t[0] + 0.7 * torch.sin(ys / 5.0 + t[1])
        y = a[2] * ys + 0.05 * (a[3] - 1) * xs + t[1] + 0.7 * torch.cos(xs / 6.0 + t[0])
        c = torch.stack([x, y], -1)
        if e >= 5:
            c = c + 3.0 * torch.randn(ht, wd, 2, generator=g)
        if e == 8:
            c = c * 3.0 - 20.0
        coords.append(c)
    return fm, ii, jj, torch.stack(coords)[None].contiguous()


def plane_disps(poses, intr, ht, wd):
    from .lietorch_shim import SE3
    c2w = SE3(poses.double()).inv().data
    t, q = c2w[:, None, None, :3], c2w[:, None, None, 3:]
    fx, fy, cx, cy = intr.double().tolist()
    v, u = torch.meshgrid(torch.arange(ht, dtype=torch.float64, device=poses.device),
                          torch.arange(wd, dtype=torch.float64, device=poses.device), indexing="ij")
    ray = torch.stack([(u - cx) / fx, (v - cy) / fy, torch.ones_like(u)], -1).expand(poses.shape[0], -1, -1, -1)
    qv, w = q[..., :3].expand_as(ray), q[..., 3:]
    uv = 2.0 * torch.cross(qv, ray, dim=-1)
    ray = ray + w * uv + torch.cross(qv, uv, dim=-1)
    best = torch.full(ray.shape[:-1], float("inf"), dtype=torch.float64, device=poses.device)
    for axis, c in ((2, 4.0), (1, 1.2)):
        z = (c - t[..., axis]) / ray[..., axis]
        best = torch.minimum(best, torch.where(z > 0.1, z, torch.full_like(z, float("inf"))))
    return torch.where(torch.isfinite(best), 1.0 / best, torch.zeros_like(best)).float()


def arc_poses(n, step_m=0.03, step_deg=0.5):
    from .lietorch_shim import SE3
    k = torch.arange(n, dtype=torch.float64)
    yaw = math.radians(step_deg) * k
    pos = torch.stack([step_m * k + 0.05 * torch.sin(0.2 * k), 0.02 * torch.sin(0.13 * k), 0.5 * step_m * k], 1)
    q = torch.stack([torch.zeros(n, dtype=torch.float64), torch.sin(yaw / 2), torch.zeros(n, dtype=torch.float64),
                     torch.cos(yaw / 2)], 1)
    return SE3(torch.cat([pos, q], 1)).inv().data.float()


class PlaneSequence:
# ... 27 lines not shown
```

include/goslam_hip.h:

```cpp
#ifndef GOSLAM_HIP_H
#define GOSLAM_HIP_H

#include <stddef.h>
#include <stdint.h>

#ifdef __cplusplus
extern "C" {
#endif

typedef void* gs_stream_t;

typedef enum {
  GS_OK = 0,
  GS_ERR_INVALID_ARG = -1,
  GS_ERR_WORKSPACE = -2,
  GS_ERR_LAUNCH = -3,
  GS_ERR_UNSUPPORTED = -4
} gs_status;

typedef enum { GS_F16 = 0, GS_F32 = 1, GS_F64 = 2 } gs_dtype;

const char* gs_version(void);
const char* gs_last_error(void);

int gs_timing_begin(gs_stream_t stream);
int gs_timing_end(void);
int gs_timing_read(const char* name, double* total_ms, int* count);
int gs_timing_names(char* buf, int buf_bytes);


int gs_corr_index_forward(const void* volume, const float* coords, void* corr,
                          int n, int h1, int w1, int h2, int w2, int radius, int dtype,
                          gs_stream_t stream);

int gs_corr_index_backward(const float* coords, const void* corr_grad, void* volume_grad,
                           int n, int h1, int w1, int h2, int w2, int radius, int dtype,
                           gs_stream_t stream);

#define GS_CORR_ROWMAJOR 0
#define GS_CORR_TILE8 1
int gs_corr_lookup_pyramid(const void* vol0, const void* vol1, const void* vol2, const void* vol3,
                           const float* coords, void* corr,
                           int n, int h1, int w1, int h2, int w2, int radius, int dtype,
                           int channels_last, int layout, gs_stream_t stream);
int gs_corr_lookup_enc(const void* vol0, const void* vol1, const void* vol2, const void* vol3, const float* coords,
                       const void* wpad, const float* bias, void* y, int y_stride, int n, int h1, int w1, int h2,
                       int w2, int layout, gs_stream_t stream);
int gs_corr_lookup_enc_slots(const void* vol0, const void* vol1, const void* vol2, const void* vol3, const int64_t* slot,
                             const float* coords, const void* wpad, const float* bias, void* y, int y_stride, int n,
                             int h1, int w1, int h2, int w2, int layout, gs_stream_t stream);
int gs_corr_lookup_pyramid_slots(const void* vol0, const void* vol1, const void* vol2, const void* vol3,
                                 const int64_t* slot, const float* coords, void* corr, int n, int h1, int w1, int h2,
                                 int w2, int radius, int dtype, int channels_last, int layout, gs_stream_t stream);

size_t gs_corr_volume_workspace_bytes(int n, int dim, int h, int w);
size_t gs_corr_level_elems(int h, int w, int level, int layout);
int gs_corr_volume_pyramid(const void* fmap1, const void* fmap2, void* vol0, void* vol1, void* vol2,
                           void* vol3, int n, int dim, int h, int w, int layout,
                           void* workspace, size_t workspace_bytes, gs_stream_t stream);
int gs_corr_volume_pyramid_slots(const void* fmap1, const void* fmap2, void* vol0, void* vol1, void* vol2,
                                 void* vol3, const int64_t* out_slot, int n, int dim, int h, int w, int layout,
                                 void* workspace, size_t workspace_bytes, gs_stream_t stream);

int gs_altcorr_forward(const void* fmap1, const void* fmap2, const float* coords, void* corr,
                       int b, int s, int h1, int w1, int h2, int w2, int c, int radius, int dtype,
                       gs_stream_t stream);

int gs_altcorr_backward(const float* fmap1, const float* fmap2, const float* coords, const float* corr_grad,
                        float* fmap1_grad, float* fmap2_grad, int b, int s, int h1, int w1, int h2, int w2,
                        int c, int radius, gs_stream_t stream);

int gs_altcorr_pyramid(const void* pyr0, const void* pyr1, const void* pyr2, const void* pyr3, const float* coords,
                       const int64_t* ii, const int64_t* jj, void* out, int e, int h, int w, int c, int radius,
                       gs_stream_t stream);


int gs_reproject(const float* poses, const float* disps, const float* intrinsics,
                 const int64_t* ii, const int64_t* jj, float* coords, float* valid,
                 int n, int h, int w, gs_stream_t stream);

int gs_projmap(const float* poses, const float* disps, const float* intrinsics,
               const int64_t* ii, const int64_t* jj, float* coords, float* valid,
               int n, int h, int w, gs_stream_t stream);

int gs_frame_distance(const float* poses, const float* disps, const float* intrinsics,
                      const int64_t* ii, const int64_t* jj, float* dist,
                      int n, int h, int w, float beta, gs_stream_t stream);

int gs_iproj(const float* poses, const float* disps, const float* intrinsics, float* points,
             int n, int h, int w, gs_stream_t stream);

int gs_depth_filter(const float* poses, const float* disps, const float* intrinsics,
                    const int64_t* ix, const float* thresh, float* counter,
                    int n, int num, int h, int w, gs_stream_t stream);

size_t gs_pointcloud_workspace_bytes(int k, int h, int w);
int gs_pointcloud_count(const float* poses, const float* disps, const float* intrinsics, const int64_t* index,
                        const float* disp_floor, float thresh, float visible_num, int k, int num, int h, int w,
                        void* workspace, size_t workspace_bytes, gs_stream_t stream);
int gs_pointcloud_mask(const float* mask, const int64_t* index, int k, int num, int h, int w, void* workspace,
                       size_t workspace_bytes, gs_stream_t stream);
int gs_pointcloud_scan(int k, int h, int w, void* workspace, size_t workspace_bytes, long long* offsets,
                       gs_stream_t stream);
int gs_pointcloud_emit(const float* poses_inv, const float* disps, const float* intrinsics, const float* images,
                       const int64_t* index, int k, int num, int h, int w, const void* workspace,
                       size_t workspace_bytes, long long n_points, float* points, float* colors, gs_stream_t stream);

#define GS_TSDF_BATCH 16
int gs_tsdf_batch(void);
int gs_tsdf_integrate(float* tsdf, float* weight, float* colors, int nx, int ny, int nz, const float* depth,
                      const float* mask, const float* images, const float* w2c, int k, int h, int w, float fx, float fy,
                      float cx, float cy, float lo_x, float lo_y, float lo_z, float voxel, float trunc,
                      float max_weight, gs_stream_t stream);
int gs_tsdf_vertex_attr(const float* vertices, int n_vertices, const float* weight, const float* colors, int nx, int ny,
                        int nz, float min_weight, unsigned char* keep, float* rgb, gs_stream_t stream);

size_t gs_tsdf_brick_flags_bytes(int nx, int ny, int nz);
int gs_tsdf_brick_flags(const float* tsdf, int nx, int ny, int nz, unsigned char* flags, gs_stream_t stream);
int gs_tsdf_raycast(const float* tsdf, const float* weight, const float* colors, int nx, int ny, int nz,
                    const unsigned char* flags, const float* c2w, int k, int h, int w, float fx, float fy, float cx,
                    float cy, float lo_x, float lo_y, float lo_z, float voxel, float near, float far, float step_voxels,
                    float min_weight, float* depth, float* normal, float* color, gs_stream_t stream);

#define GS_FRAME_PREP_MAX_VIEWS 32
typedef struct {
  const uint8_t* src;
  const float* map_x;
  const float* map_y;
  uint8_t* tmp;
  float* dst;
  int h, w, c, mh, mw;
} gs_color_view;
typedef struct {
  const uint16_t* src;
  float* dst;
  int h, w;
} gs_depth_view;
int gs_frame_prep_color(const gs_color_view* views_host, int n, int H_out, int W_out, int H_edge, int W_edge,
                        gs_stream_t stream);
int gs_frame_prep_depth(const gs_depth_view* views_host, int n, float scale, int H_out, int W_out, int H_edge,
                        int W_edge, gs_stream_t stream);


int gs_gru_gate_zr(const void* zr_pre, const float* bias_zr, const float* glo_zr, const void* inp_pre, void* hx,
                   void* z_out, int n, int hw, int ldx, gs_stream_t stream);
int gs_gru_gate_q(const void* q_pre, const float* bias_q, const float* glo_q, const void* inp_pre, const void* z,
                  const void* net, void* net_out, int n, int hw, gs_stream_t stream);
int gs_bias_act(const void* x, const float* bias, void* y, int rows, int channels, int x_stride, int y_stride,
                int act, gs_stream_t stream);
int gs_motion_features(const float* coords1, const float* target, void* out, int n, int h, int w,
                       gs_stream_t stream);
int gs_lowmem_gather(const float* coords1, const float* target, const void* net, const int64_t* sel,
                     float* coords_out, void* motion_out, void* net_out, int n_sel, int h, int w, gs_stream_t stream);
int gs_lowmem_scatter(const float* coords, const float* delta, const float* weight, const void* net_new,
                      const int64_t* sel, float* target, float* weight_all, void* net, int n_sel, int h, int w,
                      gs_stream_t stream);

int gs_ba_inputs(const float* coords1, const float* delta, const float* weight, float* target,
                 float* ba_target, float* ba_weight, int n, int h, int w, gs_stream_t stream);
int gs_conv1x1(const void* x, int x_stride, int k_in, const void* wpack, const float* bias, int act, void* y,
               int y_stride, int n_out, long long rows, gs_stream_t stream);
int gs_conv7x7_c4(const void* x, const void* wpack, const float* bias, void* y, int ys, int n, int h, int w, int relu,
                  int rt, gs_stream_t stream);
size_t gs_conv3x3_wpack_elems(int c_in, int n_out);
int gs_conv3x3_pp(const void* x, int x_stride, int c_in, const void* wpack, int tw, void* y, int y_stride, int n_out,
                  int n, int h, int w, int xcd_order, gs_stream_t stream);
int gs_conv3x3_bias_relu(const void* x, int x_stride, int c_in, const void* wpack, const float* bias, void* y,
                         int y_stride, int n_out, int n, int h, int w, gs_stream_t stream);
int gs_conv3x3_gru_zr2(const void* net, const void* x_rest, int x_rest_stride, int c_rest, const void* wpack,
                       const float* bias_zr, const float* glo_zr, const void* inp_pre, void* z_out, void* rnet_out,
                       int n, int h, int w, gs_stream_t stream);
int gs_conv3x3_gru_zr(const void* hx, int hx_stride, int c_in, const void* wpack, const float* bias_zr,
                      const float* glo_zr, const void* inp_pre, void* z_out, void* rnet_out, int n, int h, int w,
                      gs_stream_t stream);
int gs_conv3x3_gru_q(const void* rnet, const void* x_rest, int x_rest_stride, int c_rest, const void* wpack,
                     const float* bias_q, const float* glo_q, const void* inp_pre, const void* z, const void* net,
                     void* net_out, int n, int h, int w, gs_stream_t stream);
int gs_conv3x3_head(const void* x, int x_stride, const float* in_bias, int in_relu, const void* wpack,
                    const float* bias, int n_out, int epilogue, float out_scale, float* out, int n, int h, int w,
                    gs_stream_t stream);
int gs_conv3x3_heads(const void* x, int x_stride, int c_in, const void* wpack, int tw, const void* tap_wpack,
                     const float* in_bias, int n_tap_blocks, float* tap_out, void* y, int y_stride, int n_out, int n,
                     int h, int w, gs_stream_t stream);
int gs_conv3x3_heads_finish(const float* tap, const float* bias0, const float* bias1, int epilogue0, int epilogue1,
                            float out_scale0, float out_scale1, float* out0, float* out1, int n, int h, int w,
                            gs_stream_t stream);
int gs_segment_mean(const void* x, int x_stride, const float* in_bias, int in_relu, const int* seg_offsets,
                    const int* seg_edges, void* out, int n_seg, int hw, int channels, gs_stream_t stream);
size_t gs_norm_act_workspace_bytes(int n, int hw, int channels);
size_t gs_norm_act_workspace_bytes_chunks(int n, int chunks, int channels);
size_t gs_enc_conv_wpack_elems(int ksize, int c_in, int c_out);
int gs_enc_conv_stat_chunks(int h_out, int w_out, int c_out);
int gs_enc_conv(const void* x, int x_stride, int c_in, const void* wpack, const void* bias, void* y, int y_stride,
                int c_out, int ksize, int stride, int n, int h, int w, const void* stat_bias, void* stats_ws,
                gs_stream_t stream);
int gs_norm_act(const void* x, const void* bias, const void* skip, void* y, int n, int hw, int channels,
                int instance_norm, int relu_in, int relu_out, float eps, void* workspace, size_t workspace_bytes,
                int stat_chunks, gs_stream_t stream);
size_t gs_gru_glo_workspace_bytes(int n);
int gs_gru_glo(const void* w_pre, const float* w_bias, const void* net, const void* wz, const void* wr,
               const void* wq, const float* bz, const float* br, const float* bq, float* gzr, float* gq,
               int n, int hw, void* workspace, size_t workspace_bytes, gs_stream_t stream);

size_t gs_gru_glo_fused_workspace_bytes(int n, int hw);
int gs_gru_glo_fused(const void* net, int net_stride, const void* w_pack, const float* w_bias, const void* wz,
                     const void* wr, const void* wq, const float* bz, const float* br, const float* bq, float* gzr,
                     float* gq, int n, int hw, void* workspace, size_t workspace_bytes, gs_stream_t stream);

int gs_damping_rows(const float* eta, const int* inv, const int64_t* index, float* damping_buf, float* out,
                    int n_rows, int hw, float scale, float eps, gs_stream_t stream);

int gs_cvx_upsample(const float* disps, const void* mask, const int64_t* ix, float* out,
                    int m, int h, int w, int mask_channels_last, gs_stream_t stream);
int gs_upmask_upsample(const void* x, int x_stride, const void* weight, const float* bias, const float* disps,
                       const int64_t* ix, float* out, int m, int h, int w, gs_stream_t stream);


size_t gs_ba_workspace_bytes(int n_edges, int n_poses, int n_depth, int nbuf, int hw);

int gs_ba(float* poses, float* disps, const float* intrinsics, const float* disps_sens,
          const float* targets, const float* weights, const float* eta,
          const int64_t* ii, const int64_t* jj,
          int t0, int t1, int iterations, float lm, float ep, int motion_only,
          int n_edges, int n_depth, int nbuf, int h, int w,
          float* dx, float* dz, int32_t* status_out,
          void* workspace, size_t workspace_bytes, gs_stream_t stream);

#define GS_BA_REUSE_TABLES 1
int gs_ba_ex(float* poses, float* disps, const float* intrinsics, const float* disps_sens,
             const float* targets, const float* weights, const float* eta,
             const int64_t* ii, const int64_t* jj,
             int t0, int t1, int iterations, float lm, float ep, int motion_only,
             int n_edges, int n_depth, int nbuf, int h, int w,
             float* dx, float* dz, int32_t* status_out,
             void* workspace, size_t workspace_bytes, int flags, gs_stream_t stream);

int gs_chol_solve(double* H, double* b, int n, float lm, float ep, int path, float* dx, int32_t* status,
                  gs_stream_t stream);

int gs_edge_prep(const float* raw, float* d_work, const long long* ex_i, const long long* ex_j, int n_existing,
                 long long* es, int* count, int cap, int i0, int j0, int t, int rad, int nms, float cut, int stereo,
                 int jmin, gs_stream_t stream);
int gs_edge_greedy(const float* raw, const float* sorted_vals, const long long* order, long long* es, int* count,
                   int cap, int i0, int j0, int t, int nms, float thresh, int max_factors, int loop, gs_stream_t stream);

size_t gs_traj_eval_workspace_bytes(int n);
int gs_traj_world(const float* w2c, const float* compensate, int n, double* tq, double* mat, gs_stream_t stream);
int gs_ape_moments(const double* est, const double* ref, const unsigned char* mask, int n, double* moments,
                   void* workspace, size_t workspace_bytes, gs_stream_t stream);
int gs_ape_stats(const double* est, const double* ref, const unsigned char* mask, const double* sim, int n,
                 double* err, double* stats, void* workspace, size_t workspace_bytes, gs_stream_t stream);

#ifdef __cplusplus
}
#endif
#endif
```

Measured before the change: 82.89 keyframes/s.

## Fuse motion features into reproject, damping into BA inputs, and drop BA memsets

The reprojection kernel now also writes the fp16 motion features, and the BA-input kernel also produces the damping rows. Both save a separate launch and a re-read of the same buffers. The small-path Cholesky kernel now zeroes H and b as it loads them and sets a clean flag, so later iterations skip the per-iteration hipMemsetAsync. The status write also moves into the last update kernel instead of its own launch. This trades launch overhead for more cross-kernel state coupling, which risks stale H if the clean magic is ever wrong.

Result: no change. 83.58 keyframes/s (median of 6 runs) (+0.8%).

```diff
diff --git a/go_slam_amd/_lib.py b/go_slam_amd/_lib.py
--- a/go_slam_amd/_lib.py
+++ b/go_slam_amd/_lib.py
@@ -36,6 +36,7 @@
     "gs_altcorr_forward": (c_int, [_P] * 4 + [c_int] * 9 + [_P]),
     "gs_altcorr_pyramid": (c_int, [_P] * 8 + [c_int] * 5 + [_P]),
     "gs_reproject": (c_int, [_P] * 7 + [c_int] * 3 + [_P]),
+    "gs_reproject_motion": (c_int, [_P] * 10 + [c_int] * 3 + [_P]),
     "gs_projmap": (c_int, [_P] * 7 + [c_int] * 3 + [_P]),
     "gs_frame_distance": (c_int, [_P] * 6 + [c_int] * 3 + [c_float, _P]),
     "gs_iproj": (c_int, [_P] * 4 + [c_int] * 3 + [_P]),
@@ -61,6 +62,7 @@
     "gs_lowmem_gather": (c_int, [_P] * 7 + [c_int, c_int, c_int, _P]),
     "gs_lowmem_scatter": (c_int, [_P] * 8 + [c_int, c_int, c_int, _P]),
     "gs_damping_rows": (c_int, [_P] * 5 + [c_int, c_int, c_float, c_float, _P]),
+    "gs_ba_inputs_damping": (c_int, [_P] * 6 + [c_int] * 3 + [_P] * 5 + [c_int, c_float, c_float, _P]),
     "gs_conv1x1": (c_int, [_P, c_int, c_int, _P, _P, c_int, _P, c_int, c_int, ctypes.c_longlong, _P]),
     "gs_conv7x7_c4": (c_int, [_P, _P, _P, _P, c_int, c_int, c_int, c_int, c_int, c_int, _P]),
     "gs_conv3x3_wpack_elems": (c_size_t, [c_int, c_int]),
diff --git a/go_slam_amd/csrc/ba.hip b/go_slam_amd/csrc/ba.hip
--- a/go_slam_amd/csrc/ba.hip
+++ b/go_slam_amd/csrc/ba.hip
@@ -1,7 +1,8 @@
 #include "common.h"
 
+bool gs_chol_small_path(int n);
 int gs_chol_solve_launch(double* H, double* b, int n, float lm, float ep, float* dx_out, int32_t* fail_flag,
-                         int32_t* fail_count, hipStream_t st);
+                         int32_t* fail_count, int32_t* clean, hipStream_t st);
 
 namespace {
 
@@ -116,6 +117,7 @@
     w.hdr[1] = (M_dev != M_host) ? 1 : 0;
     w.hdr[2] = 0;
     w.hdr[3] = 0;
+    w.hdr[5] = 0;
   }
   __syncthreads();
   for (int m = tid; m < kMaxBuf; m += kPrepThreads) { cnt_a[m] = 0; cnt_b[m] = 0; }
@@ -170,7 +172,10 @@
     const float* __restrict__ eta, const int64_t* __restrict__ jj, int t0, int t1, int hw, int wd,
     int motion_only, int reset_fail, BaWs w) {
   __shared__ float red[4][92];
-  if (reset_fail && blockIdx.x == 0 && blockIdx.y == 0 && blockIdx.z == 0 && threadIdx.x == 0) { w.hdr[2] = 0; w.hdr[3] = 0; }
+  if (blockIdx.x == 0 && blockIdx.y == 0 && blockIdx.z == 0 && threadIdx.x == 0) {
+    w.hdr[5] = 0;
+    if (reset_fail) { w.hdr[2] = 0; w.hdr[3] = 0; }
+  }
   typedef const __attribute__((address_space(4))) int* cip;
   typedef const __attribute__((address_space(4))) int64_t* clp;
   typedef const __attribute__((address_space(4))) float* cfp;
@@ -490,11 +495,12 @@
 
 __global__ __launch_bounds__(256) void ba_update_kernel(
     float* __restrict__ poses, float* __restrict__ disps, const float* __restrict__ dx,
-    float* __restrict__ dz, int M, int t0, int t1, int hw, BaWs w) {
+    float* __restrict__ dz, int M, int t0, int t1, int hw, int32_t* __restrict__ status_out, BaWs w) {
   const int tid = threadIdx.x;
   const int P = t1 - t0;
   if ((int)blockIdx.y == M) {
     if (blockIdx.x != 0) return;
+    if (status_out && tid < 4) status_out[tid] = (tid == 2) ? w.hdr[3] : (tid == 3 ? w.hdr[4] : w.hdr[tid]);
     for (int kk = t0 + tid; kk < t1; kk += 256) {
       float* pp = poses + (size_t)kk * 7;
       float t[3] = {pp[0], pp[1], pp[2]};
@@ -532,6 +538,11 @@
   dz[o] = z;
   const size_t dk = (size_t)w.kx[m] * hw + p;
   disps[dk] = disps[dk] + z;
+}
+
+__global__ __launch_bounds__(256) void ba_clear_unless_clean_kernel(size_t n_doubles, BaWs w) {
+  if (w.hdr[5] == kCholCleanMagic) return;
+  for (size_t i = (size_t)blockIdx.x * 256 + threadIdx.x; i < n_doubles; i += (size_t)gridDim.x * 256) w.H[i] = 0.0;
 }
 
 __global__ void ba_status_kernel(int32_t* status_out, BaWs w) {
@@ -574,10 +585,17 @@
     GS_CHECK_LAUNCH("ba_prep");
   }
   const int chunks = gs_cdiv(hw, 256);
+  const bool small = gs_chol_small_path(n6);
+  const size_t n_sys = (size_t)n6 * n6 + n6;
   for (int it = 0; it < iterations; ++it) {
-    if (hipMemsetAsync(ws.H, 0, ((size_t)n6 * n6 + n6) * sizeof(double), st) != hipSuccess) {
-      gs_set_error("ba: memset failed");
-      return GS_ERR_LAUNCH;
+    if (!small || (it == 0 && !reuse)) {
+      if (hipMemsetAsync(ws.H, 0, n_sys * sizeof(double), st) != hipSuccess) {
+        gs_set_error("ba: memset failed");
+        return GS_ERR_LAUNCH;
+      }
+    } else if (it == 0) {
+      ba_clear_unless_clean_kernel<<<gs_cdiv((int)n_sys, 256 * 8), 256, 0, st>>>(n_sys, ws);
+      GS_CHECK_LAUNCH("ba_clear_unless_clean");
     }
     const int nsp = (!motion_only && n_edges >= 6 * M) ? kAccSplit : 1;
     ba_accum_kernel<<<dim3(chunks, M, nsp), 256, 0, st>>>(poses, disps, intrinsics, disps_sens, targets, weights,
@@ -592,15 +610,16 @@
       ba_schur_kernel<<<2048, 256, 0, st>>>(M, hw, P, ws);
       GS_CHECK_LAUNCH("ba_schur");
     }
-    int rc = gs_chol_solve_launch(ws.H, ws.b, n6, lm, ep, dx, &ws.hdr[2], &ws.hdr[3], st);
+    int rc = gs_chol_solve_launch(ws.H, ws.b, n6, lm, ep, dx, &ws.hdr[2], &ws.hdr[3], small ? &ws.hdr[5] : nullptr, st);
     if (rc != GS_OK) return rc;
+    int32_t* status_it = (it == iterations - 1) ? status_out : nullptr;
     if (motion_only)
-      ba_update_kernel<<<dim3(1, 1), 256, 0, st>>>(poses, disps, dx, dz, 0, t0, t1, hw, ws);
+      ba_update_kernel<<<dim3(1, 1), 256, 0, st>>>(poses, disps, dx, dz, 0, t0, t1, hw, status_it, ws);
     else
-      ba_update_kernel<<<dim3(chunks, M + 1), 256, 0, st>>>(poses, disps, dx, dz, M, t0, t1, hw, ws);
+      ba_update_kernel<<<dim3(chunks, M + 1), 256, 0, st>>>(poses, disps, dx, dz, M, t0, t1, hw, status_it, ws);
     GS_CHECK_LAUNCH("ba_update");
   }
-  if (status_out) {
+  if (status_out && iterations == 0) {
     ba_status_kernel<<<1, 64, 0, st>>>(status_out, ws);
     GS_CHECK_LAUNCH("ba_status");
   }
diff --git a/go_slam_amd/csrc/chol.hip b/go_slam_amd/csrc/chol.hip
--- a/go_slam_amd/csrc/chol.hip
+++ b/go_slam_amd/csrc/chol.hip
@@ -637,6 +637,7 @@
   __syncthreads();
 }
 
+template <bool kZero = false>
 __device__ __forceinline__ void lds_load_packed(double* Lp, const double* __restrict__ H, const double* __restrict__ bg,
                                                 const int n, const int c0, const double lm, const double ep) {
   const int tid = threadIdx.x;
@@ -645,6 +646,7 @@
   for (int base = 0; base < npk; base += SMALL_NT * 4) {
     double v[4];
     int dg[4];
+    size_t off[4];
 #pragma unroll
     for (int u = 0; u < 4; ++u) {
       const int idx = base + u * SMALL_NT + tid;
@@ -653,26 +655,33 @@
       while ((r * (r + 1)) >> 1 > idx) --r;
       const int c = idx - ((r * (r + 1)) >> 1);
       dg[u] = (c == r) ? 1 : 0;
-      v[u] = idx < npk ? H[(size_t)(c0 + r) * n + (c0 + c)] : 0.0;
+      off[u] = (size_t)(c0 + r) * n + (c0 + c);
+      v[u] = idx < npk ? H[off[u]] : 0.0;
     }
 #pragma unroll
     for (int u = 0; u < 4; ++u) {
       const int idx = base + u * SMALL_NT + tid;
       if (idx < npk) Lp[idx] = dg[u] ? v[u] + (ep + lm * v[u]) : v[u];
-    }
-  }
-  for (int i = tid; i <= m; i += SMALL_NT) Lp[npk + i] = (i < m) ? bg[c0 + i] : 0.0;
-}
-
-__global__ __launch_bounds__(SMALL_NT) void chol_small_kernel(const double* __restrict__ H, const double* __restrict__ bg,
-                                                         int n, double lm, double ep, float* __restrict__ dx,
-                                                         int32_t* fail_flag, int32_t* fail_count) {
+      if (kZero && idx < npk) const_cast<double*>(H)[off[u]] = 0.0;
+    }
+  }
+  for (int i = tid; i <= m; i += SMALL_NT) {
+    Lp[npk + i] = (i < m) ? bg[c0 + i] : 0.0;
+    if (kZero && i < m) const_cast<double*>(bg)[c0 + i] = 0.0;
+  }
+}
+
+template <bool kZero>
+__global__ __launch_bounds__(SMALL_NT) void chol_small_kernel(double* H, double* bg, int n, double lm, double ep,
+                                                         float* __restrict__ dx, int32_t* fail_flag,
+                                                         int32_t* fail_count, int32_t* clean) {
   extern __shared__ double sm[];
   double* Lp = sm;
   double* invd = sm + (((n + 1) * (n + 2)) >> 1);
   const int tid = threadIdx.x;
   CHOL_STAMP(0);
-  lds_load_packed(Lp, H, bg, n, 0, lm, ep);
+  lds_load_packed<kZero>(Lp, H, bg, n, 0, lm, ep);
+  if (kZero && tid == 0) *clean = kCholCleanMagic;
   __syncthreads();
   CHOL_STAMP(1);
 
@@ -1042,13 +1051,21 @@
 }
 
 int chol_solve_path(double* H, double* b, int n, float lm, float ep, int path, float* dx_out, int32_t* fail_flag,
-                    int32_t* fail_count, hipStream_t st) {
+                    int32_t* fail_count, int32_t* clean, hipStream_t st) {
   if (path == CHOL_PATH_SMALL) {
     const size_t lds = ((size_t)(n + 1) * (n + 2) / 2 + (size_t)n) * sizeof(double);
-    static GsLdsLimit limit;
     const size_t cap = ((size_t)(SMALL_N + 1) * (SMALL_N + 2) / 2 + SMALL_N) * sizeof(double);
-    if (int rc = limit.raise((const void*)chol_small_kernel, cap, "chol")) return rc;
-    chol_small_kernel<<<1, SMALL_NT, lds, st>>>(H, b, n, (double)lm, (double)ep, dx_out, fail_flag, fail_count);
+    if (clean) {
+      static GsLdsLimit limit;
+      if (int rc = limit.raise((const void*)chol_small_kernel<true>, cap, "chol")) return rc;
+      chol_small_kernel<true><<<1, SMALL_NT, lds, st>>>(H, b, n, (double)lm, (double)ep, dx_out, fail_flag, fail_count,
+                                                        clean);
+    } else {
+      static GsLdsLimit limit;
+      if (int rc = limit.raise((const void*)chol_small_kernel<false>, cap, "chol")) return rc;
+      chol_small_kernel<false><<<1, SMALL_NT, lds, st>>>(H, b, n, (double)lm, (double)ep, dx_out, fail_flag, fail_count,
+                                                         nullptr);
+    }
     GS_CHECK_LAUNCH("chol_small");
     return GS_OK;
   }
@@ -1088,9 +1105,12 @@
 
 }
 
+bool gs_chol_small_path(int n) { return chol_dispatch(n) == CHOL_PATH_SMALL; }
 int gs_chol_solve_launch(double* H, double* b, int n, float lm, float ep, float* dx_out, int32_t* fail_flag,
-                         int32_t* fail_count, hipStream_t st) {
-  return chol_solve_path(H, b, n, lm, ep, chol_dispatch(n), dx_out, fail_flag, fail_count, st);
+                         int32_t* fail_count, int32_t* clean, hipStream_t st) {
+  const int path = chol_dispatch(n);
+  return chol_solve_path(H, b, n, lm, ep, path, dx_out, fail_flag, fail_count, path == CHOL_PATH_SMALL ? clean : nullptr,
+                         st);
 }
 
 extern "C" int gs_chol_solve(double* H, double* b, int n, float lm, float ep, int path, float* dx, int32_t* status,
@@ -1108,5 +1128,5 @@
   }
   GS_REQUIRE(H && b && dx && status, "chol_solve: null pointer");
   if (path == CHOL_PATH_DISPATCH) path = chol_dispatch(n);
-  return chol_solve_path(H, b, n, lm, ep, path, dx, status, status + 1, (hipStream_t)stream);
-}
+  return chol_solve_path(H, b, n, lm, ep, path, dx, status, status + 1, nullptr, (hipStream_t)stream);
+}
diff --git a/go_slam_amd/csrc/common.h b/go_slam_amd/csrc/common.h
--- a/go_slam_amd/csrc/common.h
+++ b/go_slam_amd/csrc/common.h
@@ -37,6 +37,18 @@
       return GS_ERR_LAUNCH;                                                     \
     }                                                                           \
   } while (0)
+
+typedef _Float16 gs_half4 __attribute__((ext_vector_type(4)));
+__device__ __forceinline__ gs_half4 gs_motion4(const float2 c, const float gx, const float gy, const float2 tg) {
+  gs_half4 o;
+  o[0] = (_Float16)fminf(fmaxf(c.x - gx, -64.0f), 64.0f);
+  o[1] = (_Float16)fminf(fmaxf(c.y - gy, -64.0f), 64.0f);
+  o[2] = (_Float16)fminf(fmaxf(tg.x - c.x, -64.0f), 64.0f);
+  o[3] = (_Float16)fminf(fmaxf(tg.y - c.y, -64.0f), 64.0f);
+  return o;
+}
+
+constexpr int32_t kCholCleanMagic = 0x48436c6e;
 
 #include <atomic>
 struct GsLdsLimit {
diff --git a/go_slam_amd/csrc/geom.hip b/go_slam_amd/csrc/geom.hip
--- a/go_slam_amd/csrc/geom.hip
+++ b/go_slam_amd/csrc/geom.hip
@@ -5,10 +5,12 @@
 constexpr float kMinDepthKernel = 0.25f;
 constexpr float kMinDepthPy = 0.2f;
 
+template <bool kMotion>
 __global__ __launch_bounds__(256) void reproject_kernel(
     const float* __restrict__ poses, const float* __restrict__ disps, const float* __restrict__ intr,
     const int64_t* __restrict__ ii, const int64_t* __restrict__ jj, float* __restrict__ coords,
-    float* __restrict__ valid, int hw, int wd) {
+    float* __restrict__ valid, int hw, int wd, const float2* __restrict__ coords0, const float2* __restrict__ target,
+    _Float16* __restrict__ motion) {
   const int p = blockIdx.x * 256 + threadIdx.x;
   const int e = blockIdx.y;
   if (p >= hw) return;
@@ -37,8 +39,13 @@
   gs_act_se3(tij, qij, X0, X1);
   const float Z = (X1[2] < 0.5f * kMinDepthPy) ? 1.0f : X1[2];
   const size_t o = (size_t)e * hw + p;
-  reinterpret_cast<float2*>(coords)[o] = make_float2(fxj * (X1[0] / Z) + cxj, fyj * (X1[1] / Z) + cyj);
+  const float2 c = make_float2(fxj * (X1[0] / Z) + cxj, fyj * (X1[1] / Z) + cyj);
+  reinterpret_cast<float2*>(coords)[o] = c;
   valid[o] = ((X1[2] > kMinDepthPy) && (X0[2] > kMinDepthPy)) ? 1.0f : 0.0f;
+  if (kMotion) {
+    const float2 g = coords0[p];
+    reinterpret_cast<gs_half4*>(motion)[o] = gs_motion4(c, g.x, g.y, target[o]);
+  }
 }
 
 __global__ __launch_bounds__(256) void projmap_kernel(
@@ -152,8 +159,23 @@
   GS_REQUIRE(poses && disps && intrinsics && ii && jj && coords && valid, "reproject: null pointer");
   GS_GEOM_COMMON("reproject");
   GS_REQUIRE(n <= 65535, "reproject: n=%d exceeds grid.y limit", n);
-  reproject_kernel<<<dim3(gs_cdiv(hw, 256), n), 256, 0, st>>>(poses, disps, intrinsics, ii, jj, coords, valid, hw, w);
+  reproject_kernel<false><<<dim3(gs_cdiv(hw, 256), n), 256, 0, st>>>(poses, disps, intrinsics, ii, jj, coords, valid, hw,
+                                                                     w, nullptr, nullptr, nullptr);
   GS_CHECK_LAUNCH("reproject");
+  return GS_OK;
+}
+
+extern "C" int gs_reproject_motion(const float* poses, const float* disps, const float* intrinsics, const int64_t* ii,
+                                   const int64_t* jj, const float* coords0, const float* target, float* coords,
+                                   float* valid, void* motion, int n, int h, int w, gs_stream_t stream) {
+  GS_REQUIRE(poses && disps && intrinsics && ii && jj && coords && valid, "reproject_motion: null pointer");
+  GS_REQUIRE(coords0 && target && motion, "reproject_motion: null pointer");
+  GS_GEOM_COMMON("reproject_motion");
+  GS_REQUIRE(n <= 65535, "reproject_motion: n=%d exceeds grid.y limit", n);
+  reproject_kernel<true><<<dim3(gs_cdiv(hw, 256), n), 256, 0, st>>>(poses, disps, intrinsics, ii, jj, coords, valid, hw, w,
+                                                                    (const float2*)coords0, (const float2*)target,
+                                                                    (_Float16*)motion);
+  GS_CHECK_LAUNCH("reproject_motion");
   return GS_OK;
 }
 
diff --git a/go_slam_amd/csrc/gru_gates.hip b/go_slam_amd/csrc/gru_gates.hip
--- a/go_slam_amd/csrc/gru_gates.hip
+++ b/go_slam_amd/csrc/gru_gates.hip
@@ -421,21 +421,12 @@
   const int p = (int)(t % hw);
   const float gx = (float)(p % w), gy = (float)(p / w);
   const float2 c = coords1[t], tg = target[t];
-  typedef _Float16 half4m __attribute__((ext_vector_type(4)));
-  half4m o;
-  o[0] = (_Float16)fminf(fmaxf(c.x - gx, -64.0f), 64.0f);
-  o[1] = (_Float16)fminf(fmaxf(c.y - gy, -64.0f), 64.0f);
-  o[2] = (_Float16)fminf(fmaxf(tg.x - c.x, -64.0f), 64.0f);
-  o[3] = (_Float16)fminf(fmaxf(tg.y - c.y, -64.0f), 64.0f);
-  reinterpret_cast<half4m*>(out)[t] = o;
-}
-
-__global__ __launch_bounds__(256) void damping_rows_kernel(const float* __restrict__ eta, const int* __restrict__ inv,
-                                                           const int64_t* __restrict__ index,
-                                                           float* __restrict__ damping_buf, float* __restrict__ out,
-                                                           int hw, float scale, float eps, size_t total) {
-  const size_t t = (size_t)blockIdx.x * 256 + threadIdx.x;
-  if (t >= total) return;
+  reinterpret_cast<gs_half4*>(out)[t] = gs_motion4(c, gx, gy, tg);
+}
+
+__device__ __forceinline__ void damping_row_elem(const float* __restrict__ eta, const int* __restrict__ inv,
+                                                 const int64_t* __restrict__ index, float* __restrict__ damping_buf,
+                                                 float* __restrict__ out, int hw, float scale, float eps, size_t t) {
   const int k = (int)(t / hw), p = (int)(t - (size_t)k * hw);
   const int m = inv[k];
   float* slot = damping_buf + (size_t)index[k] * hw + p;
@@ -445,12 +436,19 @@
   out[t] = scale * v + eps;
 }
 
-__global__ __launch_bounds__(256) void ba_inputs_kernel(const float2* __restrict__ coords1, const float2* __restrict__ delta,
-                                                        const float2* __restrict__ weight, float2* __restrict__ target,
-                                                        float* __restrict__ ba_target, float* __restrict__ ba_weight,
-                                                        int hw, size_t total) {
-  const size_t t = (size_t)blockIdx.x * 256 + threadIdx.x;
-  if (t >= total) return;
+__global__ __launch_bounds__(256) void damping_rows_kernel(const float* __restrict__ eta, const int* __restrict__ inv,
+                                                           const int64_t* __restrict__ index,
+                                                           float* __restrict__ damping_buf, float* __restrict__ out,
+                                                           int hw, float scale, float eps, size_t total) {
+  const size_t t = (size_t)blockIdx.x * 256 + threadIdx.x;
+  if (t >= total) return;
+  damping_row_elem(eta, inv, index, damping_buf, out, hw, scale, eps, t);
+}
+
+__device__ __forceinline__ void ba_inputs_elem(const float2* __restrict__ coords1, const float2* __restrict__ delta,
+                                               const float2* __restrict__ weight, float2* __restrict__ target,
+                                               float* __restrict__ ba_target, float* __restrict__ ba_weight, int hw,
+                                               size_t t) {
   const size_t e = t / hw;
   const int p = (int)(t - e * hw);
   const float2 c = coords1[t], d = delta[t], wt = weight[t];
@@ -460,6 +458,29 @@
   bt[0] = tg.x; bt[hw] = tg.y;
   float* bw = ba_weight + e * 2 * hw + p;
   bw[0] = wt.x; bw[hw] = wt.y;
+}
+
+__global__ __launch_bounds__(256) void ba_inputs_kernel(const float2* __restrict__ coords1, const float2* __restrict__ delta,
+                                                        const float2* __restrict__ weight, float2* __restrict__ target,
+                                                        float* __restrict__ ba_target, float* __restrict__ ba_weight,
+                                                        int hw, size_t total) {
+  const size_t t = (size_t)blockIdx.x * 256 + threadIdx.x;
+  if (t >= total) return;
+  ba_inputs_elem(coords1, delta, weight, target, ba_target, ba_weight, hw, t);
+}
+
+__global__ __launch_bounds__(256) void ba_inputs_damping_kernel(
+    const float2* __restrict__ coords1, const float2* __restrict__ delta, const float2* __restrict__ weight,
+    float2* __restrict__ target, float* __restrict__ ba_target, float* __restrict__ ba_weight, size_t total_e,
+    unsigned edge_blocks, const float* __restrict__ eta, const int* __restrict__ inv, const int64_t* __restrict__ index,
+    float* __restrict__ damping_buf, float* __restrict__ out, float scale, float eps, size_t total_d, int hw) {
+  if (blockIdx.x < edge_blocks) {
+    const size_t t = (size_t)blockIdx.x * 256 + threadIdx.x;
+    if (t < total_e) ba_inputs_elem(coords1, delta, weight, target, ba_target, ba_weight, hw, t);
+  } else {
+    const size_t t = (size_t)(blockIdx.x - edge_blocks) * 256 + threadIdx.x;
+    if (t < total_d) damping_row_elem(eta, inv, index, damping_buf, out, hw, scale, eps, t);
+  }
 }
 }
 
@@ -499,3 +520,21 @@
   GS_CHECK_LAUNCH("damping_rows");
   return GS_OK;
 }
+
+extern "C" int gs_ba_inputs_damping(const float* coords1, const float* delta, const float* weight, float* target,
+                                    float* ba_target, float* ba_weight, int n, int h, int w, const float* eta,
+                                    const int* inv, const int64_t* index, float* damping_buf, float* out, int n_rows,
+                                    float scale, float eps, gs_stream_t stream) {
+  GS_REQUIRE(coords1 && delta && weight && target && ba_target && ba_weight, "ba_inputs_damping: null pointer");
+  GS_REQUIRE(inv && index && damping_buf && out, "ba_inputs_damping: null pointer");
+  GS_REQUIRE(n >= 0 && n_rows >= 0 && h > 0 && w > 0, "ba_inputs_damping: bad shape");
+  const size_t total_e = (size_t)n * h * w, total_d = (size_t)n_rows * h * w;
+  const size_t be = (total_e + 255) / 256, bd = (total_d + 255) / 256;
+  if (be + bd == 0) return GS_OK;
+  GS_REQUIRE(be + bd <= 0x7fffffffu, "ba_inputs_damping: %zu blocks exceed the grid", be + bd);
+  ba_inputs_damping_kernel<<<(unsigned)(be + bd), 256, 0, (hipStream_t)stream>>>(
+      (const float2*)coords1, (const float2*)delta, (const float2*)weight, (float2*)target, ba_target, ba_weight, total_e,
+      (unsigned)be, eta, inv, index, damping_buf, out, scale, eps, total_d, h * w);
+  GS_CHECK_LAUNCH("ba_inputs_damping");
+  return GS_OK;
+}
diff --git a/go_slam_amd/depth_video.py b/go_slam_amd/depth_video.py
--- a/go_slam_amd/depth_video.py
+++ b/go_slam_amd/depth_video.py
@@ -232,6 +232,10 @@
         ii, jj = DepthVideo.format_indices(ii, jj, self.device)
         return droid_backends.reproject(self.poses, self.disps, self.intrinsics, ii, jj)
 
+    def reproject_motion(self, ii, jj, coords0, target):
+        ii, jj = DepthVideo.format_indices(ii, jj, self.device)
+        return droid_backends.reproject(self.poses, self.disps, self.intrinsics, ii, jj, coords0=coords0, target=target)
+
     def distance(self, ii=None, jj=None, beta=0.3, bidirectional=True):
         return_matrix = False
         N = self._count()
diff --git a/go_slam_amd/droid_backends.py b/go_slam_amd/droid_backends.py
--- a/go_slam_amd/droid_backends.py
+++ b/go_slam_amd/droid_backends.py
@@ -225,7 +225,7 @@
     return corr
 
 
-def reproject(poses, disps, intrinsics, ii, jj):
+def reproject(poses, disps, intrinsics, ii, jj, coords0=None, target=None):
     _chk("poses", poses, torch.float32)
     _chk("disps", disps, torch.float32)
     _chk("intrinsics", intrinsics, torch.float32)
@@ -235,6 +235,20 @@
     _, ht, wd = disps.shape
     coords = torch.empty(1, n, ht, wd, 2, dtype=torch.float32, device=poses.device)
     valid = torch.empty(1, n, ht, wd, 1, dtype=torch.float32, device=poses.device)
+    if target is not None:
+        _chk("coords0", coords0, torch.float32)
+        _chk("target", target, torch.float32)
+        if coords0.numel() != ht * wd * 2 or target.numel() != n * ht * wd * 2:
+            raise RuntimeError(f"reproject: coords0 {tuple(coords0.shape)} / target {tuple(target.shape)} do not match "
+                               f"{n} edges of {ht}x{wd}")
+        motion = torch.empty(n, ht, wd, 4, dtype=torch.float16, device=poses.device)
+        with torch.cuda.device(poses.device):
+            rc = _lib.lib().gs_reproject_motion(_lib.ptr(poses), _lib.ptr(disps), _lib.ptr(intrinsics), _lib.ptr(ii),
+                                                _lib.ptr(jj), _lib.ptr(coords0), _lib.ptr(target), _lib.ptr(coords),
+                                                _lib.ptr(valid), _lib.ptr(motion), n, ht, wd,
+                                                _lib.stream_ptr(poses.device))
+        _lib.check(rc, "reproject_motion")
+        return coords, valid, motion
     with torch.cuda.device(poses.device):
         rc = _lib.lib().gs_reproject(_lib.ptr(poses), _lib.ptr(disps), _lib.ptr(intrinsics), _lib.ptr(ii),
                                      _lib.ptr(jj), _lib.ptr(coords), _lib.ptr(valid), n, ht, wd,
diff --git a/go_slam_amd/factor_graph.py b/go_slam_amd/factor_graph.py
--- a/go_slam_amd/factor_graph.py
+++ b/go_slam_amd/factor_graph.py
@@ -120,6 +120,13 @@
         c["uniq_host"] = uniq
         self._eidx = c
         return c
+
+    def _motion_fusable(self):
+        return hasattr(self.video, "reproject_motion") and self.channels_last and self.target.is_cuda \
+            and self.target.dtype == torch.float32 and self.target.is_contiguous() \
+            and self.coords0.dtype == torch.float32 and self.coords0.is_contiguous() \
+            and self.coords0.numel() == 2 * self.ht * self.wd \
+            and self.target.numel() == 2 * self.ht * self.wd * self.ii.numel()
 
     def _glue_fusable(self, coords1):
         return coords1.is_cuda and self.channels_last and self.target.dtype == torch.float32 \
@@ -369,16 +376,21 @@
     def update(self, t0=None, t1=None, iters=2, use_inactive=False, EPS=1e-7, motion_only=False):
         idx = self._edge_index(t0, t1, use_inactive)
         t0, t1, seg = idx["t0"], idx["t1"], idx["seg"]
-        coords1, mask = self.video.reproject(self.ii, self.jj)
-        fused = self._glue_fusable(coords1)
         ht, wd = self.ht, self.wd
         E = self.ii.numel()
+        m4 = None
+        if self._motion_fusable():
+            coords1, mask, m4 = self.video.reproject_motion(self.ii, self.jj, self.coords0, self.target)
+        else:
+            coords1, mask = self.video.reproject(self.ii, self.jj)
+        fused = self._glue_fusable(coords1)
         if fused:
             from . import _lib
             L, st = _lib.lib(), _lib.stream_ptr(self.device)
-            m4 = torch.empty(E, ht, wd, 4, dtype=torch.float16, device=self.device)
-            _lib.check(L.gs_motion_features(_lib.ptr(coords1), _lib.ptr(self.target), _lib.ptr(m4), E, ht, wd, st),
-                       "motion_features")
+            if m4 is None:
+                m4 = torch.empty(E, ht, wd, 4, dtype=torch.float16, device=self.device)
+                _lib.check(L.gs_motion_features(_lib.ptr(coords1), _lib.ptr(self.target), _lib.ptr(m4), E, ht, wd, st),
+                           "motion_features")
             motion = m4.permute(0, 3, 1, 2).unsqueeze(0)
         else:
             motion = torch.cat([coords1 - self.coords0, self.target - coords1], dim=-1)
@@ -394,12 +406,22 @@
         if not fuse_damping:
             self.damping[seg["uniq"]] = damping.float()
         eta_rows = damping
+        damping_done = False
         if fused and delta.dtype == torch.float32 and weight.dtype == torch.float32:
             bt, bw, n_in = self._ba_buffers(idx, use_inactive)
             target_new = torch.empty_like(coords1)
-            _lib.check(L.gs_ba_inputs(_lib.ptr(coords1), _lib.ptr(delta.contiguous()), _lib.ptr(weight.contiguous()),
-                                      _lib.ptr(target_new), bt[n_in:].data_ptr(), bw[n_in:].data_ptr(), E, ht, wd, st),
-                       "ba_inputs")
+            if fuse_damping:
+                damping = torch.empty(idx["damping_index"].numel(), ht, wd, device=self.device)
+                _lib.check(L.gs_ba_inputs_damping(
+                    _lib.ptr(coords1), _lib.ptr(delta.contiguous()), _lib.ptr(weight.contiguous()), _lib.ptr(target_new),
+                    bt[n_in:].data_ptr(), bw[n_in:].data_ptr(), E, ht, wd, _lib.ptr(eta_rows),
+                    _lib.ptr(idx["damping_inv"]), _lib.ptr(idx["damping_index"]), _lib.ptr(self.damping),
+                    _lib.ptr(damping), damping.shape[0], 0.2, float(EPS), st), "ba_inputs_damping")
+                damping_done = True
+            else:
+                _lib.check(L.gs_ba_inputs(_lib.ptr(coords1), _lib.ptr(delta.contiguous()), _lib.ptr(weight.contiguous()),
+                                          _lib.ptr(target_new), bt[n_in:].data_ptr(), bw[n_in:].data_ptr(), E, ht, wd,
+                                          st), "ba_inputs")
             self.target, self.weight = target_new, weight
             target, weight = bt, bw
         else:
@@ -414,7 +436,9 @@
             target = target.view(-1, ht, wd, 2).permute(0, 3, 1, 2).contiguous()
             weight = weight.view(-1, ht, wd, 2).permute(0, 3, 1, 2).contiguous()
 
-        if fuse_damping:
+        if damping_done:
+            pass
+        elif fuse_damping:
             damping = torch.empty(idx["damping_index"].numel(), ht, wd, device=self.device)
             _lib.check(L.gs_damping_rows(_lib.ptr(eta_rows), _lib.ptr(idx["damping_inv"]), _lib.ptr(idx["damping_index"]),
                                          _lib.ptr(self.damping), _lib.ptr(damping), damping.shape[0], ht * wd, 0.2,
diff --git a/go_slam_amd/synth.py b/go_slam_amd/synth.py
--- a/go_slam_amd/synth.py
+++ b/go_slam_amd/synth.py
@@ -7,6 +7,8 @@
     "Rep": (40, 80, 640.0),
     "Scan": (30, 40, 320.0),
     "tiny": (12, 16, 128.0),
+    "odd": (9, 11, 88.0),
+    "mini": (6, 8, 64.0),
 }
 
 
diff --git a/include/goslam_hip.h b/include/goslam_hip.h
--- a/include/goslam_hip.h
+++ b/include/goslam_hip.h
@@ -78,6 +78,9 @@
 int gs_reproject(const float* poses, const float* disps, const float* intrinsics,
                  const int64_t* ii, const int64_t* jj, float* coords, float* valid,
                  int n, int h, int w, gs_stream_t stream);
+int gs_reproject_motion(const float* poses, const float* disps, const float* intrinsics, const int64_t* ii,
+                        const int64_t* jj, const float* coords0, const float* target, float* coords, float* valid,
+                        void* motion, int n, int h, int w, gs_stream_t stream);
 
 int gs_projmap(const float* poses, const float* disps, const float* intrinsics,
                const int64_t* ii, const int64_t* jj, float* coords, float* valid,
@@ -209,6 +212,10 @@
 
 int gs_damping_rows(const float* eta, const int* inv, const int64_t* index, float* damping_buf, float* out,
                     int n_rows, int hw, float scale, float eps, gs_stream_t stream);
+int gs_ba_inputs_damping(const float* coords1, const float* delta, const float* weight, float* target,
+                         float* ba_target, float* ba_weight, int n, int h, int w, const float* eta, const int* inv,
+                         const int64_t* index, float* damping_buf, float* out, int n_rows, float scale, float eps,
+                         gs_stream_t stream);
 
 int gs_cvx_upsample(const float* disps, const void* mask, const int64_t* ix, float* out,
                     int m, int h, int w, int mask_channels_last, gs_stream_t stream);
```
